# yifangao112/DinoUNet

Hardware: AMD Instinct MI355X
Metric: 2D slices/sec training, dinounet_l 512x512 bf16 (higher is better)
Workload: dtype bf16; 1 GPU; dinounet_l train step (fwd+loss+bwd+clip+SGD), 512x512x3 slices, batch 8/GPU, frozen ViT + adapter + FAPM + U-Net decoder, random-init weights; global_batch=8, parallelism=dp1

## Files before the change

### dinounet_amd/_lib.py

```python
import ctypes as C
import os
import re

HERE = os.path.dirname(os.path.abspath(__file__))
LIB_PATH = os.path.join(HERE, "libdinounet_hip.so")
HEADER = os.path.join(os.path.dirname(HERE), "include", "dinounet_hip.h")

DU_F32, DU_BF16 = 0, 1
PLAIN_ROW, PLAIN_COL, IM2COL_ROW, IM2COL_COL = 0, 1, 2, 3
ACT_NONE, ACT_GELU, ACT_RELU, ACT_LEAKY, ACT_SWIGLU = 0, 1, 2, 3, 4
STORE_PLAIN, STORE_PIXEL_SHUFFLE2, STORE_QKV_ROPE, STORE_SLABS, STORE_QKV_HEADS, STORE_MSDA_PREP = 0, 1, 2, 4, 5, 6
ERRORS = {-1: "DU_ERR_BAD_ARG", -2: "DU_ERR_UNSUPPORTED", -3: "DU_ERR_LAUNCH"}


class ConvGeom(C.Structure):
    _fields_ = [("p2", C.c_void_p), ("ld2", C.c_int64), ("C1", C.c_int32), ("Hi", C.c_int32), ("Wi", C.c_int32),
                ("C", C.c_int32), ("KH", C.c_int32), ("KW", C.c_int32), ("stride", C.c_int32), ("pad", C.c_int32),
                ("Ho", C.c_int32), ("Wo", C.c_int32), ("transposed", C.c_int32)]


class GemmArgs(C.Structure):
    _fields_ = [("dtype", C.c_int32), ("out_dtype", C.c_int32), ("a_mode", C.c_int32), ("b_mode", C.c_int32),
                ("M", C.c_int32), ("N", C.c_int32), ("K", C.c_int32),
                ("A", C.c_void_p), ("lda", C.c_int64), ("a_batch_stride", C.c_int64),
                ("B", C.c_void_p), ("ldb", C.c_int64), ("b_batch_stride", C.c_int64),
                ("C", C.c_void_p), ("ldc", C.c_int64), ("c_batch_stride", C.c_int64),
                ("batch", C.c_int32), ("split_k", C.c_int32), ("alpha", C.c_float),
                ("bias", C.c_void_p), ("act", C.c_int32), ("gamma", C.c_void_p),
                ("row_scale", C.c_void_p), ("rs_rows", C.c_int32),
                ("residual", C.c_void_p), ("ldr", C.c_int64),
                ("store_mode", C.c_int32), ("ps_H", C.c_int32), ("ps_W", C.c_int32), ("ps_C", C.c_int32),
                ("geom", ConvGeom), ("ws", C.c_void_p), ("ws_elems", C.c_int64),
                ("rope_sin", C.c_void_p), ("rope_cos", C.c_void_p), ("rope_prefix", C.c_int32), ("rope_qscale", C.c_float),
                ("a_colsum", C.c_void_p), ("b_colsum", C.c_void_p), ("C2", C.c_void_p), ("ks_ws", C.c_void_p), ("ks_ws_bytes", C.c_int64)]


class TnJob(C.Structure):
    _fields_ = [("A", C.c_void_p), ("lda", C.c_int64), ("B", C.c_void_p), ("ldb", C.c_int64), ("C", C.c_void_p), ("ldc", C.c_int64),
                ("a_colsum", C.c_void_p), ("alpha", C.c_void_p), ("M", C.c_int32), ("N", C.c_int32), ("K", C.c_int32),
                ("accumulate", C.c_int32), ("b_colsum", C.c_void_p),
                ("gather", C.c_int32), ("Hs", C.c_int32), ("Ws", C.c_int32), ("Cb", C.c_int32),
                ("taps", C.c_int32), ("inner", C.c_int32), ("inner_total", C.c_int32), ("c_off", C.c_int32)]


_CTYPE = {"int": C.c_int, "int64_t": C.c_int64, "float": C.c_float, "int32_t": C.c_int32, "double": C.c_double}


def header_prototypes(path=HEADER):
    src = open(path).read()
    src = re.sub(r"/\*.*?\*/", "", src, flags=re.S)
    protos = {}
    for m in re.finditer(r"\b(int64_t|int|const char\*)\s+(du_\w+)\s*\(([^;]*?)\)\s*;", src, flags=re.S):
        ret, name, args = m.group(1), m.group(2), m.group(3).strip()
        types = []
        if args and args != "void":
            for a in args.split(","):
                a = a.strip()
                if "*" in a:
                    types.append(C.c_void_p)
                else:
                    types.append(_CTYPE[a.split()[0] if not a.startswith("const") else a.split()[1]])
        protos[name] = (C.c_char_p if "char" in ret else (C.c_int64 if ret == "int64_t" else C.c_int), types)
    return protos


_lib = None


def lib():
    global _lib
    if _lib is None:
        if not os.path.exists(LIB_PATH):
            raise RuntimeError(
                f"{LIB_PATH} not found: the HIP extension is required (no CPU / eager fallback exists). "
                "Build it with `python -m dinounet_amd._build` or `__graft_entry__.build()`.")
        l = C.CDLL(LIB_PATH)
        for name, (ret, types) in header_prototypes().items():
            fn = getattr(l, name)
            fn.restype = ret
            fn.argtypes = types
        _lib = l
        for kv in os.environ.get("DINOUNET_LIB_OPTIONS", "").split(","):
            if "=" in kv:
                k, v = kv.split("=", 1)
                l.du_set_option(int(k), int(v))
    return _lib


def check(rc: int, what: str):
    if rc != 0:
        raise RuntimeError(f"dinounet_hip: {what} failed with {ERRORS.get(rc, rc)}")
```

### dinounet_amd/csrc/gemm.hip

```cpp
#include "common.h"
#include "gemm_params.h"
#include "gemm_plan.h"

namespace {

template <typename T, int MODE, int OUTER, int BK, int NT>
struct TileLoader {
  static constexpr int VEC = Elem<T>::VEC;
  static constexpr int LDS_LD = BK + VEC;
  static constexpr int TOTAL = OUTER * BK / VEC;
  static constexpr int NV = (TOTAL + NT - 1) / NT;
  static constexpr bool ROWMODE = (MODE == DU_PLAIN_ROW || MODE == DU_IM2COL_ROW);
  static constexpr int KV = BK / VEC;
  static constexpr int OV = OUTER / VEC;

  uint4 regs[NV];
  int pb[NV], py[NV], px[NV];

  __device__ __forceinline__ void init(const Operand& op, int tid, int o0, int outer_dim, int kbeg) {
    if constexpr (MODE == DU_IM2COL_ROW) {
#pragma unroll
      for (int i = 0; i < NV; i++) {
        int v = tid + i * NT;
        int o = o0 + v / KV;
// ... 320 lines not shown
      return;
    }
  }
  const int c = du_gemm_p8_choice(a);
  if (c) { multi_phase(a, c, 0); return; }
  if (du_gemm_glds_serves(a)) { p.family = 2; return; }
  if (du_gemm_modes_served(a.a_mode, a.b_mode)) p.family = 1; else p.rc = DU_ERR_UNSUPPORTED;
}

int64_t plan_ks_bytes(const du_gemm_args& a) {
  if (a.dtype != DU_BF16 || a.a_mode != DU_PLAIN_ROW || a.b_mode != DU_PLAIN_ROW) return 0;
  du_gemm_args head = a;
  head.ks_ws = nullptr; head.ks_ws_bytes = 0;
  int r = a.M % 256;
  if (r < 1 || r > 64 || !du_gemm_p8_tail_ok(a, r)) r = 0;
  head.M = a.M - r;
  const long pair = du_gemm_p8_ks_bytes(head);
  const int c = r > 0 ? du_gemm_p8_choice(head) : 0;
  const long tail = (c == 1 || c == 2) ? du_gemm_p8_tail_bytes(a) : 0;
  return pair > tail ? pair : tail;
}

int plan_check(const du_gemm_args& a, int family) {
  if (a.M <= 0 || a.N <= 0 || a.K <= 0) return DU_ERR_BAD_ARG;
  if (!a.A || !a.B || !a.C) return DU_ERR_BAD_ARG;
  const int vec = a.dtype == DU_BF16 ? 8 : 4;
  if (a.dtype != DU_BF16 && a.dtype != DU_F32) return DU_ERR_BAD_ARG;
  if (a.out_dtype != DU_BF16 && a.out_dtype != DU_F32) return DU_ERR_BAD_ARG;
  if (!aligned16(a.A) || !aligned16(a.B)) return DU_ERR_BAD_ARG;
  auto chk = [&](int mode, long ld, int outer, long bs) {
    if (ld % vec || bs % vec) return false;
    if (mode == DU_PLAIN_ROW) return a.K % vec == 0;
    if (mode == DU_PLAIN_COL) return outer % vec == 0;
    return true;
  };
  if (!chk(a.a_mode, a.lda, a.M, a.a_batch_stride) || !chk(a.b_mode, a.ldb, a.N, a.b_batch_stride)) return DU_ERR_BAD_ARG;
  const bool a_i2c = (a.a_mode == DU_IM2COL_ROW), b_i2c = (a.b_mode == DU_IM2COL_COL);
  if (a_i2c || b_i2c) {
    const du_conv_geom& g = a.geom;
    if (g.C % vec || g.KH <= 0 || g.KW <= 0 || g.stride <= 0) return DU_ERR_BAD_ARG;
    if (g.p2 && (g.C1 % vec || g.ld2 % vec || !aligned16(g.p2))) return DU_ERR_BAD_ARG;
    if (a_i2c && a.K != g.KH * g.KW * g.C) return DU_ERR_BAD_ARG;
    if (b_i2c && a.N != g.KH * g.KW * g.C) return DU_ERR_BAD_ARG;
  }
  const bool k_scale = a.row_scale && a.a_mode == DU_PLAIN_COL;
  if (k_scale && (family != 1 || a.rs_rows <= 0 || a.rs_rows % 64 || a.bias || a.act || a.gamma || a.residual || a.store_mode)) return DU_ERR_UNSUPPORTED;
  if (a.split_k > 1 && (a.out_dtype != DU_F32 || a.bias || a.act || a.gamma || (a.row_scale && !k_scale) || a.residual ||
                        (a.store_mode && a.store_mode != DU_STORE_SLABS))) return DU_ERR_BAD_ARG;
  if (a.store_mode == DU_STORE_SLABS && (a.split_k <= 1 || a.batch > 1 || family != 1)) return DU_ERR_UNSUPPORTED;
  if (a.store_mode == DU_STORE_PIXEL_SHUFFLE2 && (a.ps_C <= 0 || a.N != 4 * a.ps_C || a.ps_H <= 0 || a.ps_W <= 0 || a.M % (a.ps_H * a.ps_W))) return DU_ERR_BAD_ARG;
  const bool wgrad = a.a_mode == DU_PLAIN_COL && (family == 1 || family == 5);
  if (a.b_colsum && (!wgrad || a.b_mode != DU_IM2COL_COL || a.geom.C <= 0 || a.N % a.geom.C)) return DU_ERR_UNSUPPORTED;
  if (a.a_colsum && !wgrad) return DU_ERR_UNSUPPORTED;
  return DU_OK;
}

}

GemmPlan du_gemm_plan(const du_gemm_args& a) {
  static const bool generic_only = DU_GETENV("DU_GEMM_GENERIC") != nullptr;
  GemmPlan p{};
  plan_kernels(a, generic_only, p);
  if (!generic_only) {
    p.ws_elems = du_gemm_ragged_rows(a) > 0 ? du_gemm_skinny_ws_elems(a.N, a.K) : 0;
    p.ks_ws_bytes = plan_ks_bytes(a);
  }
  const int rc = plan_check(a, p.family);
  if (rc != DU_OK) p.rc = rc;
  return p;
}

extern "C" int du_gemm_route(const du_gemm_args* pa) { return pa ? du_gemm_plan(*pa).family : DU_ERR_BAD_ARG; }
extern "C" int64_t du_gemm_ws_elems(const du_gemm_args* pa) { return pa ? du_gemm_plan(*pa).ws_elems : 0; }
extern "C" int64_t du_gemm_ks_ws_bytes(const du_gemm_args* pa) { return pa ? du_gemm_plan(*pa).ks_ws_bytes : 0; }

extern "C" int du_gemm_plan_describe(const du_gemm_args* pa, int64_t* out, int n) {
  if (!pa || !out || n < 9) return DU_ERR_BAD_ARG;
  const GemmPlan p = du_gemm_plan(*pa);
  const int64_t v[9] = {p.rc, p.family, p.variant, p.gather, p.tail_rows, p.tail_form, p.tn_splits, p.ws_elems, p.ks_ws_bytes};
  for (int i = 0; i < 9; i++) out[i] = v[i];
  return 9;
}

extern "C" int du_gemm(const du_gemm_args* pa, void* stream) {
  if (!pa) return DU_ERR_BAD_ARG;
  const GemmPlan p = du_gemm_plan(*pa);
  if (p.rc != DU_OK) return p.rc;
  hipStream_t st = (hipStream_t)stream;
  du_gemm_args head = *pa, tail = *pa;
  if (p.tail_rows) split_rows(*pa, p.tail_rows, head, tail);
  int rc;
  if (p.variant) rc = du_gemm_nt_p8(head, st, p.variant, p.tail_form == DU_TAIL_RIDES ? p.tail_rows : 0);
  else switch (p.family) {
    case 0: rc = launch_generic(head, st); break;
    case 1: rc = du_gemm_bf16_tiles(head, st); break;
    case 2: rc = du_gemm_nt_glds(head, st); break;
    case 5: rc = du_gemm_tn_p8(head, st, p.tn_splits); break;
    default: rc = du_gemm_nt_rk(head, st); break;
  }
  if (rc != DU_OK) return rc;
  switch (p.tail_form) {
    case DU_TAIL_SKINNY_FUSED: case DU_TAIL_SKINNY_PAIR: return du_gemm_skinny(tail, st, p.tail_form);
    case DU_TAIL_TILE_ENGINE: tail.ws = nullptr; tail.ws_elems = 0; return du_gemm_bf16_tiles(tail, st);
  }
  return rc;
}
```

### dinounet_amd/csrc/gemm_p8.hip

```cpp
#include <algorithm>
#include <vector>
#include "common.h"
#include "gemm_params.h"
#include "gemm_plan.h"
#include "gemm_skinny_body.h"

namespace {

typedef __attribute__((address_space(3))) void lds_void;

constexpr int PBM = 256, PBN = 256, PBK = 64;
constexpr int HALF_B = 128 * PBK * 2;
constexpr int BUF_B = 4 * HALF_B;
constexpr int STG_LD = PBN + 4;

template <typename TC> struct Out4p;
template <> struct Out4p<float> {
  static __device__ __forceinline__ void load(const float* p, float* v) { float4 t = *(const float4*)p; v[0] = t.x; v[1] = t.y; v[2] = t.z; v[3] = t.w; }
  static __device__ __forceinline__ void store(float* p, const float* v) { *(float4*)p = make_float4(v[0], v[1], v[2], v[3]); }
};
template <> struct Out4p<bf16_t> {
  static __device__ __forceinline__ void load(const bf16_t* p, float* v) {
    bf16x4 t = __builtin_bit_cast(bf16x4, *(const uint2*)p);
#pragma unroll
// ... 1353 lines not shown
    stage_block_f32(acc[2 * h][0], stg, N_STG_LDF, wm * 64 + (lane & 31), wn * 64, lane);
    stage_block_f32(acc[2 * h][1], stg, N_STG_LDF, wm * 64 + (lane & 31), wn * 64 + 32, lane);
    stage_block_f32(acc[2 * h + 1][0], stg, N_STG_LDF, wm * 64 + 32 + (lane & 31), wn * 64, lane);
    stage_block_f32(acc[2 * h + 1][1], stg, N_STG_LDF, wm * 64 + 32 + (lane & 31), wn * 64 + 32, lane);
    __syncthreads();
    auto half = [&](auto w_c) {
      constexpr int w = decltype(w_c)::value;
      const int mrow0 = m0 + w * 128 + h * 64;
      const float* sp = stg + w * 64 * N_STG_LDF;
      if constexpr (sizeof(TC) == 4) {
        if (pre) {
          constexpr int CW = NBN / 4;
          float4 rr[8];
#pragma unroll
          for (int u = 0; u < 8; u++) {
            const int v = tid + u * 256;
            const int m = mrow0 + v / CW, n = n0 + (v % CW) * 4;
            rr[u] = (m < P.M && n < P.N) ? *(const float4*)((const float*)Rb + (long)m * P.ldr + n) : make_float4(0.f, 0.f, 0.f, 0.f);
          }
#pragma unroll
          for (int u = 0; u < 8; u++) {
            const int v = tid + u * 256;
            const int row = v / CW, cw = v % CW;
            const int m = mrow0 + row, n = n0 + cw * 4;
            if (m < P.M && n < P.N) {
              const float4 tt = *(const float4*)(sp + row * N_STG_LDF + cw * 4);
              float o[4] = {tt.x * P.alpha, tt.y * P.alpha, tt.z * P.alpha, tt.w * P.alpha};
              if (P.bias) {
                const float4 bb = *(const float4*)(P.bias + n);
                o[0] += bb.x; o[1] += bb.y; o[2] += bb.z; o[3] += bb.w;
              }
              if (P.act != DU_ACT_NONE) {
#pragma unroll
                for (int e = 0; e < 4; e++) o[e] = apply_act(o[e], P.act);
              }
              if (P.gamma) {
                const float4 gg = *(const float4*)(P.gamma + n);
                o[0] *= gg.x; o[1] *= gg.y; o[2] *= gg.z; o[3] *= gg.w;
              }
              if (P.row_scale) {
                const float rs = P.row_scale[m / P.rs_rows];
#pragma unroll
                for (int e = 0; e < 4; e++) o[e] *= rs;
              }
              *(float4*)((float*)Cb + (long)m * P.ldc + n) = make_float4(o[0] + rr[u].x, o[1] + rr[u].y, o[2] + rr[u].z, o[3] + rr[u].w);
            }
          }
          return;
        }
      }
      readout_f32_any<TC, NBN, 256>(P, sp, N_STG_LDF, 64, mrow0, n0, Cb, Rb, tid);
    };
    half(IC<0>{});
    half(IC<1>{});
  };
  pass(IC<0>{});
  pass(IC<1>{});
}

constexpr int PP_BIAS_OFF = P8N_LDS;
constexpr int PP_LDS = P8N_LDS + 3 * 128 * 4;
constexpr unsigned PP_OOR = 0x80000000u;

__device__ __forceinline__ void pp_swap_halves(unsigned& a, unsigned& b) {
  asm volatile("s_nop 1\n\tv_permlane32_swap_b32 %0, %1" : "+v"(a), "+v"(b));
}
__device__ __forceinline__ void pp_lds_read1(f32x4& a, unsigned addr) { asm volatile("ds_read_b128 %0, %1" : "=&v"(a) : "v"(addr)); }
__device__ __forceinline__ void pp_wait_lds(f32x4& a, f32x4& b) { asm volatile("s_waitcnt lgkmcnt(0)" : "+v"(a), "+v"(b) : : "memory"); }
__device__ __forceinline__ void pp_wait_lds1(f32x4& a) { asm volatile("s_waitcnt lgkmcnt(0)" : "+v"(a) : : "memory"); }

struct PpIdent {
  unsigned short v[128 * 128];
  constexpr PpIdent() : v() { for (int i = 0; i < 128; i++) v[i * 128 + i] = 0x3F80; }
};
__device__ const PpIdent g_pp_ident{};

constexpr int PP_ROPE_OFF = PP_BIAS_OFF + 2048;
constexpr int PP_ROPE_ROWS = 33;
constexpr int PP_LDS_ROPE = PP_ROPE_OFF + 2 * PP_ROPE_ROWS * 128;
__device__ __forceinline__ void pp_wait_lds4(f32x4& a, f32x4& b, f32x4& c, f32x4& d) {
  asm volatile("s_waitcnt lgkmcnt(0)" : "+v"(a), "+v"(b), "+v"(c), "+v"(d) : : "memory");
}

template <int ACT, bool NK4, int RES = 0, bool PS = false, int QKV = 0>
__global__ __launch_bounds__(512) void gemm_nt_pp_kernel(GemmParams P) {
  constexpr bool ROPE = QKV == 1, HEADS = QKV == 2;
  extern __shared__ __attribute__((aligned(16))) unsigned char smem[];
  if (P.tail_rows && (int)blockIdx.x >= P.main_wgs) { p8_tail<bf16_t>(P, smem); return; }
  static_assert(RES == 0 || ACT == DU_ACT_NONE, "the residual form has no activation");
  static_assert(QKV == 0 || (ACT == DU_ACT_NONE && !NK4 && RES == 0 && !PS), "the qkv stores: plain bias epilogue, K >= 384");
  constexpr bool FOUR = NK4 && RES == 0;
  const int tid = threadIdx.x, lane = tid & 63, hi = lane >> 5;
  const int wave = __builtin_amdgcn_readfirstlane(tid >> 6);
  const int wm = wave >> 1, wn = wave & 1;
  const int G = P.main_wgs;
  int lin;
  {
    const int bid = blockIdx.x, q = G >> 3, r = G & 7, xcd = bid & 7, idx = bid >> 3;
    lin = (xcd < r ? xcd * (q + 1) : r * (q + 1) + (xcd - r) * q) + idx;
  }
  const int ntiles = P.tiles_m * P.tiles_n;
  const int nk = P.K / PBK + (RES ? 2 : 0);
  auto coords = [&](int tile, int& m0, int& n0) {
    int tm, tn;
    if (P.group_m > 1) {
      const int band = P.group_m * P.tiles_n;
      const int g = tile / band, l = tile - g * band;
      const int first = g * P.group_m;
      const int gsz = min(P.tiles_m - first, P.group_m);
      tn = l / gsz; tm = first + (l - tn * gsz);
    } else {
      tm = tile / P.tiles_n; tn = tile - tm * P.tiles_n;
    }
    m0 = tm * PBM; n0 = tn * NBN;
  };

  const auto ra = __builtin_amdgcn_make_buffer_rsrc((void*)P.a.p, 0, (int)((((long)P.M - 1) * P.a.ld + P.K) * 2), 0x00020000);
  const auto rb = __builtin_amdgcn_make_buffer_rsrc((void*)P.b.p, 0, (int)((((long)P.N - 1) * P.b.ld + P.K) * 2), 0x00020000);
  const long out_rows = PS ? 4L * P.M : (long)P.M;
  const int out_cols = PS ? P.ps_C : P.N;
  const auto rc = __builtin_amdgcn_make_buffer_rsrc(P.C, 0, QKV ? (int)(3 * P.ldc * 2) : (int)(((out_rows - 1) * P.ldc + out_cols) * 2), 0x00020000);
  const int ps_lw = PS ? __builtin_ctz(P.ps_W) : 0, ps_lh = PS ? __builtin_ctz(P.ps_H) : 0;
  auto ps_pixel = [&](unsigned m) -> unsigned {
    const unsigned x = m & (unsigned)(P.ps_W - 1), y = (m >> ps_lw) & (unsigned)(P.ps_H - 1), b = m >> (ps_lw + ps_lh);
    return ((b * 2u * (unsigned)P.ps_H + 2u * y) * 2u * (unsigned)P.ps_W) + 2u * x;
  };
  const auto rbias = __builtin_amdgcn_make_buffer_rsrc(P.bias ? (void*)P.bias : P.C, 0, P.bias ? P.N * 4 : 0, 0x00020000);
  const int nrec_r = RES ? (int)(((out_rows - 1) * P.ldr + out_cols) * 2) : 0;
  const unsigned ldr2 = (unsigned)(P.ldr * 2);

  const int lc = (lane & 7) ^ (((wave & 1) << 2) | (lane >> 4));
  int srow[2];
  unsigned va0[2][2], vb0[2];
#pragma unroll
  for (int r = 0; r < 2; r++) {
    srow[r] = (r * 8 + wave) * 8 + (lane >> 3);
    va0[0][r] = (unsigned)srow[r] * (unsigned)(P.a.ld * 2) + lc * 16;
    va0[1][r] = (unsigned)(128 + srow[r]) * (unsigned)(P.a.ld * 2) + lc * 16;
    vb0[r] = (unsigned)srow[r] * (unsigned)(P.b.ld * 2) + lc * 16;
  }
  const unsigned lds_base = (unsigned)(unsigned long long)(__attribute__((address_space(3))) unsigned char*)smem;
  unsigned va_s[2][2], vb_s[2];
  unsigned sa_base = 0, sb_base = 0, sr_base = 0;
  unsigned sm0 = 0;
  unsigned sn0 = 0;
  auto set_stage_tile = [&](int tile, int slot) {
    if (tile < ntiles) {
      int m0, n0;
      coords(tile, m0, n0);
#pragma unroll
      for (int r = 0; r < 2; r++) {
        if constexpr (ROPE) {
          sm0 = (unsigned)m0; sn0 = (unsigned)n0;
        } else {
          va_s[0][r] = m0 + srow[r] < P.M ? va0[0][r] : PP_OOR;
          va_s[1][r] = m0 + 128 + srow[r] < P.M ? va0[1][r] : PP_OOR;
          vb_s[r] = n0 + srow[r] < P.N ? vb0[r] : PP_OOR;
        }
      }
      sa_base = (unsigned)m0 * (unsigned)(P.a.ld * 2);
      sb_base = (unsigned)n0 * (unsigned)(P.b.ld * 2);
      if constexpr (RES != 0 && !PS) sr_base = (unsigned)m0 * ldr2 + (unsigned)n0 * 2u;
      if constexpr (RES != 0 && PS) {
        const int q = n0 / P.ps_C, co0 = n0 - q * P.ps_C;
        sr_base = (unsigned)((q >> 1) * 2 * P.ps_W + (q & 1)) * ldr2 + (unsigned)co0 * 2u;
        sm0 = (unsigned)m0;
      }
      if (wave < 2) {
        const unsigned lds_dst = __builtin_amdgcn_readfirstlane(lds_base + PP_BIAS_OFF + slot * 512 + wave * 256);
        const unsigned voff = (unsigned)(n0 + wave * 64 + lane) * 4u;
        unsigned keep;
        asm volatile("s_mov_b32 %0, m0\n\ts_mov_b32 m0, %3\n\ts_nop 0\n\tbuffer_load_dword %1, %2, 0 offen lds\n\ts_mov_b32 m0, %0"
                     : "=&s"(keep) : "v"(voff), "s"(rbias), "s"(lds_dst) : "memory");
      }
    } else {
#pragma unroll
      for (int r = 0; r < 2; r++) { va_s[0][r] = PP_OOR; va_s[1][r] = PP_OOR; vb_s[r] = PP_OOR; }
      if constexpr (ROPE) { sm0 = 0x7fffffffu; sn0 = 0x7fffffffu; }
    }
  };
  const auto rr = __builtin_amdgcn_make_buffer_rsrc(RES ? (void*)P.residual : (void*)P.a.p, 0, nrec_r, 0x00020000);
  const auto ri = __builtin_amdgcn_make_buffer_rsrc((void*)g_pp_ident.v, 0, 32768, 0x00020000);
  auto stage = [&](auto which_c, int bo, unsigned kofs, auto ext_c) {
    constexpr int which = decltype(which_c)::value;
    constexpr bool EXT = RES != 0 && decltype(ext_c)::value != 0;
#pragma unroll
    for (int r = 0; r < 2; r++) {
      unsigned char* dst = smem + bo + which * HALF_B + (r * 8 + wave) * 1024;
      if constexpr (EXT) {
        unsigned sr = (unsigned)srow[r];
        asm volatile("" : "+v"(sr));
        if constexpr (which < 2) {
          const unsigned rowi = PS ? ps_pixel(sm0 + which * 128u + sr) : which * 128u + sr;
          const unsigned vext = va_s[which][r] == PP_OOR ? PP_OOR : rowi * ldr2 + (unsigned)lc * 16u;
          __builtin_amdgcn_raw_ptr_buffer_load_lds(rr, (lds_void*)dst, 16, vext, sr_base + kofs, 0, 0);
        } else {
          __builtin_amdgcn_raw_ptr_buffer_load_lds(ri, (lds_void*)dst, 16, sr * 256u + (unsigned)lc * 16u, kofs, 0, 0);
        }
      } else if constexpr (ROPE) {
        unsigned sr = (unsigned)srow[r];
        asm volatile("" : "+v"(sr));
        if constexpr (which < 2) {
          const unsigned row = which * 128u + sr;
          const unsigned vo = sm0 + row < (unsigned)P.M ? row * (unsigned)(P.a.ld * 2) + (unsigned)lc * 16u : PP_OOR;
          __builtin_amdgcn_raw_ptr_buffer_load_lds(ra, (lds_void*)dst, 16, vo, sa_base + kofs, 0, 0);
        } else {
          const unsigned vo = sn0 + sr < (unsigned)P.N ? sr * (unsigned)(P.b.ld * 2) + (unsigned)lc * 16u : PP_OOR;
          __builtin_amdgcn_raw_ptr_buffer_load_lds(rb, (lds_void*)dst, 16, vo, sb_base + kofs, 0, 0);
        }
      } else {
        if constexpr (which < 2) __builtin_amdgcn_raw_ptr_buffer_load_lds(ra, (lds_void*)dst, 16, va_s[which][r], sa_base + kofs, 0, 0);
        else __builtin_amdgcn_raw_ptr_buffer_load_lds(rb, (lds_void*)dst, 16, vb_s[r], sb_base + kofs, 0, 0);
      }
    }
  };
  int L[4];
  {
    const int x = hi ^ ((lane >> 1) & 7);
#pragma unroll
    for (int kk = 0; kk < 4; kk++) L[kk] = (lane & 31) * 128 + ((x ^ (2 * kk)) << 4);
  }
  const int aoff = wm * 32 * 128, boff = 2 * HALF_B + wn * 64 * 128;

  bf16x8 Af[2][4];
  bf16x8 Bf[2][2][4];
  f32x16 acc[2][2];
  f32x16 prev[2][2];
#pragma unroll
  for (int i = 0; i < 2; i++)
#pragma unroll
    for (int c = 0; c < 2; c++)
#pragma unroll
      for (int r = 0; r < 16; r++) prev[i][c][r] = 0.f;
  auto readA = [&](auto set_c, int bo) {
    constexpr int set = decltype(set_c)::value;
#pragma unroll
    for (int kk = 0; kk < 4; kk++) Af[set][kk] = *(const bf16x8*)(smem + bo + set * HALF_B + aoff + L[kk]);
  };
  auto readB = [&](auto set_c, int bo) {
    constexpr int set = decltype(set_c)::value;
#pragma unroll
    for (int c = 0; c < 2; c++)
#pragma unroll
      for (int kk = 0; kk < 4; kk++) Bf[set][c][kk] = *(const bf16x8*)(smem + bo + boff + c * 4096 + L[kk]);
  };
  auto mma = [&](auto i_c, auto bset_c, auto first_c) {
    constexpr int i = decltype(i_c)::value, bset = decltype(bset_c)::value;
    constexpr bool FIRST = decltype(first_c)::value;
#pragma unroll
    for (int kk = 0; kk < 4; kk++)
#pragma unroll
      for (int c = 0; c < 2; c++) {
        if constexpr (FIRST) {
          if (kk == 0) {
            const f32x16 z = {0.f, 0.f, 0.f, 0.f, 0.f, 0.f, 0.f, 0.f, 0.f, 0.f, 0.f, 0.f, 0.f, 0.f, 0.f, 0.f};
            acc[i][c] = __builtin_amdgcn_mfma_f32_32x32x16_bf16(Bf[bset][c][kk], Af[i][kk], z, 0, 0, 0);
            continue;
          }
        }
        acc[i][c] = __builtin_amdgcn_mfma_f32_32x32x16_bf16(Bf[bset][c][kk], Af[i][kk], acc[i][c], 0, 0, 0);
      }
  };
  auto pin = [&](auto nrd_c, auto ndma_c) {
    constexpr int nrd = decltype(nrd_c)::value, ndma = decltype(ndma_c)::value;
#pragma unroll
    for (int m = 0; m < 8; m++) {
      __builtin_amdgcn_sched_group_barrier(0x008, 1, 0);
      if (m < 4) __builtin_amdgcn_sched_group_barrier(0x100, nrd / 4, 0);
      else if (m - 4 < ndma) __builtin_amdgcn_sched_group_barrier(0x020, 1, 0);
    }
  };
  const int nlim = (P.dbg & 1) ? 0 : P.N;
  unsigned pbias = lds_base + PP_BIAS_OFF + (unsigned)((wn * 64 + 4 * hi) * 4);
  unsigned crow[2] = {PP_OOR, PP_OOR};
  int pcol = 0;
  float rs_cur = 1.0f, rs_prev = 1.0f;
  unsigned trow[2] = {0u, 0u};
  float qs_prev = 1.0f;
  const unsigned rope_tbl = lds_base + PP_ROPE_OFF + (unsigned)(4 * hi * 4);
  auto set_prev_tile = [&](int tile) {
    int m0, n0;
    coords(tile, m0, n0);
    pcol = n0 + wn * 64 + hi * 8;
    if constexpr (QKV != 0) {
      const int hd = P.ps_C * 64, which = n0 / hd, head = ((n0 - which * hd) >> 6) + wn;
      if constexpr (ROPE) qs_prev = which == 0 ? P.rope_qscale : 1.0f;
#pragma unroll
      for (int i = 0; i < 2; i++) {
        const int m = m0 + i * 128 + wm * 32 + (lane & 31);
        const int b = m / P.ps_H, t = m - b * P.ps_H;
        crow[i] = m < P.M ? (unsigned)(((long)which * P.ldc + (((long)b * P.ps_C + head) * P.ps_W + t) * 64 + hi * (ROPE ? 4 : 8)) * 2) : PP_OOR;
        if constexpr (ROPE) {
          const int tt = t - P.rope_prefix, ty = tt / P.b.Wi, tx = tt - ty * P.b.Wi;
          trow[i] = (which < 2 && tt >= 0 && m < P.M) ? (unsigned)ty | ((unsigned)tx << 8) : (32u | (32u << 8));
        }
      }
      return;
    }
#pragma unroll
    for (int i = 0; i < 2; i++) {
      const int m = m0 + i * 128 + wm * 32 + (lane & 31);
      if constexpr (PS) {
        const int q = n0 / P.ps_C, co0 = n0 - q * P.ps_C;
        const unsigned pix = ps_pixel((unsigned)m) + (unsigned)((q >> 1) * 2 * P.ps_W + (q & 1));
        crow[i] = m < P.M ? (unsigned)(((long)pix * P.ldc + co0 + wn * 64 + hi * 8) * 2) : PP_OOR;
      } else {
        crow[i] = m < P.M ? (unsigned)(((long)m * P.ldc + pcol) * 2) : PP_OOR;
      }
    }
  };
  f32x4 bqa = {0.f, 0.f, 0.f, 0.f}, bqb = {0.f, 0.f, 0.f, 0.f};
  unsigned keep0 = 0u, keep1 = 0u;
  f32x4 cq = {0.f, 0.f, 0.f, 0.f}, sq = {0.f, 0.f, 0.f, 0.f};
  auto fetch = [&](auto h_c, f32x4& bq, unsigned base) {
    constexpr int h = decltype(h_c)::value;
    if constexpr (h >= 0) {
      if constexpr (ROPE) {
        constexpr int ph = h >> 1, c = h & 1, i = ph >> 2, g = ph & 3, axis = g >> 1;
        pp_lds_read1(bq, base + (unsigned)((c * 32 + 8 * g) * 4));
        if constexpr (c == 0) {
          const unsigned pos = axis ? (trow[i] >> 8) : (trow[i] & 0xffu);
          const unsigned ta = rope_tbl + (unsigned)(axis * PP_ROPE_ROWS * 128 + ((8 * g) & 15) * 4) + pos * 128u;
          pp_lds_read1(cq, ta);
          pp_lds_read1(sq, ta + 64u);
        }
      } else {
        constexpr int u = h >> 1, c = (u >> 1) & 1, g = 2 * (u & 1) + (h & 1);
        pp_lds_read1(bq, base + (unsigned)((c * 32 + 8 * g) * 4));
      }
    }
  };
  auto rope_pair = [&](auto h_c) {
    constexpr int h = decltype(h_c)::value;
    if constexpr (h >= 0) {
      constexpr int ph = h >> 1, i = ph >> 2, g = ph & 3, h2 = g >> 1;
      const f32x16& a0 = prev[i][0];
      const f32x16& a1 = prev[i][1];
      unsigned pk[4];
#pragma unroll
      for (int e = 0; e < 4; e += 2) {
        const float ca = cq[e], sa = sq[e], cb = cq[e + 1], sb = sq[e + 1];
        const float x1a = a0[4 * g + e] + bqa[e], x1b = a0[4 * g + e + 1] + bqa[e + 1];
        const float x2a = a1[4 * g + e] + bqb[e], x2b = a1[4 * g + e + 1] + bqb[e + 1];
        const float o1a = (x1a * ca - x2a * sa) * qs_prev, o1b = (x1b * cb - x2b * sb) * qs_prev;
        const float o2a = (x2a * ca + x1a * sa) * qs_prev, o2b = (x2b * cb + x1b * sb) * qs_prev;
        const bf16x2 t1 = {(bf16_t)o1a, (bf16_t)o1b}, t2 = {(bf16_t)o2a, (bf16_t)o2b};
        pk[e >> 1] = __builtin_bit_cast(unsigned, t1);
        pk[2 + (e >> 1)] = __builtin_bit_cast(unsigned, t2);
      }
      (void)h2;
      typedef unsigned u32x2_t __attribute__((ext_vector_type(2)));
      const u32x2_t v0 = {pk[0], pk[1]}, v1 = {pk[2], pk[3]};
      const unsigned off = nlim ? crow[i] + (unsigned)(8 * g * 2) : PP_OOR;
      __builtin_amdgcn_raw_buffer_store_b64(v0, rc, off, 0, 0);
      __builtin_amdgcn_raw_buffer_store_b64(v1, rc, off == PP_OOR ? PP_OOR : off + 64u, 0, 0);
    }
  };
  auto half = [&](auto h_c, const f32x4& bq) {
    constexpr int h = decltype(h_c)::value;
    if constexpr (h >= 0) {
      constexpr int u = h >> 1, part = h & 1, i = u >> 2, c = (u >> 1) & 1, h2 = u & 1, g = 2 * h2 + part;
      const f32x16& a = prev[i][c];
      f32x2 o0, o1;
      if constexpr (RES == 2) {
        o0 = {__builtin_fmaf(bq[0], rs_prev, a[4 * g]), __builtin_fmaf(bq[1], rs_prev, a[4 * g + 1])};
        o1 = {__builtin_fmaf(bq[2], rs_prev, a[4 * g + 2]), __builtin_fmaf(bq[3], rs_prev, a[4 * g + 3])};
      } else {
        o0 = {a[4 * g] + bq[0], a[4 * g + 1] + bq[1]}; o1 = {a[4 * g + 2] + bq[2], a[4 * g + 3] + bq[3]};
      }
      if constexpr (ACT == DU_ACT_GELU) { o0 = gelu_pk(o0); o1 = gelu_pk(o1); }
      const bf16x2 t0 = {(bf16_t)o0.x, (bf16_t)o0.y}, t1 = {(bf16_t)o1.x, (bf16_t)o1.y};
      if constexpr (part == 0) {
        keep0 = __builtin_bit_cast(unsigned, t0); keep1 = __builtin_bit_cast(unsigned, t1);
      } else {
        unsigned k4 = __builtin_bit_cast(unsigned, t0), k5 = __builtin_bit_cast(unsigned, t1);
        pp_swap_halves(keep0, k4);
        pp_swap_halves(keep1, k5);
        const u32x4_t v = {keep0, keep1, k4, k5};
        const unsigned off = pcol + c * 32 + 16 * h2 < nlim ? crow[i] + (unsigned)((c * 32 + 16 * h2) * 2) : PP_OOR;
        __builtin_amdgcn_raw_buffer_store_b128(v, rc, off, 0, 0);
      }
    }
  };
  auto finish6 = [&]() {
    __builtin_amdgcn_sched_barrier(0);
    asm volatile("s_waitcnt vmcnt(6)" ::: "memory");
    if constexpr (ROPE) pp_wait_lds4(bqa, bqb, cq, sq); else pp_wait_lds(bqa, bqb);
    __builtin_amdgcn_s_barrier();
    __builtin_amdgcn_sched_barrier(0);
  };
// ... 68 lines not shown

  int bc = 0, bn = NBUF_B, bnn = 2 * NBUF_B;
  int slot = 0;
  auto rot2 = [&]() { const int o = bc; bc = bnn; bnn = bn; bn = o; };
  auto bias_at = [&](int sl) { return lds_base + PP_BIAS_OFF + (unsigned)(sl * 512 + (wn * 64 + 4 * hi) * 4); };
  for (;;) {
    const int next = tile + G;
    if constexpr (RES == 2) {
      int m0c, n0c;
      coords(tile, m0c, n0c);
      rs_cur = P.row_scale[__builtin_amdgcn_readfirstlane(m0c / P.rs_rows)];
    }
    if constexpr (FOUR) {
      const int nslot = slot == 2 ? 0 : slot + 1;
      dstep(IC<0>{}, IC<0>{}, bc, bn, bnn, 2u * 128u, 0u);
      dstep(IC<1>{}, IC<1>{}, bn, bnn, bc, 3u * 128u, 0u);
      rot2();
      set_stage_tile(next, nslot);
      dstep(IC<2>{}, IC<0>{}, bc, bn, bnn, 0u, 0u);
      dstep(IC<3>{}, IC<1>{}, bn, bnn, bc, 128u, bias_at(slot));
      rot2();
      pbias = bias_at(slot);
      set_prev_tile(tile);
      slot = nslot;
    } else {
      dstep(IC<0>{}, IC<0>{}, bc, bn, bnn, 2u * 128u, 0u);
      dstep(IC<1>{}, IC<1>{}, bn, bnn, bc, 3u * 128u, 0u);
      rot2();
      dstep(IC<2>{}, IC<0>{}, bc, bn, bnn, 4u * 128u, 0u);
      dstep(IC<3>{}, IC<1>{}, bn, bnn, bc, 5u * 128u, 0u);
      rot2();
      int t = 4;
      for (; t + (RES != 0 && !NK4 ? 4 : 2) < nk; t += 2) {
        kstep(IC<0>{}, F_{}, N_{}, N_{}, N_{}, N_{}, N_{}, N_{}, F_{}, F_{}, bc, bn, bnn, (unsigned)(t + 2) * 128u, 0u, 0u, IC<0>{}, IC<0>{});
        kstep(IC<1>{}, F_{}, N_{}, N_{}, N_{}, N_{}, N_{}, N_{}, F_{}, F_{}, bn, bnn, bc, (unsigned)(t + 3) * 128u, 0u, 0u, IC<0>{}, IC<0>{});
        rot2();
      }
      if constexpr (RES != 0 && !NK4) {
        kstep(IC<0>{}, F_{}, N_{}, N_{}, N_{}, N_{}, N_{}, N_{}, F_{}, F_{}, bc, bn, bnn, 0u, 0u, 0u, IC<0>{}, IC<1>{});
        kstep(IC<1>{}, F_{}, N_{}, N_{}, N_{}, N_{}, N_{}, N_{}, F_{}, F_{}, bn, bnn, bc, 128u, 0u, 0u, IC<1>{}, IC<1>{});
        rot2();
      }
      set_stage_tile(next, slot ^ 1);
      pbias = bias_at(slot);
      if constexpr (ROPE) set_prev_tile(tile);
      kstep(IC<0>{}, F_{}, N_{}, N_{}, N_{}, N_{}, N_{}, N_{}, F_{}, F_{}, bc, bn, bnn, 0u, 0u, 0u, IC<2>{}, IC<0>{});
      kstep(IC<1>{}, F_{}, N_{}, N_{}, N_{}, N_{}, IC<0>{}, IC<1>{}, F_{}, T_{}, bn, bnn, bc, 128u, 0u, pbias, IC<0>{}, IC<0>{});
      rot2();
      if constexpr (!ROPE) set_prev_tile(tile);
      rs_prev = rs_cur;
      slot ^= 1;
    }
    tile = next;
    if (tile >= ntiles) break;
  }
  prev[1][0] = acc[1][0]; prev[1][1] = acc[1][1];
  if (P.dbg & 2) return;
  auto last = [&](auto h_c) {
    constexpr int h = decltype(h_c)::value;
    pp_wait_lds(bqa, bqb);
    __builtin_amdgcn_sched_barrier(0);
    if constexpr (h & 1) half(h_c, bqb); else half(h_c, bqa);
    __builtin_amdgcn_sched_barrier(0);
    if constexpr (h & 1) { fetch(IC<(h + 1 < 16 ? h + 1 : -1)>{}, bqa, pbias); fetch(IC<(h + 2 < 16 ? h + 2 : -1)>{}, bqb, pbias); }
  };
  auto last_pair = [&](auto ph_c) {
    constexpr int ph = decltype(ph_c)::value;
    pp_wait_lds4(bqa, bqb, cq, sq);
    __builtin_amdgcn_sched_barrier(0);
    rope_pair(IC<2 * ph>{});
    __builtin_amdgcn_sched_barrier(0);
    fetch(IC<(ph + 1 < 8 ? 2 * ph + 2 : -1)>{}, bqa, pbias); fetch(IC<(ph + 1 < 8 ? 2 * ph + 3 : -1)>{}, bqb, pbias);
  };
  if constexpr (ROPE) {
    last_pair(IC<0>{}); last_pair(IC<1>{}); last_pair(IC<2>{}); last_pair(IC<3>{});
    last_pair(IC<4>{}); last_pair(IC<5>{}); last_pair(IC<6>{}); last_pair(IC<7>{});
  } else {
    last(IC<0>{}); last(IC<1>{}); last(IC<2>{}); last(IC<3>{}); last(IC<4>{}); last(IC<5>{}); last(IC<6>{}); last(IC<7>{});
    last(IC<8>{}); last(IC<9>{}); last(IC<10>{}); last(IC<11>{}); last(IC<12>{}); last(IC<13>{}); last(IC<14>{}); last(IC<15>{});
  }
  if (P.tail_rows && (int)gridDim.x == G) p8_tail_inline<bf16_t>(P, smem, lin, G);
}

int g_p8_mode = -1;
int g_p8_sched = 1;
int g_p8_corun = 1;
int g_p8_persist = 1;
int g_p8_tail_inline = 0;
int g_p8_res = 1;
int g_p8_pp_full = 0;
int g_p8_group = 4;
int g_p8_debug = 0;

constexpr long KS_STATE_BYTES = 131072;
int g_p8_tail_slices = 1;
static int tail_slices_for(const du_gemm_args& a, bool have_ws) {
  if (!g_p8_tail_slices || a.K < (g_p8_tail_slices >= 2 ? 1024 : 2048) || g_p8_tail_inline) return 1;
  const int units = (a.N + SK_BN - 1) / SK_BN;
  int s = a.K / 512;
  if (s > 8) s = 8;
  while (s > 1 && (a.K % (s * SK_CHUNK) || units * s > 256)) s--;
  if (s < 2 || units > 16384) return 1;
  if (have_ws && (!a.ks_ws || a.ks_ws_bytes < KS_STATE_BYTES + (long)units * s * 64 * SK_BN * 4)) return 1;
  return s;
}

template <typename TC, int SCHED, bool NARROW, bool GA = false>
int launch_p8(const du_gemm_args& a, hipStream_t st, int tail_rows = 0) {
  static_assert(!(NARROW && GA), "the gather form exists for the 256 x 256 kernel only");
  constexpr int LDS_BYTES = NARROW ? P8N_LDS : P8_LDS;
  constexpr int TBN = NARROW ? NBN : PBN;
  GemmParams P = make_params(a, GA ? DU_IM2COL_ROW : DU_PLAIN_ROW, DU_PLAIN_ROW, PBM, TBN, PBK);
  P.tiles_m = (a.M + PBM - 1) / PBM;
  P.group_m = g_p8_group;
  P.dbg = g_p8_debug;
  dim3 grid(P.tiles_m * P.tiles_n, a.batch < 1 ? 1 : a.batch);
  if (tail_rows > 0 && !GA) {
    P.tail_rows = tail_rows; P.main_wgs = P.tiles_m * P.tiles_n;
    if (!(g_p8_tail_inline && grid.y == 1 && (long)grid.x * g_p8_corun >= 256)) {
      P.tail_slices = tail_slices_for(a, true); P.ks_ws = a.ks_ws;
      grid.x += (a.N + SK_BN - 1) / SK_BN * P.tail_slices;
    }
  }
  void (*kfn)(GemmParams);
  if constexpr (NARROW) kfn = gemm_nt_p8n_kernel<TC, SCHED>; else kfn = gemm_nt_p8_kernel<TC, SCHED, false, GA>;
  static bool attr_set = false;
  if (!attr_set) {
    if (hipFuncSetAttribute((const void*)kfn, hipFuncAttributeMaxDynamicSharedMemorySize, LDS_BYTES) != hipSuccess) return DU_ERR_LAUNCH;
    attr_set = true;
  }
  hipLaunchKernelGGL(kfn, grid, dim3(512), LDS_BYTES, st, P);
  return du_check_launch();
}

int launch_pp(const du_gemm_args& a, hipStream_t st, int tail_rows = 0) {
  GemmParams P = make_params(a, DU_PLAIN_ROW, DU_PLAIN_ROW, PBM, NBN, PBK);
  P.tiles_m = (a.M + PBM - 1) / PBM;
  P.group_m = g_p8_group;
  P.dbg = g_p8_debug;
  const long ntiles = (long)P.tiles_m * P.tiles_n;
  const long cus = g_p8_pp_full ? 256 : 256 / g_p8_corun;
  P.main_wgs = (int)(ntiles < cus ? ntiles : cus);
  dim3 grid(P.main_wgs, 1);
  if (tail_rows > 0) {
    P.tail_rows = tail_rows;
    if (!g_p8_tail_inline) grid.x += (a.N + SK_BN - 1) / SK_BN;
  }
  const bool nk4 = a.K == 256;
  const int res = a.residual ? (a.row_scale ? 2 : 1) : 0;
  const bool ps = a.store_mode == DU_STORE_PIXEL_SHUFFLE2;
  const bool rope = a.store_mode == DU_STORE_QKV_ROPE;
  const bool heads = a.store_mode == DU_STORE_QKV_HEADS;
  if (rope) { P.b.Hi = a.geom.Hi; P.b.Wi = a.geom.Wi; }
  void (*kfn)(GemmParams);
  if (rope) kfn = gemm_nt_pp_kernel<DU_ACT_NONE, false, 0, false, 1>;
  else if (heads) kfn = gemm_nt_pp_kernel<DU_ACT_NONE, false, 0, false, 2>;
  else if (ps) kfn = gemm_nt_pp_kernel<DU_ACT_NONE, false, 1, true>;
  else if (res == 2) kfn = nk4 ? gemm_nt_pp_kernel<DU_ACT_NONE, true, 2> : gemm_nt_pp_kernel<DU_ACT_NONE, false, 2>;
  else if (res == 1) kfn = nk4 ? gemm_nt_pp_kernel<DU_ACT_NONE, true, 1> : gemm_nt_pp_kernel<DU_ACT_NONE, false, 1>;
  else if (nk4) kfn = a.act == DU_ACT_GELU ? gemm_nt_pp_kernel<DU_ACT_GELU, true> : gemm_nt_pp_kernel<DU_ACT_NONE, true>;
  else kfn = a.act == DU_ACT_GELU ? gemm_nt_pp_kernel<DU_ACT_GELU, false> : gemm_nt_pp_kernel<DU_ACT_NONE, false>;
  static bool attr_set[11] = {false, false, false, false, false, false, false, false, false, false, false};
  const int lds_bytes = rope ? PP_LDS_ROPE : PP_LDS;
  const int ai = heads ? 10 : rope ? 9 : ps ? 8 : (res ? 2 + 2 * res + (nk4 ? 1 : 0) : (a.act == DU_ACT_GELU ? 1 : 0) + (nk4 ? 2 : 0));
  if (!attr_set[ai]) {
    if (hipFuncSetAttribute((const void*)kfn, hipFuncAttributeMaxDynamicSharedMemorySize, lds_bytes) != hipSuccess) return DU_ERR_LAUNCH;
    attr_set[ai] = true;
  }
  hipLaunchKernelGGL(kfn, grid, dim3(512), lds_bytes, st, P);
  return du_check_launch();
}

template <typename TC>
int launch_p4(const du_gemm_args& a, hipStream_t st, int tail_rows = 0) {
  GemmParams P = make_params(a, DU_PLAIN_ROW, DU_PLAIN_ROW, PBM, NBN, 32);
  P.tiles_m = (a.M + PBM - 1) / PBM;
  P.group_m = g_p8_group;
  P.dbg = g_p8_debug;
  dim3 grid(P.tiles_m * P.tiles_n, a.batch < 1 ? 1 : a.batch);
  if (tail_rows > 0) {
    P.tail_rows = tail_rows; P.main_wgs = P.tiles_m * P.tiles_n;
    grid.x += (a.N + SK_BN - 1) / SK_BN;
  }
  void (*kfn)(GemmParams) = gemm_nt_p4_kernel<TC>;
  static bool attr_set = false;
  if (!attr_set) {
    if (hipFuncSetAttribute((const void*)kfn, hipFuncAttributeMaxDynamicSharedMemorySize, P4_LDS) != hipSuccess) return DU_ERR_LAUNCH;
    attr_set = true;
  }
  hipLaunchKernelGGL(kfn, grid, dim3(256), P4_LDS, st, P);
  return du_check_launch();
}

int g_p8_ks = 0;
inline long ks_ws_need(long tiles) { return KS_STATE_BYTES + tiles * 2 * PBM * PBN * 4; }

int launch_p8ks(const du_gemm_args& a, hipStream_t st, int tail_rows) {
  GemmParams P = make_params(a, DU_PLAIN_ROW, DU_PLAIN_ROW, PBM, PBN, PBK);
  P.tiles_m = (a.M + PBM - 1) / PBM;
  P.group_m = g_p8_group;
  P.dbg = g_p8_debug;
  P.ks_ws = a.ks_ws;
  P.main_wgs = 2 * P.tiles_m * P.tiles_n;
  dim3 grid(P.main_wgs, 1);
  if (tail_rows > 0) { P.tail_rows = tail_rows; grid.x += (a.N + SK_BN - 1) / SK_BN; }
  void (*kfn)(GemmParams) = g_p8_sched ? gemm_nt_p8ks_kernel<1> : gemm_nt_p8ks_kernel<0>;
  static bool attr_set[2] = {false, false};
  if (!attr_set[g_p8_sched ? 1 : 0]) {
    if (hipFuncSetAttribute((const void*)kfn, hipFuncAttributeMaxDynamicSharedMemorySize, P8_LDS) != hipSuccess) return DU_ERR_LAUNCH;
    attr_set[g_p8_sched ? 1 : 0] = true;
  }
  hipLaunchKernelGGL(kfn, grid, dim3(512), P8_LDS, st, P);
  return du_check_launch();
}

int g_p8_tn = 1;

template <int SCHED, bool GA>
int launch_p8_tn(const du_gemm_args& a, int splits, hipStream_t st) {
  GemmParams P = make_params(a, DU_PLAIN_COL, GA ? DU_IM2COL_COL : DU_PLAIN_COL, PBM, PBN, PBK);
  P.tiles_m = (a.M + PBM - 1) / PBM;
  P.split_k = splits;
  P.k_per_split = 0;
  P.dbg = g_p8_debug;
  dim3 grid(P.tiles_m * P.tiles_n * splits, 1);
  void (*kfn)(GemmParams) = GA ? gemm_nt_p8_kernel<float, SCHED, true, true> : gemm_nt_p8_kernel<float, SCHED, true, false>;
  static bool attr_set = false;
  if (!attr_set) {
    if (hipFuncSetAttribute((const void*)kfn, hipFuncAttributeMaxDynamicSharedMemorySize, P8_LDS) != hipSuccess) return DU_ERR_LAUNCH;
    attr_set = true;
  }
  hipLaunchKernelGGL(kfn, grid, dim3(512), P8_LDS, st, P);
  return du_check_launch();
}

}

extern int g_attn_w;
extern int g_attn_impl, g_attn_thresh_log2, g_attn_var;
extern int g_rk_mode;
extern int g_wgrad_rows;
extern int g_ln_rows2;
extern int g_dwconv_band;

extern "C" int du_set_option(int key, int value) {
  switch (key) {
    case 4: g_attn_w = value; return DU_OK;
    case 6: g_attn_impl = value; return DU_OK;
    case 7: g_attn_thresh_log2 = value; return DU_OK;
    case 8: g_attn_var = value; return DU_OK;
    case 0: g_p8_mode = value; return DU_OK;
    case 1: g_p8_sched = value; return DU_OK;
// ... 73 lines not shown
    if ((4L * a.M * a.ldc + a.N) * 2 >= 0x7fffffffL || (4L * a.M * a.ldr + a.N) * 2 >= 0x7fffffffL) return false;
  } else if (a.store_mode != DU_STORE_PLAIN) return false;
  if (a.gamma || a.alpha != 1.0f || (a.act != DU_ACT_NONE && a.act != DU_ACT_GELU)) return false;
  if ((a.K != 256 && a.K < 384) || a.N % 8 || a.ldc % 8 || (((uintptr_t)a.C) & 15)) return false;
  const long lim = 0x7fffffffL;
  if (a.residual) {
    if (a.act != DU_ACT_NONE || a.N % 128 || a.ldr % 8 || (((uintptr_t)a.residual) & 15)) return false;
    if (a.row_scale && (a.rs_rows < 256 || a.rs_rows % 256)) return false;
    if (((long)a.M * a.ldr + a.N) * 2 >= lim) return false;
  } else if (a.row_scale) return false;
  return ((long)a.M * a.lda + a.K) * 2 < lim && ((long)a.N * a.ldb + a.K) * 2 < lim && ((long)a.M * a.ldc + a.N) * 2 < lim;
}

static bool ks_shape_ok(const du_gemm_args& a) {
  if (!p8_legal(a) || a.out_dtype != DU_F32 || a.store_mode != DU_STORE_PLAIN || a.batch > 1 || a.act == DU_ACT_SWIGLU) return false;
  if (a.K % 256 || a.K < 1024 || g_p8_corun != 1) return false;
  const long tiles = (long)((a.M + 255) / 256) * ((a.N + 255) / 256);
  return tiles % 8 == 0 && tiles >= 64 && tiles <= 128;
}
static bool ks_legal(const du_gemm_args& a) {
  if (!ks_shape_ok(a) || !a.ks_ws || (((uintptr_t)a.ks_ws) & 15)) return false;
  return a.ks_ws_bytes >= ks_ws_need((long)((a.M + 255) / 256) * ((a.N + 255) / 256));
}

int du_gemm_p8_choice(const du_gemm_args& a) {
  if (g_p8_mode != 0 && g_p8_tn && p8_gather_legal(a))
    return (g_p8_mode > 0 || (long)((a.M + 255) / 256) * ((a.N + 255) / 256) >= 192) ? 1 : 0;
  if (g_p8_mode == 0 || !p8_legal(a)) return 0;
  if (a.store_mode == DU_STORE_MSDA_PREP) return 1;
  if (a.store_mode == DU_STORE_QKV_HEADS) return (g_p8_mode != 0 && pp_legal(a)) ? 4 : 0;
  if (a.store_mode == DU_STORE_QKV_ROPE) {
    const long t = (long)((a.M + 255) / 256) * ((a.N + 127) / 128);
    return (g_p8_persist && g_p8_mode != 2 && pp_legal(a) && (g_p8_persist > 1 || g_p8_mode == 4 || t >= 2 * (256 / g_p8_corun))) ? 4 : 2;
  }
  if (g_p8_ks && g_p8_mode < 0 && ks_legal(a)) return 5;
  if (g_p8_mode == 5) return ks_legal(a) ? 5 : 2;
  if (g_p8_mode == 3) return a.act == DU_ACT_SWIGLU ? 2 : 3;
  if (g_p8_mode == 4) return pp_legal(a) ? 4 : 2;
  if (g_p8_mode > 0) return g_p8_mode == 2 ? 2 : 1;
  const long batch = a.batch < 1 ? 1 : a.batch;
  const long tm = (a.M + 255) / 256;
  const long t256 = tm * ((a.N + 255) / 256) * batch, t128 = tm * ((a.N + 127) / 128) * batch;
  const long cus = 256 / g_p8_corun;
  if (t128 * g_p8_corun < 192) return 0;
  const double c256 = (double)((t256 + cus - 1) / cus) * 1.0, c128 = (double)((t128 + cus - 1) / cus) * (a.K >= 1024 ? 0.68 : 0.56);
  if (g_p8_persist && pp_legal(a)) {
    if (a.residual) {
      if (g_p8_res && (g_p8_persist > 1 || t128 >= 2 * cus)) return 4;
    } else {
    const double r = a.K <= 256 ? 0.40 : (a.K <= 512 ? 0.45 : (a.act == DU_ACT_GELU ? 0.49 : 0.53));
    const double cpp = (double)((t128 + cus - 1) / cus) * r;
    const double best = (t256 * g_p8_corun >= 128 && c256 <= c128) ? c256 : c128;
    if (g_p8_persist > 1 || (t128 >= 2 * cus && cpp < best)) return 4;
    }
  }
  if (t256 * g_p8_corun >= 128 && c256 <= c128) return 1;
  return 2;
}
bool du_gemm_p8_wants(const du_gemm_args& a) { return du_gemm_p8_choice(a) != 0; }
long du_gemm_p8_tail_bytes(const du_gemm_args& whole) {
  const int s = tail_slices_for(whole, false);
  return s > 1 ? KS_STATE_BYTES + (long)((whole.N + SK_BN - 1) / SK_BN) * s * 64 * SK_BN * 4 : 0;
}
long du_gemm_p8_ks_bytes(const du_gemm_args& a) {
  if (!(g_p8_ks && g_p8_mode < 0) && g_p8_mode != 5) return 0;
  return ks_shape_ok(a) ? ks_ws_need((long)((a.M + 255) / 256) * ((a.N + 255) / 256)) : 0;
}

int du_gemm_nt_p8(const du_gemm_args& a, hipStream_t st, int c, int tail_rows) {
  if (a.a_mode == DU_IM2COL_ROW) return g_p8_sched ? launch_p8<bf16_t, 1, false, true>(a, st) : launch_p8<bf16_t, 0, false, true>(a, st);
  const bool bf = a.out_dtype == DU_BF16;
  const int tr = tail_rows;
  if (c == 5) return launch_p8ks(a, st, tr);
  if (c == 4) return launch_pp(a, st, tr);
  if (c == 3) return bf ? launch_p4<bf16_t>(a, st, tr) : launch_p4<float>(a, st, tr);
  if (c == 1) {
    if (bf) return g_p8_sched ? launch_p8<bf16_t, 1, false>(a, st, tr) : launch_p8<bf16_t, 0, false>(a, st, tr);
    return g_p8_sched ? launch_p8<float, 1, false>(a, st, tr) : launch_p8<float, 0, false>(a, st, tr);
  }
  if (bf) return g_p8_sched ? launch_p8<bf16_t, 1, true>(a, st, tr) : launch_p8<bf16_t, 0, true>(a, st, tr);
  return g_p8_sched ? launch_p8<float, 1, true>(a, st, tr) : launch_p8<float, 0, true>(a, st, tr);
}

bool du_gemm_p8_tail_ok(const du_gemm_args& whole, int r) {
  static const bool off = DU_GETENV("DU_P8_NO_TAIL") != nullptr;
  static const int kmax = DU_GETENV("DU_SKINNY_FUSE_KMAX") ? atoi(DU_GETENV("DU_SKINNY_FUSE_KMAX")) : 4096;
  if (off || r < 1 || r > 64 || whole.K > kmax || whole.K % SK_CHUNK || whole.N % 4 || whole.batch > 1) return false;
  if ((whole.store_mode != DU_STORE_PLAIN && whole.store_mode != DU_STORE_QKV_HEADS) || whole.act == DU_ACT_SWIGLU ||
      whole.a_mode != DU_PLAIN_ROW || whole.b_mode != DU_PLAIN_ROW) return false;
  return 8 * 64 * (SK_BN + 1) * 4 <= P8_LDS;
}

int du_gemm_tn_p8_splits(const du_gemm_args& a) {
  if (!g_p8_tn || g_p8_mode == 0) return 0;
  if (a.dtype != DU_BF16 || a.out_dtype != DU_F32 || a.a_mode != DU_PLAIN_COL) return 0;
  if (a.b_mode != DU_PLAIN_COL && a.b_mode != DU_IM2COL_COL) return 0;
  if (a.split_k <= 1 || a.batch > 1 || a.store_mode != DU_STORE_PLAIN) return 0;
  if (a.bias || a.act || a.gamma || a.row_scale || a.residual) return 0;
  if (a.K % 128 || a.K < 512 || a.M <= 128 || a.N <= 128) return 0;
  if (a.lda % 8 || a.ldb % 8 || (((uintptr_t)a.A) & 15) || (((uintptr_t)a.B) & 15)) return 0;
  if (a.b_mode == DU_IM2COL_COL) {
    if (!convt_gather_geom(a, a.B, a.ldb, a.K) || a.N != 4 * a.geom.C || a.geom.C % 256) return 0;
    if (a.geom.Wo & (a.geom.Wo - 1)) return 0;
  }
  const long tiles = (long)((a.M + 255) / 256) * ((a.N + 255) / 256);
  const int npairs = a.K / 128;
  long s = tiles >= 256 ? 1 : 256 / tiles;
  if (s > npairs / 2) s = npairs / 2;
  if (s < 1) s = 1;
  if (g_p8_tn < 2 && npairs / s < 16) return 0;
  const long ldmax = a.b_mode == DU_PLAIN_COL && a.ldb > a.lda ? a.ldb : a.lda;
  if ((long)(npairs / s + 1) * 128 * ldmax * 2 > 0x7fffffffL) return 0;
  return (int)s;
}

static bool pow2(int x) { return x > 0 && (x & (x - 1)) == 0; }
static bool tn_group_legal(const du_tn_job& j) {
  if (!j.A || !j.B || !j.C || j.M <= 0 || j.N <= 0) return false;
  if (j.K % 128 || j.K < 512) return false;
  if (j.lda % 8 || j.ldb % 8 || j.lda < j.M) return false;
  if ((((uintptr_t)j.A) | ((uintptr_t)j.B)) & 15) return false;
  if (j.lda > 0x7fffffffL / 4 || j.ldb > 0x7fffffffL / 4 || j.ldc > 0x7fffffffL) return false;
  if (j.taps > 1 && (j.inner <= 0 || j.N != j.taps * j.inner)) return false;
  if (j.taps <= 1 && j.ldc < j.N) return false;
  if (((long)j.K + 128) * j.lda * 2 > 0x7fffffffL) return false;
  if (j.taps > 1 && (j.c_off < 0 || j.inner_total < j.c_off + j.inner)) return false;
  if (j.gather == 0) {
    if (j.ldb < j.N || j.b_colsum) return false;
    return ((long)j.K + 128) * j.ldb * 2 <= 0x7fffffffL;
  }
  if (j.gather != 2 && j.gather != 3) return false;
  if (j.Cb <= 0 || j.Cb % 8 || j.ldb < j.Cb || !pow2(j.Ws) || j.Hs <= 0 || j.K % (j.Hs * j.Ws)) return false;
  if (j.gather == 2) {
    if (j.N != 4 * j.Cb) return false;
    return (long)j.K * 4 * j.ldb * 2 <= 0x7fffff00L;
  }
  if (j.N != 9 * j.Cb || !pow2(j.Hs) || j.b_colsum) return false;
  if (j.Ws % 64) return false;
  return (long)j.K * j.ldb * 2 <= 0x7fffff00L;
}
extern "C" int du_gemm_tn_group_legal(const du_tn_job* job) { return (job && g_p8_mode != 0 && tn_group_legal(*job)) ? 1 : 0; }

template <int GG>
static int tn_group_launch(const du_tn_job* const* jobs, int njobs, hipStream_t st) {
  static const int target_units = DU_GETENV("DU_TN_GROUP_UNITS") ? atoi(DU_GETENV("DU_TN_GROUP_UNITS")) : 256;
  static const int min_pairs = DU_GETENV("DU_TN_GROUP_MINPAIRS") ? atoi(DU_GETENV("DU_TN_GROUP_MINPAIRS")) : 8;
  void (*kfn)(TnGroupArgs) = g_p8_sched ? gemm_tn_group_kernel<1, GG> : gemm_tn_group_kernel<0, GG>;
  static bool attr_set[2] = {false, false};
  if (!attr_set[g_p8_sched ? 1 : 0]) {
    if (hipFuncSetAttribute((const void*)kfn, hipFuncAttributeMaxDynamicSharedMemorySize, P8_LDS) != hipSuccess) return DU_ERR_LAUNCH;
    attr_set[g_p8_sched ? 1 : 0] = true;
  }
  static const int max_jobs = DU_GETENV("DU_TN_GROUP_MAXJOBS") ? std::max(1, std::min(TN_GROUP_MAX, atoi(DU_GETENV("DU_TN_GROUP_MAXJOBS")))) : TN_GROUP_MAX;
  int i0 = 0;
  while (i0 < njobs) {
    int tiles[TN_GROUP_MAX], pairs[TN_GROUP_MAX], splits[TN_GROUP_MAX];
    int n = 0, units = 0;
    while (i0 + n < njobs && n < max_jobs) {
      const du_tn_job& j = *jobs[i0 + n];
      const int t = ((j.M + PBM - 1) / PBM) * ((j.N + PBN - 1) / PBN);
      if (n > 0 && units + t > target_units) break;
      tiles[n] = t; pairs[n] = j.K / 128; splits[n] = 1;
      units += t; n++;
    }
    for (;;) {
      int best = -1; double len = 0.0;
// ... 50 lines not shown
```

### dinounet_amd/csrc/gemm_plan.h

```cpp
#pragma once
#include "common.h"

enum { DU_TAIL_NONE = 0, DU_TAIL_RIDES = 1, DU_TAIL_SKINNY_FUSED = 2, DU_TAIL_SKINNY_PAIR = 3, DU_TAIL_TILE_ENGINE = 4 };

struct GemmPlan {
  int rc;
  int family;
  int variant;
  int gather;
  int tail_rows;
  int tail_form;
  int tn_splits;
  int64_t ws_elems;
  int64_t ks_ws_bytes;
};

GemmPlan du_gemm_plan(const du_gemm_args& a);

bool du_gemm_modes_served(int a_mode, int b_mode);
int du_gemm_bf16_tiles(const du_gemm_args& a, hipStream_t st);
int du_gemm_ragged_rows(const du_gemm_args& a);
bool du_gemm_glds_serves(const du_gemm_args& a);
int du_gemm_nt_glds(const du_gemm_args& a, hipStream_t st);
bool du_gemm_rk_serves(const du_gemm_args& a);
int du_gemm_nt_rk(const du_gemm_args& a, hipStream_t st);
bool p8_legal(const du_gemm_args& a);
int du_gemm_p8_choice(const du_gemm_args& a);
bool du_gemm_p8_tail_ok(const du_gemm_args& whole, int r);
long du_gemm_p8_ks_bytes(const du_gemm_args& a);
long du_gemm_p8_tail_bytes(const du_gemm_args& whole);
int du_gemm_nt_p8(const du_gemm_args& a, hipStream_t st, int choice, int tail_rows);
int du_gemm_tn_p8_splits(const du_gemm_args& a);
int du_gemm_tn_p8(const du_gemm_args& a, hipStream_t st, int splits);
int du_gemm_skinny_form(const du_gemm_args& a);
int64_t du_gemm_skinny_ws_elems(int N, int K);
int du_gemm_skinny(const du_gemm_args& a, hipStream_t st, int form);
```

### dinounet_amd/csrc/norm.hip

```cpp
#include "common.h"
#include "ln_bwd_row.h"

int g_ln_rows2 = 1;

namespace {

template <typename TI, typename TO, int MAXV>
__global__ __launch_bounds__(256) void layernorm_fwd_kernel(const TI* __restrict__ x, long ldx, const float* __restrict__ w,
                                                            const float* __restrict__ b, TO* __restrict__ y, long ldy,
                                                            float* __restrict__ mean_out, float* __restrict__ rstd_out,
                                                            long rows, int D, float eps) {
  constexpr int VI = Elem<TI>::VEC;
  const int lane = threadIdx.x & 63;
  const long row = (long)blockIdx.x * 4 + (threadIdx.x >> 6);
  if (row >= rows) return;
  const int nvec = D / VI;
  float v[MAXV][VI];
  float s = 0.f;
#pragma unroll
  for (int i = 0; i < MAXV; i++) {
    int vi = lane + i * 64;
    if (vi < nvec) {
      Vec16<TI> t = as_vec<TI>(*(const uint4*)(x + row * ldx + (long)vi * VI));
#pragma unroll
      for (int j = 0; j < VI; j++) { v[i][j] = to_f32(t.v[j]); s += v[i][j]; }
    } else {
#pragma unroll
      for (int j = 0; j < VI; j++) v[i][j] = 0.f;
    }
  }
  const float mean = wave_sum(s) / (float)D;
  float s2 = 0.f;
#pragma unroll
  for (int i = 0; i < MAXV; i++) {
    int vi = lane + i * 64;
    if (vi < nvec) {
#pragma unroll
      for (int j = 0; j < VI; j++) { float d = v[i][j] - mean; s2 += d * d; }
    }
  }
  const float rstd = rsqrtf(wave_sum(s2) / (float)D + eps);
  if (lane == 0) {
    if (mean_out) mean_out[row] = mean;
    if (rstd_out) rstd_out[row] = rstd;
  }
#pragma unroll
  for (int i = 0; i < MAXV; i++) {
    int vi = lane + i * 64;
    if (vi < nvec) {
      const int c0 = vi * VI;
#pragma unroll
      for (int j = 0; j < VI; j++) y[row * ldy + c0 + j] = from_f32<TO>((v[i][j] - mean) * rstd * w[c0 + j] + b[c0 + j]);
    }
  }
}

template <typename TI, typename TO, int MAXV>
__global__ __launch_bounds__(256) void layernorm_fwd2_kernel(const TI* __restrict__ x, long ldx, const float* __restrict__ w,
                                                             const float* __restrict__ b, TO* __restrict__ y, long ldy,
                                                             float* __restrict__ mean_out, float* __restrict__ rstd_out,
                                                             long rows, int D, float eps) {
  constexpr int VI = Elem<TI>::VEC;
  const int lane = threadIdx.x & 63;
  const long row0 = ((long)blockIdx.x * 4 + (threadIdx.x >> 6)) * 2;
  if (row0 >= rows) return;
  const bool two = row0 + 1 < rows;
  const int nvec = D / VI;
  float v[2][MAXV][VI];
  float s[2] = {0.f, 0.f};
#pragma unroll
  for (int u = 0; u < 2; u++)
#pragma unroll
    for (int i = 0; i < MAXV; i++) {
      const int vi = lane + i * 64;
      if (vi < nvec && (u == 0 || two)) {
        Vec16<TI> t = as_vec<TI>(*(const uint4*)(x + (row0 + u) * ldx + (long)vi * VI));
#pragma unroll
        for (int j = 0; j < VI; j++) { v[u][i][j] = to_f32(t.v[j]); s[u] += v[u][i][j]; }
      } else {
#pragma unroll
        for (int j = 0; j < VI; j++) v[u][i][j] = 0.f;
      }
    }
  float mean[2], rstd[2];
#pragma unroll
  for (int u = 0; u < 2; u++) mean[u] = wave_sum(s[u]) / (float)D;
#pragma unroll
  for (int u = 0; u < 2; u++) {
    float s2 = 0.f;
#pragma unroll
    for (int i = 0; i < MAXV; i++) {
      const int vi = lane + i * 64;
      if (vi < nvec) {
#pragma unroll
        for (int j = 0; j < VI; j++) { const float d = v[u][i][j] - mean[u]; s2 += d * d; }
      }
    }
    rstd[u] = rsqrtf(wave_sum(s2) / (float)D + eps);
  }
  if (lane == 0) {
    if (mean_out) { mean_out[row0] = mean[0]; if (two) mean_out[row0 + 1] = mean[1]; }
    if (rstd_out) { rstd_out[row0] = rstd[0]; if (two) rstd_out[row0 + 1] = rstd[1]; }
  }
#pragma unroll
  for (int i = 0; i < MAXV; i++) {
    const int vi = lane + i * 64;
    if (vi < nvec) {
      const int c0 = vi * VI;
#pragma unroll
      for (int u = 0; u < 2; u++) {
        if (u == 1 && !two) break;
#pragma unroll
        for (int j = 0; j < VI; j++) y[(row0 + u) * ldy + c0 + j] = from_f32<TO>((v[u][i][j] - mean[u]) * rstd[u] * w[c0 + j] + b[c0 + j]);
      }
    }
  }
}

template <typename T, int MAXV>
__global__ __launch_bounds__(256) void layernorm_bwd_dx_kernel(const T* __restrict__ x, const T* __restrict__ dy,
                                                               const float* __restrict__ w, const float* __restrict__ mean,
                                                               const float* __restrict__ rstd, T* __restrict__ dx, long rows, int D,
                                                               const T* __restrict__ dres) {
  constexpr int VI = Elem<T>::VEC;
  const int lane = threadIdx.x & 63;
  const long row = (long)blockIdx.x * 4 + (threadIdx.x >> 6);
  if (row >= rows) return;
  const int nvec = D / VI;
  const float mu = mean[row], rs = rstd[row];
  float xh[MAXV][VI], g[MAXV][VI];
  float c1 = 0.f, c2 = 0.f;
#pragma unroll
  for (int i = 0; i < MAXV; i++) {
    int vi = lane + i * 64;
    if (vi < nvec) {
      Vec16<T> tx = as_vec<T>(*(const uint4*)(x + row * (long)D + (long)vi * VI));
      Vec16<T> tg = as_vec<T>(*(const uint4*)(dy + row * (long)D + (long)vi * VI));
#pragma unroll
// ... 3 lines not shown
        c1 += g[i][j];
        c2 += g[i][j] * xh[i][j];
      }
    }
  }
  c1 = wave_sum(c1) / (float)D;
  c2 = wave_sum(c2) / (float)D;
#pragma unroll
  for (int i = 0; i < MAXV; i++) {
    int vi = lane + i * 64;
    if (vi < nvec) {
      Vec16<T> o;
      if (dres) {
        Vec16<T> tr = as_vec<T>(*(const uint4*)(dres + row * (long)D + (long)vi * VI));
#pragma unroll
        for (int j = 0; j < VI; j++) o.v[j] = from_f32<T>(rs * (g[i][j] - c1 - xh[i][j] * c2) + to_f32(tr.v[j]));
      } else {
#pragma unroll
        for (int j = 0; j < VI; j++) o.v[j] = from_f32<T>(rs * (g[i][j] - c1 - xh[i][j] * c2));
      }
      *(uint4*)(dx + row * (long)D + (long)vi * VI) = as_u4(o);
    }
  }
}

template <typename T, int MAXV>
__global__ __launch_bounds__(256) void layernorm_bwd_fused_kernel(const T* __restrict__ x, const T* __restrict__ dy,
                                                                  const float* __restrict__ w, const float* __restrict__ mean,
                                                                  const float* __restrict__ rstd, T* __restrict__ dx, long rows, int D,
                                                                  const T* __restrict__ dres, int strip, float* __restrict__ part) {
  constexpr int VI = Elem<T>::VEC;
  extern __shared__ float ln_red[];
  const int lane = threadIdx.x & 63, wave = threadIdx.x >> 6;
  const int nvec = D / VI;
  float wv[MAXV][VI], sa[MAXV][VI], sb[MAXV][VI];
#pragma unroll
  for (int i = 0; i < MAXV; i++) {
    const int vi = lane + i * 64;
#pragma unroll
    for (int j = 0; j < VI; j++) { wv[i][j] = vi < nvec ? w[vi * VI + j] : 0.f; sa[i][j] = 0.f; sb[i][j] = 0.f; }
  }
  const long r0 = (long)blockIdx.x * strip;
  const long r1 = r0 + strip < rows ? r0 + strip : rows;
  for (long row0 = r0 + wave; row0 < r1; row0 += 8) {
    uint4 rx[2][MAXV], rg[2][MAXV];
    float mu[2], rs[2];
#pragma unroll
    for (int u = 0; u < 2; u++) {
      const long row = row0 + 4 * u;
      const bool live = row < r1;
      mu[u] = live ? mean[row] : 0.f; rs[u] = live ? rstd[row] : 0.f;
#pragma unroll
      for (int i = 0; i < MAXV; i++) {
        const int vi = lane + i * 64;
        rx[u][i] = make_uint4(0, 0, 0, 0); rg[u][i] = make_uint4(0, 0, 0, 0);
        if (live && vi < nvec) {
          rx[u][i] = *(const uint4*)(x + row * (long)D + (long)vi * VI);
          rg[u][i] = *(const uint4*)(dy + row * (long)D + (long)vi * VI);
        }
      }
    }
#pragma unroll
    for (int u = 0; u < 2; u++) {
      const long row = row0 + 4 * u;
      if (row >= r1) break;
      float xh[MAXV][VI], g[MAXV][VI];
      float c1 = 0.f, c2 = 0.f;
#pragma unroll
      for (int i = 0; i < MAXV; i++) {
        const int vi = lane + i * 64;
        if (vi < nvec) ln_bwd_row_terms<T>(rx[u][i], rg[u][i], mu[u], rs[u], wv[i], xh[i], g[i], c1, c2, sa[i], sb[i]);
      }
      c1 = wave_sum(c1) / (float)D;
      c2 = wave_sum(c2) / (float)D;
#pragma unroll
      for (int i = 0; i < MAXV; i++) {
        const int vi = lane + i * 64;
        if (vi < nvec) {
          uint4 o;
          if (dres) o = ln_bwd_row_dx<T, true>(xh[i], g[i], c1, c2, rs[u], *(const uint4*)(dres + row * (long)D + (long)vi * VI));
          else o = ln_bwd_row_dx<T, false>(xh[i], g[i], c1, c2, rs[u], make_uint4(0, 0, 0, 0));
          *(uint4*)(dx + row * (long)D + (long)vi * VI) = o;
        }
      }
    }
  }
  if (wave > 0) {
#pragma unroll
    for (int i = 0; i < MAXV; i++) {
      const int vi = lane + i * 64;
      if (vi < nvec) {
#pragma unroll
        for (int j = 0; j < VI; j += 2)
          *(float4*)(ln_red + ((long)(wave - 1) * D + vi * VI + j) * 2) = make_float4(sa[i][j], sb[i][j], sa[i][j + 1], sb[i][j + 1]);
      }
    }
  }
  __syncthreads();
  if (wave == 0) {
#pragma unroll
    for (int i = 0; i < MAXV; i++) {
      const int vi = lane + i * 64;
      if (vi < nvec) {
#pragma unroll
        for (int j = 0; j < VI; j += 2) {
          float4 t = make_float4(sa[i][j], sb[i][j], sa[i][j + 1], sb[i][j + 1]);
#pragma unroll
          for (int q = 0; q < 3; q++) {
            const float4 u = *(const float4*)(ln_red + ((long)q * D + vi * VI + j) * 2);
            t.x += u.x; t.y += u.y; t.z += u.z; t.w += u.w;
          }
          *(float4*)(part + ((long)blockIdx.x * D + vi * VI + j) * 2) = t;
        }
      }
    }
  }
}

static inline int pick_strip(int G, long P, int C, int vec) {
  const int cvb = (C / vec) < 256 ? (C / vec) : 256;
  const int np = 256 / (cvb > 0 ? cvb : 1);
  static const long tmax = DU_GETENV("DU_STRIP_TARGET") ? atol(DU_GETENV("DU_STRIP_TARGET")) : 512;
  long target = 65536L * 8 / C;
  if (target > tmax) target = tmax;
  if (target < 256) target = 256;
  long per_group = target / (G > 0 ? G : 1);
  if (per_group < 1) per_group = 1;
  long s = (P + per_group - 1) / per_group;
  const long smin = (long)np * 4;
  if (s < smin) s = smin;
  if (s > P) s = P;
  return (int)s;
}

template <typename T, int KIND>
struct StatOp;

template <int V, typename E>
__device__ __forceinline__ void lane_reduce(float* a, float* b, int cvb, int np, int tp, int tcv, float (*red)[256 * V], bool valid, E emit) {
  const bool pow2 = (cvb & (cvb - 1)) == 0;
  if (pow2 && cvb < 64) {
#pragma unroll
    for (int j = 0; j < V; j++) {
      for (int o = cvb; o < 64; o <<= 1) { a[j] += __shfl_xor(a[j], o, 64); b[j] += __shfl_xor(b[j], o, 64); }
    }
    const int wave = threadIdx.x >> 6, lane = threadIdx.x & 63;
    if (lane < cvb) {
#pragma unroll
      for (int j = 0; j < V; j++) { red[0][(wave * cvb + lane) * V + j] = a[j]; red[1][(wave * cvb + lane) * V + j] = b[j]; }
    }
    __syncthreads();
    if (threadIdx.x < cvb && valid) {
#pragma unroll
      for (int j = 0; j < V; j++) {
        float sa = 0.f, sb = 0.f;
#pragma unroll
        for (int q = 0; q < 4; q++) { sa += red[0][(q * cvb + threadIdx.x) * V + j]; sb += red[1][(q * cvb + threadIdx.x) * V + j]; }
        emit(j, sa, sb);
      }
    }
    __syncthreads();
    return;
  }
#pragma unroll
  for (int j = 0; j < V; j++) { red[0][threadIdx.x * V + j] = a[j]; red[1][threadIdx.x * V + j] = b[j]; }
  __syncthreads();
  if (tp == 0 && valid) {
#pragma unroll
    for (int j = 0; j < V; j++) {
      float sa = 0.f, sb = 0.f;
      for (int q = 0; q < np; q++) { sa += red[0][(q * cvb + tcv) * V + j]; sb += red[1][(q * cvb + tcv) * V + j]; }
      emit(j, sa, sb);
    }
  }
  __syncthreads();
}

template <typename T, typename F>
__device__ __forceinline__ void strip_reduce(int G, long P, int C, int STRIP, float* out , float* part, F f) {
  constexpr int V = Elem<T>::VEC;
  __shared__ float red[2][256 * V];
  const int cv_total = C / V;
  const long strips = (P + STRIP - 1) / STRIP;
  const int g = blockIdx.x / strips;
  const long p0 = (long)(blockIdx.x % strips) * STRIP;
  const long p1 = min(P, p0 + STRIP);
  const int cvb = min(cv_total, 256);
  const int tp = threadIdx.x / cvb;
  const int tcv = threadIdx.x % cvb;
  const int np = 256 / cvb;
  for (int cv0 = 0; cv0 < cv_total; cv0 += cvb) {
    const int cv = cv0 + tcv;
    float a[V], b[V];
#pragma unroll
    for (int j = 0; j < V; j++) { a[j] = 0.f; b[j] = 0.f; }
    if (cv < cv_total && tp < np) {
#pragma unroll 4
      for (long p = p0 + tp; p < p1; p += np) f((long)g * P + p, g, cv * V, a, b);
    }
    lane_reduce<V>(a, b, cvb, np, tp, tcv, red, cv < cv_total, [&](int j, float sa, float sb) {
      if (part) {
        part[((long)blockIdx.x * C + cv * V + j) * 2 + 0] = sa;
        part[((long)blockIdx.x * C + cv * V + j) * 2 + 1] = sb;
      } else {
        atomic_add_f32(out + ((long)g * C + cv * V + j) * 2 + 0, sa);
        atomic_add_f32(out + ((long)g * C + cv * V + j) * 2 + 1, sb);
      }
    });
  }
}

template <typename T>
__global__ __launch_bounds__(256) void layernorm_bwd_wb_kernel(const T* __restrict__ x, const T* __restrict__ dy,
                                                               const float* __restrict__ mean, const float* __restrict__ rstd,
                                                               float* __restrict__ out, long rows, int D, int strip, float* part) {
  constexpr int V = Elem<T>::VEC;
  strip_reduce<T>(1, rows, D, strip, out, part, [&](long row, int g, int c0, float* a, float* b) {
    Vec16<T> tx = as_vec<T>(*(const uint4*)(x + row * (long)D + c0));
    Vec16<T> tg = as_vec<T>(*(const uint4*)(dy + row * (long)D + c0));
    const float mu = mean[row], rs = rstd[row];
#pragma unroll
    for (int j = 0; j < V; j++) {
      float gy = to_f32(tg.v[j]);
      a[j] += gy * (to_f32(tx.v[j]) - mu) * rs;
      b[j] += gy;
    }
  });
}

template <typename T>
__global__ __launch_bounds__(256) void chan_stats_kernel(const T* __restrict__ x, long ldx, float* __restrict__ sums, int G,
                                                         long P, int C, int strip, float* part) {
  constexpr int V = Elem<T>::VEC;
  strip_reduce<T>(G, P, C, strip, sums, part, [&](long pix, int g, int c0, float* a, float* b) {
    Vec16<T> t = as_vec<T>(*(const uint4*)(x + pix * ldx + c0));
#pragma unroll
    for (int j = 0; j < V; j++) { float v = to_f32(t.v[j]); a[j] += v; b[j] += v * v; }
  });
}

template <typename T>
__global__ __launch_bounds__(256) void chan_dot_kernel(const T* __restrict__ a_, long lda, const T* __restrict__ b_, long ldb,
                                                       float* __restrict__ sums, int G, long P, int C, int strip, float* part) {
  constexpr int V = Elem<T>::VEC;
  strip_reduce<T>(G, P, C, strip, sums, part, [&](long pix, int g, int c0, float* a, float* b) {
    Vec16<T> ta = as_vec<T>(*(const uint4*)(a_ + pix * lda + c0));
    Vec16<T> tb = as_vec<T>(*(const uint4*)(b_ + pix * ldb + c0));
#pragma unroll
    for (int j = 0; j < V; j++) { float va = to_f32(ta.v[j]); a[j] += va * to_f32(tb.v[j]); b[j] += va; }
  });
}

template <typename T>
__global__ __launch_bounds__(256) void norm_act_fwd_kernel(const T* __restrict__ x, long ldx, T* __restrict__ y, long ldy,
                                                           const float* __restrict__ mean, const float* __restrict__ rstd,
                                                           const float* __restrict__ w, const float* __restrict__ b, long P,
                                                           int C, int act) {
  constexpr int V = Elem<T>::VEC;
  const int cvn = C / V, cvb = min(cvn, 256), np = 256 / cvb;
  const int tp = threadIdx.x / cvb, tcv = threadIdx.x % cvb;
  if (tp >= np) return;
  const int g = blockIdx.y;
  for (int cv = tcv; cv < cvn; cv += cvb) {
    const int c0 = cv * V;
    float sc[V], sh[V];
#pragma unroll
    for (int j = 0; j < V; j++) {
      sc[j] = rstd[(long)g * C + c0 + j] * w[c0 + j];
      sh[j] = b[c0 + j] - mean[(long)g * C + c0 + j] * sc[j];
    }
    const long step = (long)gridDim.x * np;
    long p = (long)blockIdx.x * np + tp;
    for (; p + 3 * step < P; p += 4 * step) {
      uint4 r[4];
#pragma unroll
      for (int u = 0; u < 4; u++) r[u] = *(const uint4*)(x + ((long)g * P + p + u * step) * ldx + c0);
#pragma unroll
      for (int u = 0; u < 4; u++) {
        Vec16<T> t = as_vec<T>(r[u]);
        Vec16<T> o;
#pragma unroll
        for (int j = 0; j < V; j++) o.v[j] = from_f32<T>(apply_act(to_f32(t.v[j]) * sc[j] + sh[j], act));
        *(uint4*)(y + ((long)g * P + p + u * step) * ldy + c0) = as_u4(o);
      }
    }
    for (; p < P; p += step) {
      const long pix = (long)g * P + p;
      Vec16<T> t = as_vec<T>(*(const uint4*)(x + pix * ldx + c0));
      Vec16<T> o;
#pragma unroll
      for (int j = 0; j < V; j++) o.v[j] = from_f32<T>(apply_act(to_f32(t.v[j]) * sc[j] + sh[j], act));
      *(uint4*)(y + pix * ldy + c0) = as_u4(o);
    }
  }
}

template <typename T, int U>
__global__ __launch_bounds__(256) void norm_act_bwd_stats_kernel(const T* __restrict__ x, long ldx, const T* __restrict__ dy,
                                                                 long lddy, const float* __restrict__ mean,
                                                                 const float* __restrict__ rstd, const float* __restrict__ w,
                                                                 const float* __restrict__ b, float* __restrict__ bsums, int G,
                                                                 long P, int C, int act, int STRIP, float* part) {
  constexpr int V = Elem<T>::VEC;
// ... 273 lines not shown
  float a = 0.f, b = 0.f;
  for (int g = 0; g < G; g++) { b += bs[((long)g * C + c) * 2]; a += bs[((long)g * C + c) * 2 + 1]; }
  dw[c] = a; db[c] = b;
}

int grid_for(long total) { long g = (total + 255) / 256; return (int)(g > 8192 ? 8192 : (g < 1 ? 1 : g)); }

template <typename TI, typename TO>
int ln_fwd_dispatch(const void* x, long ldx, const float* w, const float* b, void* y, long ldy, float* m, float* r, long rows,
                    int D, float eps, hipStream_t st) {
  const int nvec = D / Elem<TI>::VEC;
  const int maxv = (nvec + 63) / 64;
  dim3 grid((unsigned)((rows + 3) / 4)), block(256);
  static int wave_slots = 0;
  if (!wave_slots) {
    int dev = 0; hipDeviceProp_t prop;
    wave_slots = (hipGetDevice(&dev) == hipSuccess && hipGetDeviceProperties(&prop, dev) == hipSuccess) ? 32 * prop.multiProcessorCount : 8192;
  }
  if (g_ln_rows2 && maxv <= 4 && (g_ln_rows2 > 1 || (rows > wave_slots && rows <= 2L * wave_slots))) {
    dim3 grid2((unsigned)((rows + 7) / 8));
#define LN2_LAUNCH(MV) hipLaunchKernelGGL((layernorm_fwd2_kernel<TI, TO, MV>), grid2, block, 0, st, (const TI*)x, ldx, w, b, (TO*)y, ldy, m, r, rows, D, eps)
    if (maxv <= 1) LN2_LAUNCH(1); else if (maxv <= 2) LN2_LAUNCH(2); else LN2_LAUNCH(4);
#undef LN2_LAUNCH
    return du_check_launch();
  }
#define LN_LAUNCH(MV) hipLaunchKernelGGL((layernorm_fwd_kernel<TI, TO, MV>), grid, block, 0, st, (const TI*)x, ldx, w, b, (TO*)y, ldy, m, r, rows, D, eps)
  if (maxv <= 1) LN_LAUNCH(1); else if (maxv <= 2) LN_LAUNCH(2); else if (maxv <= 4) LN_LAUNCH(4);
  else if (maxv <= 8) LN_LAUNCH(8); else if (maxv <= 16) LN_LAUNCH(16); else return DU_ERR_UNSUPPORTED;
#undef LN_LAUNCH
  return du_check_launch();
}

template <typename T>
int ln_bwd_dispatch(const void* x, const void* dy, const float* w, const float* mean, const float* rstd, void* dx, float* dwdb,
                    long rows, int D, float* ws, long ws_elems, const void* dres, hipStream_t st) {
  const int nvec = D / Elem<T>::VEC;
  const int maxv = (nvec + 63) / 64;
  dim3 grid((unsigned)((rows + 3) / 4)), block(256);
  {
    static const bool off = DU_GETENV("DU_LN_BWD_FUSED") && atoi(DU_GETENV("DU_LN_BWD_FUSED")) == 0;
    const int STRIP = pick_strip(1, rows, D, Elem<T>::VEC);
    const long strips = (rows + STRIP - 1) / STRIP;
    const size_t lds = (size_t)3 * D * 2 * sizeof(float);
    if (!off && maxv <= 4 && ws && ws_elems >= strips * D * 2 && lds <= 64 * 1024) {
      return strip_launch(dwdb, ws, ws_elems, 1, strips, D, st, [&](float* part) {
#define LNF_LAUNCH(MV) hipLaunchKernelGGL((layernorm_bwd_fused_kernel<T, MV>), dim3((unsigned)strips), block, lds, st, (const T*)x, (const T*)dy, w, mean, rstd, (T*)dx, rows, D, (const T*)dres, STRIP, part)
        if (maxv <= 1) LNF_LAUNCH(1); else if (maxv <= 2) LNF_LAUNCH(2); else LNF_LAUNCH(4);
#undef LNF_LAUNCH
      }, 2);
    }
  }
#define LNB_LAUNCH(MV) hipLaunchKernelGGL((layernorm_bwd_dx_kernel<T, MV>), grid, block, 0, st, (const T*)x, (const T*)dy, w, mean, rstd, (T*)dx, rows, D, (const T*)dres)
  if (maxv <= 1) LNB_LAUNCH(1); else if (maxv <= 2) LNB_LAUNCH(2); else if (maxv <= 4) LNB_LAUNCH(4);
  else if (maxv <= 8) LNB_LAUNCH(8); else if (maxv <= 16) LNB_LAUNCH(16); else return DU_ERR_UNSUPPORTED;
#undef LNB_LAUNCH
  const int STRIP = pick_strip(1, rows, D, Elem<T>::VEC);
  long strips = (rows + STRIP - 1) / STRIP;
  return strip_launch(dwdb, ws, ws_elems, 1, strips, D, st, [&](float* part) {
    hipLaunchKernelGGL(layernorm_bwd_wb_kernel<T>, dim3((unsigned)strips), block, 0, st, (const T*)x, (const T*)dy, mean, rstd, dwdb, rows, D, STRIP, part);
  }, (ws && ws_elems >= (long)strips * D * 2) ? 2 : 0);
}

}

int du_norm_finalize_planar(const float* part, float* out, int strips, int C, hipStream_t st) {
  if ((long)C * 2 >= 4096) hipLaunchKernelGGL(finalize_kernel<32>, dim3((unsigned)((C * 2 + 31) / 32)), dim3(256), 0, st, part, out, 1, strips, C * 2, 2);
  else hipLaunchKernelGGL(finalize_kernel<4>, dim3((unsigned)((C * 2 + 3) / 4)), dim3(256), 0, st, part, out, 1, strips, C * 2, 2);
  return du_check_launch();
}

extern "C" int du_layernorm_fwd(int in_dtype, int out_dtype, const void* x, int64_t ldx, const float* w, const float* b, void* y,
                                int64_t ldy, float* mean_out, float* rstd_out, int64_t rows, int D, float eps, void* stream) {
  hipStream_t st = (hipStream_t)stream;
  if (rows <= 0 || D <= 0 || !x || !y || !w || !b) return DU_ERR_BAD_ARG;
  const int vi = in_dtype == DU_BF16 ? 8 : 4;
  if (D % vi || ldx % vi) return DU_ERR_BAD_ARG;
  if (in_dtype == DU_F32 && out_dtype == DU_F32) return ln_fwd_dispatch<float, float>(x, ldx, w, b, y, ldy, mean_out, rstd_out, rows, D, eps, st);
  if (in_dtype == DU_F32 && out_dtype == DU_BF16) return ln_fwd_dispatch<float, bf16_t>(x, ldx, w, b, y, ldy, mean_out, rstd_out, rows, D, eps, st);
  if (in_dtype == DU_BF16 && out_dtype == DU_BF16) return ln_fwd_dispatch<bf16_t, bf16_t>(x, ldx, w, b, y, ldy, mean_out, rstd_out, rows, D, eps, st);
  if (in_dtype == DU_BF16 && out_dtype == DU_F32) return ln_fwd_dispatch<bf16_t, float>(x, ldx, w, b, y, ldy, mean_out, rstd_out, rows, D, eps, st);
  return DU_ERR_BAD_ARG;
}

extern "C" int du_strip_finalize(const float* part, float* out, int G, int strips, int C, void* stream) {
  hipStream_t st = (hipStream_t)stream;
  if (!part || !out || G <= 0 || strips <= 0 || C <= 0) return DU_ERR_BAD_ARG;
  if ((long)G * C * 2 >= 4096) {
    const int chunks = (C * 2 + 31) / 32;
    hipLaunchKernelGGL(finalize_kernel<32>, dim3((unsigned)(G * chunks)), dim3(256), 0, st, part, out, G, strips, C * 2, 0);
  } else {
    const int chunks = (C * 2 + 3) / 4;
    hipLaunchKernelGGL(finalize_kernel<4>, dim3((unsigned)(G * chunks)), dim3(256), 0, st, part, out, G, strips, C * 2, 0);
  }
  return du_check_launch();
}

extern "C" int64_t du_reduce_ws_elems(int dtype, int G, int64_t P, int C) {
  const int v = dtype == DU_BF16 ? 8 : 4;
  if (G <= 0 || P <= 0 || C <= 0 || C % v) return 0;
  const int STRIP = pick_strip(G, P, C, v);
  return (int64_t)G * ((P + STRIP - 1) / STRIP) * C * 2;
}

extern "C" int du_layernorm_bwd(int dtype, const void* x, const void* dy, const float* w, const float* mean, const float* rstd,
                                void* dx, float* dwdb, int64_t rows, int D, float* ws, int64_t ws_elems, const void* dres, void* stream) {
  hipStream_t st = (hipStream_t)stream;
  if (rows <= 0 || D <= 0 || !x || !dy || !dx || !dwdb) return DU_ERR_BAD_ARG;
  const int vi = dtype == DU_BF16 ? 8 : 4;
  if (D % vi) return DU_ERR_BAD_ARG;
  if (dtype == DU_F32) return ln_bwd_dispatch<float>(x, dy, w, mean, rstd, dx, dwdb, rows, D, ws, ws_elems, dres, st);
  if (dtype == DU_BF16) return ln_bwd_dispatch<bf16_t>(x, dy, w, mean, rstd, dx, dwdb, rows, D, ws, ws_elems, dres, st);
  return DU_ERR_BAD_ARG;
}

extern "C" int du_chan_stats(int dtype, const void* x, int64_t ldx, float* sums, int G, int64_t P, int C, float* ws, int64_t ws_elems,
                             void* stream) {
  hipStream_t st = (hipStream_t)stream;
  const int v = dtype == DU_BF16 ? 8 : 4;
  if (G <= 0 || P <= 0 || C <= 0 || C % v || ldx % v || !x || !sums) return DU_ERR_BAD_ARG;
  const int STRIP = pick_strip(G, P, C, v);
  long strips = (P + STRIP - 1) / STRIP;
  dim3 grid((unsigned)(G * strips)), block(256);
  if (dtype != DU_BF16 && dtype != DU_F32) return DU_ERR_BAD_ARG;
  return strip_launch(sums, ws, ws_elems, G, strips, C, st, [&](float* part) {
    if (dtype == DU_BF16) hipLaunchKernelGGL(chan_stats_kernel<bf16_t>, grid, block, 0, st, (const bf16_t*)x, ldx, sums, G, P, C, STRIP, part);
    else hipLaunchKernelGGL(chan_stats_kernel<float>, grid, block, 0, st, (const float*)x, ldx, sums, G, P, C, STRIP, part);
  });
}

extern "C" int du_colsum(int dtype, const void* x, int64_t ldx, float* out, int64_t rows, int C, float* ws, int64_t ws_elems, void* stream) {
  hipStream_t st = (hipStream_t)stream;
  const int v = dtype == DU_BF16 ? 8 : 4;
  if (rows <= 0 || C <= 0 || C % v || ldx % v || !x || !out || !ws) return DU_ERR_BAD_ARG;
  if (dtype != DU_BF16 && dtype != DU_F32) return DU_ERR_BAD_ARG;
  const int STRIP = pick_strip(1, rows, C, v);
  long strips = (rows + STRIP - 1) / STRIP;
  dim3 grid((unsigned)strips), block(256);
  return strip_launch(out, ws, ws_elems, 1, strips, C, st, [&](float* part) {
    if (dtype == DU_BF16) hipLaunchKernelGGL(chan_stats_kernel<bf16_t>, grid, block, 0, st, (const bf16_t*)x, ldx, out, 1, (long)rows, C, STRIP, part);
    else hipLaunchKernelGGL(chan_stats_kernel<float>, grid, block, 0, st, (const float*)x, ldx, out, 1, (long)rows, C, STRIP, part);
  }, 1);
}

extern "C" int du_chan_dot(int dtype, const void* a, int64_t lda, const void* b, int64_t ldb, float* sums, int G, int64_t P, int C,
                           float* ws, int64_t ws_elems, void* stream) {
  hipStream_t st = (hipStream_t)stream;
  const int v = dtype == DU_BF16 ? 8 : 4;
  if (G <= 0 || P <= 0 || C <= 0 || C % v || lda % v || ldb % v || !a || !b || !sums) return DU_ERR_BAD_ARG;
  const int STRIP = pick_strip(G, P, C, v);
  long strips = (P + STRIP - 1) / STRIP;
  dim3 grid((unsigned)(G * strips)), block(256);
  if (dtype != DU_BF16 && dtype != DU_F32) return DU_ERR_BAD_ARG;
  return strip_launch(sums, ws, ws_elems, G, strips, C, st, [&](float* part) {
    if (dtype == DU_BF16) hipLaunchKernelGGL(chan_dot_kernel<bf16_t>, grid, block, 0, st, (const bf16_t*)a, lda, (const bf16_t*)b, ldb, sums, G, P, C, STRIP, part);
    else hipLaunchKernelGGL(chan_dot_kernel<float>, grid, block, 0, st, (const float*)a, lda, (const float*)b, ldb, sums, G, P, C, STRIP, part);
  });
}

extern "C" int du_norm_stats_finalize(const float* sums, float count, float eps, float* mean, float* rstd, int G, int C, float* run_mean,
                                      float* run_var, float momentum, void* stream) {
  hipStream_t st = (hipStream_t)stream;
  if (!sums || !mean || !rstd || G <= 0 || C <= 0 || count <= 0.f || (run_mean && G != 1) || (!run_mean != !run_var)) return DU_ERR_BAD_ARG;
  const long n = (long)G * C;
  const float unbias = count > 1.f ? count / (count - 1.f) : 1.f;
  hipLaunchKernelGGL(norm_stats_finalize_kernel, dim3((unsigned)((n + 255) / 256)), dim3(256), 0, st, sums, 1.f / count, eps, mean, rstd, n,
                     run_mean, run_var, momentum, unbias);
// ... 117 lines not shown
```

### dinounet_amd/dinov3/adapter.py

```python
import math
from functools import partial

import torch
from torch import nn

from .. import ops
from .._lib import ACT_GELU, ACT_NONE, ACT_RELU


def _act_dtype(module):
    return getattr(module, "_act_dtype", torch.bfloat16)


class MSDeformAttn(nn.Module):

    def __init__(self, d_model=256, n_levels=4, n_heads=8, n_points=4, ratio=1.0):
        super().__init__()
        if d_model % n_heads != 0:
            raise ValueError("d_model must be divisible by n_heads, but got {} and {}".format(d_model, n_heads))
        self.im2col_step = 64
        self.d_model, self.n_levels, self.n_heads, self.n_points, self.ratio = d_model, n_levels, n_heads, n_points, ratio
        self.sampling_offsets = nn.Linear(d_model, n_heads * n_levels * n_points * 2)
        self.attention_weights = nn.Linear(d_model, n_heads * n_levels * n_points)
        self.value_proj = nn.Linear(d_model, int(d_model * ratio))
        self.output_proj = nn.Linear(int(d_model * ratio), d_model)
        self._reset_parameters()

    def _reset_parameters(self):
        nn.init.constant_(self.sampling_offsets.weight.data, 0.0)
        thetas = torch.arange(self.n_heads, dtype=torch.float32) * (2.0 * math.pi / self.n_heads)
        grid_init = torch.stack([thetas.cos(), thetas.sin()], -1)
        grid_init = (grid_init / grid_init.abs().max(-1, keepdim=True)[0]).view(self.n_heads, 1, 1, 2).repeat(
            1, self.n_levels, self.n_points, 1)
        for i in range(self.n_points):
            grid_init[:, :, i, :] *= i + 1
        with torch.no_grad():
            self.sampling_offsets.bias = nn.Parameter(grid_init.view(-1))
        nn.init.constant_(self.attention_weights.weight.data, 0.0)
        nn.init.constant_(self.attention_weights.bias.data, 0.0)
        nn.init.xavier_uniform_(self.value_proj.weight.data)
        nn.init.constant_(self.value_proj.bias.data, 0.0)
        nn.init.xavier_uniform_(self.output_proj.weight.data)
        nn.init.constant_(self.output_proj.bias.data, 0.0)

    def forward(self, query, reference_points, input_flatten, input_spatial_shapes, input_level_start_index,
                input_padding_mask=None, residual=None, query_norm=None):
        assert input_padding_mask is None and self.n_levels == 1 and len(input_spatial_shapes) == 1
        N, Lq, _ = query.shape
        _, S, _ = input_flatten.shape
        Hs, Ws = input_spatial_shapes[0]
        assert Hs * Ws == S
        M, P = self.n_heads, self.n_points
        value = ops.linear(input_flatten, self.value_proj.weight, self.value_proj.bias)
        value = value.view(N, S, M, value.shape[-1] // M)
        if query_norm is not None:
            loc, attn, residual = ops.layer_norm_offsets_prep(query, query_norm.weight, query_norm.bias, query_norm.eps,
                                                              self.sampling_offsets.weight, self.attention_weights.weight,
                                                              self.sampling_offsets.bias, self.attention_weights.bias, reference_points,
                                                              Lq, M, P, Hs, Ws)
        else:
            loc, attn = ops.offsets_prep(query, self.sampling_offsets.weight, self.attention_weights.weight, self.sampling_offsets.bias,
                                         self.attention_weights.bias, reference_points, Lq, M, P, Hs, Ws)
        shapes, lsi = _level_tensors(Hs, Ws, query.device)
        out = ops.msda(value, shapes, lsi, loc.view(N, Lq, M, 1, P, 2), attn.view(N, Lq, M, 1, P))
        return ops.linear(out, self.output_proj.weight, self.output_proj.bias, residual=residual)


_LEVEL_CACHE = {}


def _level_tensors(Hs, Ws, device):
    key = (Hs, Ws, str(device))
    if key not in _LEVEL_CACHE:
        _LEVEL_CACHE[key] = (torch.tensor([[Hs, Ws]], dtype=torch.long, device=device),
                             torch.zeros(1, dtype=torch.long, device=device))
    return _LEVEL_CACHE[key]


class DWConv(nn.Module):
    def __init__(self, dim=768):
        super().__init__()
        self.dwconv = nn.Conv2d(dim, dim, 3, 1, 1, bias=True, groups=dim)


class ConvFFN(nn.Module):

    def __init__(self, in_features, hidden_features=None, out_features=None, drop=0.0):
        super().__init__()
        out_features = out_features or in_features
        hidden_features = hidden_features or in_features
        self.fc1 = nn.Linear(in_features, hidden_features)
        self.dwconv = DWConv(hidden_features)
        self.act = nn.GELU()
        self.fc2 = nn.Linear(hidden_features, out_features)
        self.drop = nn.Dropout(drop)

    def forward(self, x, H, W, residual=None, row_scale=None, norm=None):
        if norm is not None:
            h, residual = ops.layer_norm_linear(x, norm.weight, norm.bias, norm.eps, self.fc1.weight, self.fc1.bias)
        else:
            h = ops.linear(x, self.fc1.weight, self.fc1.bias)
        h = ops.dwconv_tokens(h, self.dwconv.dwconv.weight, self.dwconv.dwconv.bias, H, W, ACT_GELU)
        return ops.linear(h, self.fc2.weight, self.fc2.bias, residual=residual, row_scale=row_scale, rs_rows=x.shape[1])


class DropPath(nn.Module):
    def __init__(self, drop_prob=0.0):
        super().__init__()
        self.drop_prob = drop_prob
        self.pinned_mask = None
        self.predrawn = None

    def mask(self, B, device):
        if self.drop_prob == 0.0 or not self.training:
            return None
        if self.pinned_mask is not None:
            return self.pinned_mask.to(device=device, dtype=torch.float32)
        if self.predrawn is not None and self.predrawn.shape[0] == B:
            m, self.predrawn = self.predrawn, None
            return m
        keep = 1 - self.drop_prob
        m = torch.empty(B, device=device, dtype=torch.float32).bernoulli_(keep)
        if keep > 0.0:
            m.div_(keep)
        return m


class Extractor(nn.Module):

    def __init__(self, dim, num_heads=6, n_points=4, n_levels=1, deform_ratio=1.0, with_cffn=True, cffn_ratio=0.25, drop=0.0,
                 drop_path=0.0, norm_layer=partial(nn.LayerNorm, eps=1e-6), with_cp=False):
        super().__init__()
        self.query_norm = norm_layer(dim)
        self.feat_norm = norm_layer(dim)
        self.attn = MSDeformAttn(d_model=dim, n_levels=n_levels, n_heads=num_heads, n_points=n_points, ratio=deform_ratio)
        self.with_cffn = with_cffn
        self.with_cp = with_cp
        if with_cffn:
            self.ffn = ConvFFN(in_features=dim, hidden_features=int(dim * cffn_ratio), drop=drop)
            self.ffn_norm = norm_layer(dim)
            self.drop_path = DropPath(drop_path) if drop_path > 0.0 else nn.Identity()

    def forward(self, query, reference_points, feat, spatial_shapes, level_start_index, H, W):
        fn = ops.layer_norm(feat, self.feat_norm.weight, self.feat_norm.bias, self.feat_norm.eps)
        query = self.attn(query, reference_points, fn, spatial_shapes, level_start_index, None, query_norm=self.query_norm)
        if self.with_cffn:
            mask = self.drop_path.mask(query.shape[0], query.device) if isinstance(self.drop_path, DropPath) else None
            query = self.ffn(query, H, W, row_scale=mask, norm=self.ffn_norm)
        return query


class InteractionBlockWithCls(nn.Module):

    def __init__(self, dim, num_heads=6, n_points=4, norm_layer=partial(nn.LayerNorm, eps=1e-6), drop=0.0, drop_path=0.0,
                 with_cffn=True, cffn_ratio=0.25, init_values=0.0, deform_ratio=1.0, extra_extractor=False, with_cp=False):
        super().__init__()
        mk = lambda: Extractor(dim=dim, n_levels=1, num_heads=num_heads, n_points=n_points, norm_layer=norm_layer,
                               deform_ratio=deform_ratio, with_cffn=with_cffn, cffn_ratio=cffn_ratio, drop=drop,
                               drop_path=drop_path, with_cp=with_cp)
        self.extractor = mk()
        self.extra_extractors = nn.Sequential(*[mk() for _ in range(2)]) if extra_extractor else None

    def forward(self, x, c, ref, shapes, H_c, W_c):
        c = self.extractor(c, ref, x, shapes, None, H_c, W_c)
        if self.extra_extractors is not None:
            for ex in self.extra_extractors:
                c = ex(c, ref, x, shapes, None, H_c, W_c)
        return c


class SpatialPriorModule(nn.Module):

    def __init__(self, inplanes=64, embed_dim=384, with_cp=False):
        super().__init__()
        bn = nn.SyncBatchNorm
        self.stem = nn.Sequential(
            nn.Conv2d(3, inplanes, kernel_size=3, stride=2, padding=1, bias=False), bn(inplanes), nn.ReLU(inplace=True),
            nn.Conv2d(inplanes, inplanes, kernel_size=3, stride=1, padding=1, bias=False), bn(inplanes), nn.ReLU(inplace=True),
            nn.Conv2d(inplanes, inplanes, kernel_size=3, stride=1, padding=1, bias=False), bn(inplanes), nn.ReLU(inplace=True),
            nn.MaxPool2d(kernel_size=3, stride=2, padding=1))
        self.conv2 = nn.Sequential(nn.Conv2d(inplanes, 2 * inplanes, 3, 2, 1, bias=False), bn(2 * inplanes), nn.ReLU(inplace=True))
        self.conv3 = nn.Sequential(nn.Conv2d(2 * inplanes, 4 * inplanes, 3, 2, 1, bias=False), bn(4 * inplanes), nn.ReLU(inplace=True))
        self.conv4 = nn.Sequential(nn.Conv2d(4 * inplanes, 4 * inplanes, 3, 2, 1, bias=False), bn(4 * inplanes), nn.ReLU(inplace=True))
        self.fc1 = nn.Conv2d(inplanes, embed_dim, kernel_size=1)
        self.fc2 = nn.Conv2d(2 * inplanes, embed_dim, kernel_size=1)
        self.fc3 = nn.Conv2d(4 * inplanes, embed_dim, kernel_size=1)
        self.fc4 = nn.Conv2d(4 * inplanes, embed_dim, kernel_size=1)

    def _cbr(self, x, conv, bn, stride, group):
        w = conv.weight
        if w.shape[1] % 8:
            w = torch.nn.functional.pad(w, (0, 0, 0, 0, 0, 8 - w.shape[1] % 8))
        y, st = ops.conv2d_stats(x, w, None, stride=stride, pad=1)
        return bn_act(y, bn, ACT_RELU, self.training, group, st)

    def forward(self, x8, level_embed, group=None):
        c = self._cbr(x8, self.stem[0], self.stem[1], 2, group)
        c = self._cbr(c, self.stem[3], self.stem[4], 1, group)
        c = self._cbr(c, self.stem[6], self.stem[7], 1, group)
        c1 = ops.maxpool3x3s2(c)
        c2 = self._cbr(c1, self.conv2[0], self.conv2[1], 2, group)
        c3 = self._cbr(c2, self.conv3[0], self.conv3[1], 2, group)
        c4 = self._cbr(c3, self.conv4[0], self.conv4[1], 2, group)
        c1 = ops.conv1x1(c1, self.fc1.weight, self.fc1.bias)
        c2 = ops.conv1x1(c2, self.fc2.weight, self.fc2.bias + level_embed[0])
        c3 = ops.conv1x1(c3, self.fc3.weight, self.fc3.bias + level_embed[1])
        c4 = ops.conv1x1(c4, self.fc4.weight, self.fc4.bias + level_embed[2])
        tok = lambda t: t.view(t.shape[0], -1, t.shape[-1])
        return c1, tok(c2), tok(c3), tok(c4)


_TICK_STACK = []


def _tick(bn):
    if _TICK_STACK:
        _TICK_STACK[-1].append(bn.num_batches_tracked)
    else:
        bn.num_batches_tracked += 1


class _collect_ticks:

    def __enter__(self):
        _TICK_STACK.append([])
        return self

    def __exit__(self, *exc):
        ticks = _TICK_STACK.pop()
        if ticks:
            torch._foreach_add_(ticks, 1)
        return False


def bn_act(x, bn, act, training, group, stats_part=None):
    if training and bn.track_running_stats and bn.num_batches_tracked is not None:
        _tick(bn)
    return ops.norm_act(x, bn.weight, bn.bias, "bn", act, bn.eps, training, bn.running_mean, bn.running_var,
                        bn.momentum if bn.momentum is not None else 0.1, group, stats_part=stats_part if training else None)


def get_reference_points(spatial_shapes, device):
    refs = []
    for (H_, W_) in spatial_shapes:
        ry, rx = torch.meshgrid(torch.linspace(0.5, H_ - 0.5, H_, dtype=torch.float32),
                                torch.linspace(0.5, W_ - 0.5, W_, dtype=torch.float32), indexing="ij")
        refs.append(torch.stack((rx.reshape(-1) / W_, ry.reshape(-1) / H_), -1))
    return torch.cat(refs, 0).to(device).contiguous()


class DINOv3_Adapter(nn.Module):

    def __init__(self, backbone, interaction_indexes=[9, 19, 29, 39], pretrain_size=512, conv_inplane=64, n_points=4,
                 deform_num_heads=16, drop_path_rate=0.3, init_values=0.0, with_cffn=True, cffn_ratio=0.25, deform_ratio=0.5,
                 add_vit_feature=True, use_extra_extractor=True, with_cp=True):
        super().__init__()
        self.backbone = backbone
        self.backbone.requires_grad_(False)
        self.pretrain_size = (pretrain_size, pretrain_size)
        self.interaction_indexes = interaction_indexes
        self.add_vit_feature = add_vit_feature
        embed_dim = self.backbone.embed_dim
        self.patch_size = self.backbone.patch_size
        self.level_embed = nn.Parameter(torch.zeros(3, embed_dim))
        self.spm = SpatialPriorModule(inplanes=conv_inplane, embed_dim=embed_dim, with_cp=False)
        self.interactions = nn.Sequential(*[
            InteractionBlockWithCls(dim=embed_dim, num_heads=deform_num_heads, n_points=n_points, init_values=init_values,
                                    drop_path=drop_path_rate, norm_layer=partial(nn.LayerNorm, eps=1e-6), with_cffn=with_cffn,
                                    cffn_ratio=cffn_ratio, deform_ratio=deform_ratio,
                                    extra_extractor=((i == len(interaction_indexes) - 1) and use_extra_extractor), with_cp=with_cp)
            for i in range(len(interaction_indexes))])
        self.up = nn.ConvTranspose2d(embed_dim, embed_dim, 2, 2)
        self.norm1 = nn.SyncBatchNorm(embed_dim)
        self.norm2 = nn.SyncBatchNorm(embed_dim)
        self.norm3 = nn.SyncBatchNorm(embed_dim)
        self.norm4 = nn.SyncBatchNorm(embed_dim)
        self.up.apply(self._init_weights)
        self.spm.apply(self._init_weights)
        self.interactions.apply(self._init_weights)
        self.apply(self._init_deform_weights)
        torch.nn.init.normal_(self.level_embed)
        self._ref_cache = {}

    def _init_weights(self, m):
        if isinstance(m, nn.Linear):
            torch.nn.init.trunc_normal_(m.weight, std=0.02)
            if m.bias is not None:
                nn.init.constant_(m.bias, 0)
        elif isinstance(m, (nn.LayerNorm, nn.BatchNorm2d)):
            nn.init.constant_(m.bias, 0)
            nn.init.constant_(m.weight, 1.0)
        elif isinstance(m, (nn.Conv2d, nn.ConvTranspose2d)):
            fan_out = m.kernel_size[0] * m.kernel_size[1] * m.out_channels
            fan_out //= m.groups
            m.weight.data.normal_(0, math.sqrt(2.0 / fan_out))
            if m.bias is not None:
                m.bias.data.zero_()

    def _init_deform_weights(self, m):
        if isinstance(m, MSDeformAttn):
            m._reset_parameters()

    def forward(self, x, layers=None):
        with _collect_ticks():
            return self._forward(x, layers)

    def backbone_layers(self, x):
        return self.backbone.get_intermediate_layers(x, n=self.interaction_indexes, return_class_token=True, dtype=_act_dtype(self))

    def _forward(self, x, layers=None):
        dt = _act_dtype(self)
        B, _, H, W = x.shape
        D = self.backbone.embed_dim
        H_c, W_c = H // 16, W // 16
        H_t, W_t = H // self.patch_size, W // self.patch_size
        group = torch.distributed.group.WORLD if (torch.distributed.is_available() and torch.distributed.is_initialized()) else None
        key = (H, W, str(x.device))
        if key not in self._ref_cache:
            self._ref_cache = {key: get_reference_points([(H // 8, W // 8), (H // 16, W // 16), (H // 32, W // 32)], x.device)}
        ref = self._ref_cache[key]
        shapes = [(H_t, W_t)]

        if self.training:
            dps = [m for m in self.modules() if isinstance(m, DropPath) and m.drop_prob > 0.0 and m.pinned_mask is None]
            keeps = {1 - m.drop_prob for m in dps}
            if len(dps) > 1 and len(keeps) == 1:
                keep = keeps.pop()
                tbl = torch.empty((len(dps), x.shape[0]), device=x.device, dtype=torch.float32).bernoulli_(keep)
                if keep > 0.0:
                    tbl.div_(keep)
                for i, m in enumerate(dps):
                    m.predrawn = tbl[i]
        chained = layers is None and getattr(self.backbone, "chains", 1) > 1
        if chained:
            vit = self.backbone.begin_intermediate_layers(x, n=self.interaction_indexes, return_class_token=True, dtype=dt)
            if not getattr(self.backbone, "overlap_prior", True):
                vit_out = vit()
                vit = lambda: vit_out
        x8 = ops.nchw_to_nhwc(x, dt, 8)
        c1, c2, c3, c4 = self.spm(x8, self.level_embed, group)
        n2, n3 = c2.shape[1], c3.shape[1]
        c = torch.cat([c2, c3, c4], dim=1)

        if chained:
            layers = vit()
        elif layers is None:
            layers = self.backbone.get_intermediate_layers(x, n=self.interaction_indexes, return_class_token=True, dtype=dt)

        for i, layer in enumerate(self.interactions):
            xi, _cls = layers[i]
            c = layer(xi, c, ref, shapes, H_c, W_c)

        c2, c3, c4 = c.split([n2, n3, c.shape[1] - n2 - n3], dim=1)
        c2 = c2.contiguous().view(B, H_c * 2, W_c * 2, D)
        c3 = c3.contiguous().view(B, H_c, W_c, D)
        c4 = c4.contiguous().view(B, H_c // 2, W_c // 2, D)
        c1 = ops.conv_transpose2x2(c2, self.up.weight, self.up.bias, residual=c1)
        cs = [c1, c2, c3, c4]
        if self.add_vit_feature:
            cs = [ops.bilinear_add(layers[j][0].view(B, H_t, W_t, D), cs[j]) for j in range(4)]
        norms = [self.norm1, self.norm2, self.norm3, self.norm4]
        if (self.training and group is not None and ops.sync_active(group)
                and all(bn.track_running_stats for bn in norms)):
            for bn in norms:
                if bn.num_batches_tracked is not None:
                    _tick(bn)
            fs = ops.sync_bn_multi(cs, norms, ACT_NONE, group)
        else:
            fs = [bn_act(cs[j], norms[j], ACT_NONE, self.training, group) for j in range(4)]
        return {"1": fs[0], "2": fs[1], "3": fs[2], "4": fs[3]}
```

### dinounet_amd/ops.py

```python
import ctypes as C
import math
import os
import weakref

import torch

from . import _lib
from ._lib import (ACT_GELU, ACT_LEAKY, ACT_NONE, ACT_RELU, ACT_SWIGLU, DU_BF16, DU_F32, IM2COL_COL, IM2COL_ROW, PLAIN_COL,
                   PLAIN_ROW, STORE_MSDA_PREP, STORE_PIXEL_SHUFFLE2, STORE_QKV_HEADS, STORE_QKV_ROPE, STORE_SLABS, ConvGeom, GemmArgs)

__all__ = ["mm", "linear", "conv2d", "conv_transpose2x2", "norm_act", "layer_norm", "msda", "dwconv3x3",
           "maxpool3x3s2", "bilinear_add", "bilinear_resize", "squeeze_excite", "dice_ce_loss", "dice_ce_masked_loss", "dice_bce_loss",
           "labels_to_regions", "val_dice_ce", "val_dice_bce", "ds_seg_loss", "downsample_seg"]


def _code(dt):
    if dt == torch.bfloat16:
        return DU_BF16
    if dt == torch.float32:
        return DU_F32
    raise RuntimeError(f"dinounet_amd: unsupported dtype {dt} (bf16 / fp32 only)")


def _req(*ts):
# ... 1500 lines not shown
            wsb, nws = _reduce_ws(x.dtype, 1, B * H * W, Cc, dev)
            bsj = C.c_void_p(flat.data_ptr() + 4 * offs[j])
            _lib.check(L.du_norm_act_bwd_stats(_code(x.dtype), _p(x), ld, _p(dy), Cc, _p(mean), _p(rstd), _p(wf), _p(bf), bsj, 1, B * H * W,
                                               Cc, act, _p(wsb), nws, _st()), "du_norm_act_bwd_stats")
            dw = torch.empty(Cc, dtype=torch.float32, device=dev)
            db = torch.empty(Cc, dtype=torch.float32, device=dev)
            _lib.check(L.du_norm_param_grads(bsj, _p(dw), _p(db), 1, Cc, _st()), "du_norm_param_grads")
            dws.append(dw); dbs.append(db)
        _small_all_reduce(flat, group, "syncbn_bwd")
        dxs = []
        for j in range(n):
            x, mean, rstd, wf, bf = sv[5 * j:5 * j + 5]
            B, H, W, Cc, ld = geo[j]
            dx = torch.empty((B, H, W, Cc), dtype=x.dtype, device=dev)
            _lib.check(L.du_norm_act_bwd_dx(_code(x.dtype), _p(x), ld, _p(dyc[j]), Cc, _p(dx), Cc, _p(mean), _p(rstd), _p(wf), _p(bf),
                                            C.c_void_p(flat.data_ptr() + 4 * offs[j]), 1, B * H * W, Cc, act, float(B * H * W * world), 1, _st()),
                       "du_norm_act_bwd_dx")
            dxs.append(dx)
        return (None, None, None, *dxs, *dws, *dbs, None)


def sync_bn_multi(xs, bns, act, group):
    n = len(xs)
    mods = [(bn.eps, bn.running_mean, bn.running_var, bn.momentum if bn.momentum is not None else 0.1) for bn in bns]
    return list(_SyncBNMulti.apply(group, act, n, *xs, *[bn.weight for bn in bns], *[bn.bias for bn in bns], mods))


def layernorm_raw(x2d, w, b, eps, out_dtype, want_stats=False, out=None):
    rows, D, ld = _rows2d(x2d)
    if out is None:
        y = torch.empty((rows, D), dtype=out_dtype, device=x2d.device)
    else:
        y = out
        assert y.shape == (rows, D) and y.dtype == out_dtype and y.is_contiguous()
    mean = rstd = None
    if want_stats:
        mean = torch.empty(rows, dtype=torch.float32, device=x2d.device)
        rstd = torch.empty(rows, dtype=torch.float32, device=x2d.device)
    _lib.check(_lib.lib().du_layernorm_fwd(_code(x2d.dtype), _code(out_dtype), _p(x2d), ld, _p(w), _p(b), _p(y), D, _p(mean),
                                           _p(rstd), rows, D, eps, _st()), "du_layernorm_fwd")
    return y, mean, rstd


class _LayerNorm(torch.autograd.Function):

    @staticmethod
    def forward(ctx, x, w, b, eps, with_res):
        xc = x.contiguous()
        wf, bf = _f32(w), _f32(b)
        y, mean, rstd = layernorm_raw(xc.view(-1, xc.shape[-1]), wf, bf, eps, xc.dtype, True)
        ctx.save_for_backward(xc, wf, mean, rstd)
        ctx.with_res = with_res
        ctx.set_materialize_grads(False)
        if with_res:
            return y.view(x.shape), xc.view(x.shape).view_as(xc)
        return y.view(x.shape)

    @staticmethod
    def backward(ctx, dy, dres=None):
        xc, wf, mean, rstd = ctx.saved_tensors
        D = xc.shape[-1]
        if dy is None:
            return dres, None, None, None, None
        dyc = dy.contiguous()
        dx = torch.empty_like(xc)
        dwdb = torch.empty((2, D), dtype=torch.float32, device=xc.device)
        ws, n = _reduce_ws(xc.dtype, 1, xc.numel() // D, D, xc.device)
        dr = None
        if dres is not None:
            dr = dres.contiguous()
            if dr.dtype != xc.dtype:
                dr = cast(dr, xc.dtype)
        _lib.check(_lib.lib().du_layernorm_bwd(_code(xc.dtype), _p(xc), _p(dyc), _p(wf), _p(mean), _p(rstd), _p(dx), _p(dwdb),
                                               xc.numel() // D, D, _p(ws), n, _p(dr), _st()), "du_layernorm_bwd")
        return dx, dwdb[0], dwdb[1], None, None


def layer_norm(x, w, b, eps):
    return _LayerNorm.apply(x, w, b, eps, False)


def layer_norm_res(x, w, b, eps):
    return _LayerNorm.apply(x, w, b, eps, True)


def msda_forward_raw(value, shapes, lsi, loc, attn):
    _req(value, shapes, lsi, loc, attn)
    N, S, M, D = value.shape
    _, Lq, _, L, P, _ = loc.shape
    out = torch.empty((N, Lq, M * D), dtype=value.dtype, device=value.device)
    e0 = PROFILE.start() if PROFILE is not None else None
    _lib.check(_lib.lib().du_msda_forward(_code(value.dtype), _p(value), _p(shapes), _p(lsi), _p(loc), _p(attn), _p(out), N, S, M, D,
                                          L, Lq, P, _st()), "du_msda_forward")
    if PROFILE is not None:
        PROFILE.stop("msda_fwd<gather>", e0, 8.0 * N * Lq * M * L * P * D,
                     float(value.numel() * value.element_size() + loc.numel() * 4 + attn.numel() * 4 + out.numel() * out.element_size()))
    return out


def msda_backward_raw(value, shapes, lsi, loc, attn, grad_out, gv_like_value=False):
    _req(value, shapes, lsi, loc, attn, grad_out)
    N, S, M, D = value.shape
    _, Lq, _, L, P, _ = loc.shape
    gl = torch.empty(loc.shape, dtype=torch.float32, device=value.device)
    ga = torch.empty(attn.shape, dtype=torch.float32, device=value.device)
    n = int(_lib.lib().du_msda_bwd_ws_elems(N, S, M, D, L, Lq, P))
    ws = torch.empty(max(n, 1), dtype=torch.float32, device=value.device)
    e0 = PROFILE.start() if PROFILE is not None else None

    def _prof(gv):
        if PROFILE is not None:
            PROFILE.stop("msda_bwd<gather>", e0, 24.0 * N * Lq * M * L * P * D,
                         float(value.numel() * value.element_size() + loc.numel() * 8 + attn.numel() * 8
                               + grad_out.numel() * grad_out.element_size() + gv.numel() * gv.element_size()))
    if gv_like_value and value.dtype == torch.bfloat16:
        gvb = torch.empty((N, S, M, D), dtype=torch.bfloat16, device=value.device)
        rc = _lib.lib().du_msda_backward_bf16gv(_p(value), _p(shapes), _p(lsi), _p(loc), _p(attn), _p(grad_out), _p(gvb), _p(gl), _p(ga),
                                                N, S, M, D, L, Lq, P, _p(ws), n, _st())
        if rc == 0:
            _prof(gvb)
            return gvb, gl, ga
        if rc != -2:
            _lib.check(rc, "du_msda_backward_bf16gv")
    gv = torch.empty((N, S, M, D), dtype=torch.float32, device=value.device)
    _lib.check(_lib.lib().du_msda_backward(_code(value.dtype), _p(value), _p(shapes), _p(lsi), _p(loc), _p(attn), _p(grad_out), _p(gv),
                                           _p(gl), _p(ga), N, S, M, D, L, Lq, P, _p(ws), n, _st()), "du_msda_backward")
    _prof(gv)
    return gv, gl, ga


class _MSDA(torch.autograd.Function):

    @staticmethod
    def forward(ctx, value, shapes, lsi, loc, attn):
        value, loc, attn = value.contiguous(), loc.contiguous(), attn.contiguous()
        out = msda_forward_raw(value, shapes, lsi, loc, attn)
        ctx.save_for_backward(value, shapes, lsi, loc, attn)
        return out

    @staticmethod
    def backward(ctx, go):
        value, shapes, lsi, loc, attn = ctx.saved_tensors
        gv, gl, ga = msda_backward_raw(value, shapes, lsi, loc, attn, go.contiguous(), gv_like_value=True)
        return (gv if gv.dtype == value.dtype else gv.to(value.dtype)), None, None, gl, ga


def msda(value, shapes, lsi, loc, attn):
    return _MSDA.apply(value, shapes, lsi, loc, attn)


class _MSDAPrep(torch.autograd.Function):

    @staticmethod
    def forward(ctx, raw, ref, Lq, M, P, Hs, Ws):
        rows, ncol, ld = _rows2d(raw)
        assert ncol == M * P * 3
        loc = torch.empty((rows, M, P, 2), dtype=torch.float32, device=raw.device)
        attn = torch.empty((rows, M, P), dtype=torch.float32, device=raw.device)
        _lib.check(_lib.lib().du_msda_prep(_code(raw.dtype), _p(raw), ld, _p(ref), _p(loc), _p(attn), rows, Lq, M, P, Hs, Ws, _st()),
                   "du_msda_prep")
        ctx.save_for_backward(attn)
        ctx.conf = (M, P, Hs, Ws, raw.dtype, ncol)
        return loc, attn

    @staticmethod
    def backward(ctx, gloc, gattn):
# ... 907 lines not shown
```

### include/dinounet_hip.h

```cpp
#ifndef DINOUNET_HIP_H
#define DINOUNET_HIP_H

#include <stdint.h>

#ifdef __cplusplus
extern "C" {
#endif

#define DU_OK 0
#define DU_ERR_BAD_ARG (-1)
#define DU_ERR_UNSUPPORTED (-2)
#define DU_ERR_LAUNCH (-3)

#define DU_F32 0
#define DU_BF16 1

#define DU_PLAIN_ROW 0
#define DU_PLAIN_COL 1
#define DU_IM2COL_ROW 2
#define DU_IM2COL_COL 3

#define DU_ACT_NONE 0
#define DU_ACT_GELU 1
#define DU_ACT_RELU 2
#define DU_ACT_LEAKY 3
#define DU_ACT_SWIGLU 4

#define DU_STORE_PLAIN 0
#define DU_STORE_SLABS 4
#define DU_STORE_QKV_HEADS 5
#define DU_STORE_MSDA_PREP 6
#define DU_STORE_TAPS 3
#define DU_STORE_QKV_ROPE 2
#define DU_STORE_PIXEL_SHUFFLE2 1

typedef struct {
  const void* p2;
  int64_t ld2;
  int32_t C1;
  int32_t Hi, Wi;
  int32_t C;
  int32_t KH, KW, stride, pad;
  int32_t Ho, Wo;
  int32_t transposed;
} du_conv_geom;

typedef struct {
  int32_t dtype;
  int32_t out_dtype;
  int32_t a_mode, b_mode;
  int32_t M, N, K;
  const void* A; int64_t lda; int64_t a_batch_stride;
  const void* B; int64_t ldb; int64_t b_batch_stride;
  void* C; int64_t ldc; int64_t c_batch_stride;
  int32_t batch;
  int32_t split_k;
  float alpha;
  const float* bias;
  int32_t act;
  const float* gamma;
  const float* row_scale; int32_t rs_rows;
  const void* residual; int64_t ldr;
  int32_t store_mode;
  int32_t ps_H, ps_W, ps_C;
  du_conv_geom geom;
  float* ws; int64_t ws_elems;
  const float* rope_sin; const float* rope_cos; int32_t rope_prefix; float rope_qscale;
  float* a_colsum;
  float* b_colsum;
  float* C2;
  void* ks_ws;
  int64_t ks_ws_bytes;
} du_gemm_args;

int du_gemm(const du_gemm_args* args, void* stream);
int64_t du_gemm_ws_elems(const du_gemm_args* args);
int64_t du_gemm_ks_ws_bytes(const du_gemm_args* args);
int du_gemm_route(const du_gemm_args* args);
int du_gemm_plan_describe(const du_gemm_args* args, int64_t* out, int n);

typedef struct du_tn_job {
  const void* A; int64_t lda;
  const void* B; int64_t ldb;
  float* C; int64_t ldc;
  float* a_colsum;
  const float* alpha;
  int32_t M, N, K;
  int32_t accumulate;
  float* b_colsum;
  int32_t gather, Hs, Ws, Cb, taps, inner, inner_total, c_off;
} du_tn_job;
int du_gemm_tn_group_legal(const du_tn_job* job);
int du_gemm_tn_group(const du_tn_job* jobs, int njobs, void* stream);

int du_conv3x3_halo(const void* x, int64_t ldx, const void* x2, int64_t ldx2, int C1, int Cin, int Cout, int B, int H, int W,
                    const void* w, const float* bias, void* y, int64_t ldy, float* stats_part, void* stream);
int du_conv3x3_plan_describe(const void* x, int64_t ldx, const void* x2, int64_t ldx2, int C1, int Cin, int Cout, int B, int H, int W,
                             const void* w, const void* y, int64_t ldy, int want_stats, int64_t* out, int n);
int du_conv3x3_halo_parts(int C1, int Cin, int Cout, int B, int H, int W);
int du_conv3x3_strip(const void* x, int64_t ldx, const void* x2, int64_t ldx2, int C1, int Cin, int Cout, int B, int H, int W,
                     const void* w, const float* bias, void* y, int64_t ldy, float* stats_part, void* stream);
int du_conv3x3_wgrad_halo(const void* x, int64_t ldx, const void* x2, int64_t ldx2, int C1, int Cin, int Cout, int B, int H, int W,
                          const void* dy, int64_t lddy, float* part, float* dw, int with_db, void* stream);
int du_conv3x3_wgrad_plan_describe(const void* x, int64_t ldx, const void* x2, int64_t ldx2, int C1, int Cin, int Cout, int B, int H, int W,
                                   const void* dy, int64_t lddy, int64_t* out, int n);
int du_conv3x3_wgrad_halo_blocks(int C1, int Cin, int Cout, int B, int H, int W);
int du_strip_finalize(const float* part, float* out, int G, int strips, int C, void* stream);

int du_qkv_rope_split(int dtype, const void* qkv, void* q, void* k, void* v, const float* sin_t, const float* cos_t,
                      int B, int N, int Npad, int H, int Dh, int prefix, float qscale, void* stream);
int du_qkv_rope_split_rows(int dtype, const void* qkv_rows, void* q, void* k, void* v, const float* sin_t, const float* cos_t, int B, int N,
                           int Npad, int H, int Dh, int prefix, float qscale, int64_t m_begin, int m_count, void* stream);
int du_qkv_rope_inplace(int dtype, void* q, void* k, const float* sin_t, const float* cos_t, int B, int N, int Npad, int H, int Dh,
                        int prefix, float qscale, int64_t m_limit, void* stream);
int du_attention_fwd(const void* q, const void* k, const void* v, void* out, int B, int H, int N, int Npad, int Dh,
                     void* stream);
int du_softmax_rows_f32(float* x, int64_t rows, int cols, int64_t ld, void* stream);

int du_layernorm_fwd(int in_dtype, int out_dtype, const void* x, int64_t ldx, const float* w, const float* b, void* y,
                     int64_t ldy, float* mean_out, float* rstd_out, int64_t rows, int D, float eps, void* stream);
int64_t du_reduce_ws_elems(int dtype, int G, int64_t pix_per_group, int C);
int du_layernorm_bwd(int dtype, const void* x, const void* dy, const float* w, const float* mean, const float* rstd,
                     void* dx, float* dwdb, int64_t rows, int D, float* ws, int64_t ws_elems, const void* dres, void* stream);
int du_layernorm_bwd_prod_plan(int dtype, const void* x, const void* G, int64_t ldg, const void* Wt, int64_t ldw, int K, const void* dx,
                               const void* dres, int64_t rows, int D, int64_t* out, int n);
int du_layernorm_bwd_prod(int dtype, const void* x, const void* G, int64_t ldg, const void* Wt, int64_t ldw, int K, const float* w,
                          const float* mean, const float* rstd, void* dx, float* dwdb, int64_t rows, int D, float* ws, int64_t ws_elems,
                          const void* dres, void* stream);

int du_chan_stats(int dtype, const void* x, int64_t ldx, float* sums, int G, int64_t pix_per_group, int C, float* ws,
                  int64_t ws_elems, void* stream);
int du_colsum(int dtype, const void* x, int64_t ldx, float* out, int64_t rows, int C, float* ws, int64_t ws_elems, void* stream);
int du_chan_dot(int dtype, const void* a, int64_t lda, const void* b, int64_t ldb, float* sums, int G, int64_t pix_per_group, int C,
                float* ws, int64_t ws_elems, void* stream);
int du_norm_stats_finalize(const float* sums, float count, float eps, float* mean, float* rstd, int G, int C, float* run_mean,
                           float* run_var, float momentum, void* stream);
int du_norm_param_grads(const float* bsums, float* dw, float* db, int G, int C, void* stream);
int du_chan_stats_norm(int dtype, const void* x, int64_t ldx, float* sums, int G, int64_t pix_per_group, int C, float* ws, int64_t ws_elems,
                       float count, float eps, float* mean, float* rstd, float* run_mean, float* run_var, float momentum, void* stream);
int du_strip_finalize_norm(const float* part, float* sums, int G, int strips, int C, float count, float eps, float* mean, float* rstd,
                           float* run_mean, float* run_var, float momentum, void* stream);
int du_norm_act_bwd_stats_grads(int dtype, const void* x, int64_t ldx, const void* dy, int64_t lddy, const float* mean, const float* rstd,
                                const float* w, const float* b, float* bsums, float* dw, float* db, int G, int64_t pix_per_group, int C,
                                int act, float* ws, int64_t ws_elems, void* stream);
int du_norm_act_fwd(int dtype, const void* x, int64_t ldx, void* y, int64_t ldy, const float* mean, const float* rstd,
                    const float* w, const float* b, int G, int64_t pix_per_group, int C, int act, void* stream);
int du_norm_act_bwd_stats(int dtype, const void* x, int64_t ldx, const void* dy, int64_t lddy, const float* mean,
                          const float* rstd, const float* w, const float* b, float* bsums, int G, int64_t pix_per_group,
                          int C, int act, float* ws, int64_t ws_elems, void* stream);
int du_norm_act_bwd_dx(int dtype, const void* x, int64_t ldx, const void* dy, int64_t lddy, void* dx, int64_t lddx,
                       const float* mean, const float* rstd, const float* w, const float* b, const float* bsums, int G,
                       int64_t pix_per_group, int C, int act, float count, int use_batch_stats, void* stream);

int du_msda_forward(int dtype, const void* value, const int64_t* spatial_shapes, const int64_t* level_start_index,
                    const float* sampling_loc, const float* attn_weight, void* out, int N, int S, int M, int D, int L,
                    int Lq, int P, void* stream);
int64_t du_msda_bwd_ws_elems(int N, int S, int M, int D, int L, int Lq, int P);
int du_msda_backward(int dtype, const void* value, const int64_t* spatial_shapes, const int64_t* level_start_index,
                     const float* sampling_loc, const float* attn_weight, const void* grad_out, float* grad_value,
                     float* grad_sampling_loc, float* grad_attn_weight, int N, int S, int M, int D, int L, int Lq, int P,
                     float* ws, int64_t ws_elems, void* stream);

int du_msda_forward_f64(const double* value, const int64_t* spatial_shapes, const int64_t* level_start_index, const double* sampling_loc,
                        const double* attn_weight, double* out, int N, int S, int M, int D, int L, int Lq, int P, void* stream);
int du_msda_backward_f64(const double* value, const int64_t* spatial_shapes, const int64_t* level_start_index, const double* sampling_loc,
                         const double* attn_weight, const double* grad_out, double* grad_value, double* grad_sampling_loc,
                         double* grad_attn_weight, int N, int S, int M, int D, int L, int Lq, int P, void* stream);

int du_msda_backward_bf16gv(const void* value, const int64_t* spatial_shapes, const int64_t* level_start_index, const float* sampling_loc,
                            const float* attn_weight, const void* grad_out, void* grad_value_bf16, float* grad_sampling_loc,
                            float* grad_attn_weight, int N, int S, int M, int D, int L, int Lq, int P, float* ws, int64_t ws_elems,
                            void* stream);

int du_msda_prep(int dtype, const void* raw, int64_t ldr, const float* ref, float* loc, float* attn, int64_t rows, int Lq,
                 int M, int P, int Hs, int Ws, void* stream);
int du_msda_prep_bwd(int dtype, const float* attn, const float* gloc, const float* gattn, void* graw, int64_t ldr,
                     int64_t rows, int M, int P, int Hs, int Ws, void* stream);

int du_dwconv3x3_fwd(int dtype, const void* x, const float* w, const float* bias, void* y, void* z, int64_t ld, int64_t bs, int B, int H,
                     int W, int C, int pyramid, int act, void* stream);
int64_t du_dwconv3x3_bwd_ws_elems(int dtype, int64_t ld, int64_t bs, int B, int H, int W, int C, int pyramid, int act);
int du_dwconv3x3_bwd(int dtype, const void* z, const void* dy, const void* x, const float* w, void* dx, float* dw, float* db, void* dz,
                     int64_t ld, int64_t bs, int B, int H, int W, int C, int pyramid, int act, float* ws, int64_t ws_elems, void* stream);
int du_dwconv3x3_plan_describe(int dtype, int64_t ld, int64_t bs, int B, int H, int W, int C, int pyramid, int act, int64_t* out, int n);
int du_maxpool3x3s2_fwd(int dtype, const void* x, void* y, uint8_t* idx, int B, int H, int W, int C, void* stream);
int du_maxpool3x3s2_bwd(int dtype, const uint8_t* idx, const void* dy, void* dx, int B, int H, int W, int C, void* stream);
int du_bilinear_add_fwd(int src_dtype, int dtype, const void* src, int64_t lds_, const void* base, int64_t ldb, void* out,
                        int64_t ldo, int B, int Hs, int Ws, int Ho, int Wo, int C, void* stream);
int du_bilinear_resize_bwd(int dtype, const void* dy, int64_t lddy, void* dx, int64_t lddx, int B, int Hs, int Ws, int Ho, int Wo,
                           int C, void* stream);
int du_act_bwd(int dtype, const void* z, const void* dy, void* dz, int64_t n, int act, void* stream);

int du_se_gate_fwd(const float* sums, float inv_count, const float* W1, const float* b1, const float* W2, const float* b2,
                   float* hidden, float* gate, int B, int C, int R, void* stream);
int du_se_scale_fwd(int dtype, const void* x, int64_t ldx, const float* gate, const void* shortcut, int64_t ldsc, void* y, int64_t ldy,
                    int B, int64_t P, int C, void* stream);
int du_se_gate_bwd(const float* dsum, const float* sums, float inv_count, const float* gate, const float* hidden, const float* W1,
                   const float* W2, float* dpool, float* dW1, float* db1, float* dW2, float* db2, int B, int C, int R, void* stream);
int du_se_scale_bwd(int dtype, const void* dy, int64_t lddy, const float* gate, const float* dpool, void* dx, int64_t lddx, int B,
                    int64_t P, int C, void* stream);

int64_t du_dice_ce_ws_elems(int B, int K, int64_t HW);
int du_dice_ce_sums(const float* logits, const int64_t* target, float* sums, int B, int K, int64_t HW, float* ws, int64_t ws_elems,
                    void* stream);
int du_dice_ce_finish(const float* sums, float* loss, float* coef, int K, int64_t npix, float smooth, float grad_mult, void* stream);
int du_dice_ce_bwd(const float* logits, const int64_t* target, const float* coef, const float* grad_out, float* dlogits, int B, int K,
// ... 166 lines not shown
```

Before: 320.9 slices/s.

## Batch per-level feature LayerNorm+linear into grouped multi-job GEMM and LN kernels

Adds a grouped GEMM path that walks tiles of up to eight same-shape jobs in one persistent kernel launch, plus grouped LayerNorm forward and parameter-gradient kernels driven by job tables. A new autograd function runs the adapter's per-tap LayerNorm+linear value projections, and their backward, through these grouped launches instead of one launch per tap. The aim is to cut launch overhead and the tail underutilisation of several small GEMMs. In exchange, per-tile job lookup adds buffer-descriptor rebuilds inside the hot loop, and eligibility is limited to plain-epilogue, equal-shape cases.

```diff
diff --git a/dinounet_amd/_lib.py b/dinounet_amd/_lib.py
--- a/dinounet_amd/_lib.py
+++ b/dinounet_amd/_lib.py
@@ -41,6 +41,19 @@
                 ("accumulate", C.c_int32), ("b_colsum", C.c_void_p),
                 ("gather", C.c_int32), ("Hs", C.c_int32), ("Ws", C.c_int32), ("Cb", C.c_int32),
                 ("taps", C.c_int32), ("inner", C.c_int32), ("inner_total", C.c_int32), ("c_off", C.c_int32)]
+
+
+GEMM_JOBS_MAX = LN_JOBS_MAX = 8
+
+
+class GemmJob(C.Structure):
+    _fields_ = [("A", C.c_void_p), ("lda", C.c_int64), ("B", C.c_void_p), ("ldb", C.c_int64), ("C", C.c_void_p), ("ldc", C.c_int64),
+                ("bias", C.c_void_p), ("M", C.c_int32), ("N", C.c_int32), ("K", C.c_int32), ("reserved", C.c_int32)]
+
+
+class LnJob(C.Structure):
+    _fields_ = [("x", C.c_void_p), ("ldx", C.c_int64), ("w", C.c_void_p), ("b", C.c_void_p), ("y", C.c_void_p), ("ldy", C.c_int64),
+                ("mean", C.c_void_p), ("rstd", C.c_void_p), ("rows", C.c_int64), ("dy", C.c_void_p)]
 
 
 _CTYPE = {"int": C.c_int, "int64_t": C.c_int64, "float": C.c_float, "int32_t": C.c_int32, "double": C.c_double}
diff --git a/dinounet_amd/csrc/gemm.hip b/dinounet_amd/csrc/gemm.hip
--- a/dinounet_amd/csrc/gemm.hip
+++ b/dinounet_amd/csrc/gemm.hip
@@ -426,6 +426,61 @@
   return 9;
 }
 
+du_gemm_args du_gemm_job_args(const du_gemm_args& shape, const du_gemm_job& job) {
+  du_gemm_args a = shape;
+  a.A = job.A; a.lda = job.lda; a.B = job.B; a.ldb = job.ldb; a.C = job.C; a.ldc = job.ldc; a.bias = job.bias;
+  a.M = job.M; a.N = job.N; a.K = job.K;
+  return a;
+}
+
+GemmJobsPlan du_gemm_jobs_plan(const du_gemm_args& shape, const du_gemm_job* jobs, int njobs) {
+  GemmJobsPlan p{};
+  if (!jobs || njobs < 1) { p.rc = DU_ERR_BAD_ARG; return p; }
+  for (int j = 0; j < njobs; j++) {
+    const GemmPlan one = du_gemm_plan(du_gemm_job_args(shape, jobs[j]));
+    if (j == 0) { p.family = one.family; p.variant = one.variant; }
+    if (one.rc != DU_OK) { p.rc = one.rc; return p; }
+  }
+  static const bool generic_only = DU_GETENV("DU_GEMM_GENERIC") != nullptr;
+  if (generic_only || njobs > DU_GEMM_JOBS_MAX || shape.batch > 1 || shape.gamma || shape.ws || shape.ks_ws) return p;
+  for (int j = 0; j < njobs; j++) {
+    if (jobs[j].M != jobs[0].M || jobs[j].N != jobs[0].N || jobs[j].K != jobs[0].K) return p;
+    if (!du_gemm_pp_jobs_legal(du_gemm_job_args(shape, jobs[j]))) return p;
+  }
+  du_gemm_args all = du_gemm_job_args(shape, jobs[0]);
+  if ((long)all.M * njobs > 0x7fffffffL) return p;
+  all.M *= njobs;
+  if (du_gemm_p8_choice(all) != 4) return p;
+  p.grouped = 1; p.family = 6; p.variant = 4;
+  p.tiles = (long)njobs * (jobs[0].M / 256) * ((jobs[0].N + 127) / 128);
+  return p;
+}
+
+extern "C" int du_gemm_jobs_plan_describe(const du_gemm_args* shape, const du_gemm_job* jobs, int njobs, int64_t* out, int n) {
+  if (!shape || !out || n < 6) return DU_ERR_BAD_ARG;
+  const GemmJobsPlan p = du_gemm_jobs_plan(*shape, jobs, njobs);
+  const int64_t v[6] = {p.rc, p.grouped, p.family, p.variant, p.tiles, njobs};
+  for (int i = 0; i < 6; i++) out[i] = v[i];
+  return 6;
+}
+
+extern "C" int du_gemm_jobs(const du_gemm_args* shape, const du_gemm_job* jobs, int njobs, void* stream) {
+  if (!shape) return DU_ERR_BAD_ARG;
+  const GemmJobsPlan p = du_gemm_jobs_plan(*shape, jobs, njobs);
+  if (p.rc != DU_OK) return p.rc;
+  if (p.grouped) {
+    du_gemm_args each[DU_GEMM_JOBS_MAX];
+    for (int j = 0; j < njobs; j++) each[j] = du_gemm_job_args(*shape, jobs[j]);
+    return du_gemm_nt_pp_jobs(each, njobs, (hipStream_t)stream);
+  }
+  for (int j = 0; j < njobs; j++) {
+    const du_gemm_args a = du_gemm_job_args(*shape, jobs[j]);
+    const int rc = du_gemm(&a, stream);
+    if (rc != DU_OK) return rc;
+  }
+  return DU_OK;
+}
+
 extern "C" int du_gemm(const du_gemm_args* pa, void* stream) {
   if (!pa) return DU_ERR_BAD_ARG;
   const GemmPlan p = du_gemm_plan(*pa);
diff --git a/dinounet_amd/csrc/gemm_p8.hip b/dinounet_amd/csrc/gemm_p8.hip
--- a/dinounet_amd/csrc/gemm_p8.hip
+++ b/dinounet_amd/csrc/gemm_p8.hip
@@ -1459,13 +1459,17 @@
   asm volatile("s_waitcnt lgkmcnt(0)" : "+v"(a), "+v"(b), "+v"(c), "+v"(d) : : "memory");
 }
 
-template <int ACT, bool NK4, int RES = 0, bool PS = false, int QKV = 0>
-__global__ __launch_bounds__(512) void gemm_nt_pp_kernel(GemmParams P) {
+struct PpJob { const void* A; const void* W; const float* bias; void* C; int lda, ldb, ldc, pad_; };
+struct PpJobTable { int njobs, pad_; PpJob job[DU_GEMM_JOBS_MAX]; };
+
+template <int ACT, bool NK4, int RES, bool PS, int QKV, bool JOBS>
+__device__ __forceinline__ void pp_tile_walk(const GemmParams& P, const PpJobTable* T) {
   constexpr bool ROPE = QKV == 1, HEADS = QKV == 2;
   extern __shared__ __attribute__((aligned(16))) unsigned char smem[];
   if (P.tail_rows && (int)blockIdx.x >= P.main_wgs) { p8_tail<bf16_t>(P, smem); return; }
   static_assert(RES == 0 || ACT == DU_ACT_NONE, "the residual form has no activation");
   static_assert(QKV == 0 || (ACT == DU_ACT_NONE && !NK4 && RES == 0 && !PS), "the qkv stores: plain bias epilogue, K >= 384");
+  static_assert(!JOBS || (ACT == DU_ACT_NONE && !NK4 && RES == 0 && !PS && QKV == 0), "the job table: plain bias epilogue, K >= 384");
   constexpr bool FOUR = NK4 && RES == 0;
   const int tid = threadIdx.x, lane = tid & 63, hi = lane >> 5;
   const int wave = __builtin_amdgcn_readfirstlane(tid >> 6);
@@ -1476,8 +1480,14 @@
     const int bid = blockIdx.x, q = G >> 3, r = G & 7, xcd = bid & 7, idx = bid >> 3;
     lin = (xcd < r ? xcd * (q + 1) : r * (q + 1) + (xcd - r) * q) + idx;
   }
-  const int ntiles = P.tiles_m * P.tiles_n;
+  const int tpj = P.tiles_m * P.tiles_n;
+  const int ntiles = JOBS ? tpj * T->njobs : tpj;
   const int nk = P.K / PBK + (RES ? 2 : 0);
+  auto job_of = [&](int& tile) -> int {
+    const int j = __builtin_amdgcn_readfirstlane(tile / tpj);
+    tile -= j * tpj;
+    return j;
+  };
   auto coords = [&](int tile, int& m0, int& n0) {
     int tm, tn;
     if (P.group_m > 1) {
@@ -1492,17 +1502,19 @@
     m0 = tm * PBM; n0 = tn * NBN;
   };
 
-  const auto ra = __builtin_amdgcn_make_buffer_rsrc((void*)P.a.p, 0, (int)((((long)P.M - 1) * P.a.ld + P.K) * 2), 0x00020000);
-  const auto rb = __builtin_amdgcn_make_buffer_rsrc((void*)P.b.p, 0, (int)((((long)P.N - 1) * P.b.ld + P.K) * 2), 0x00020000);
+  auto ra = __builtin_amdgcn_make_buffer_rsrc((void*)P.a.p, 0, (int)((((long)P.M - 1) * P.a.ld + P.K) * 2), 0x00020000);
+  auto rb = __builtin_amdgcn_make_buffer_rsrc((void*)P.b.p, 0, (int)((((long)P.N - 1) * P.b.ld + P.K) * 2), 0x00020000);
   const long out_rows = PS ? 4L * P.M : (long)P.M;
   const int out_cols = PS ? P.ps_C : P.N;
-  const auto rc = __builtin_amdgcn_make_buffer_rsrc(P.C, 0, QKV ? (int)(3 * P.ldc * 2) : (int)(((out_rows - 1) * P.ldc + out_cols) * 2), 0x00020000);
+  auto rc = __builtin_amdgcn_make_buffer_rsrc(P.C, 0, QKV ? (int)(3 * P.ldc * 2) : (int)(((out_rows - 1) * P.ldc + out_cols) * 2), 0x00020000);
   const int ps_lw = PS ? __builtin_ctz(P.ps_W) : 0, ps_lh = PS ? __builtin_ctz(P.ps_H) : 0;
   auto ps_pixel = [&](unsigned m) -> unsigned {
     const unsigned x = m & (unsigned)(P.ps_W - 1), y = (m >> ps_lw) & (unsigned)(P.ps_H - 1), b = m >> (ps_lw + ps_lh);
     return ((b * 2u * (unsigned)P.ps_H + 2u * y) * 2u * (unsigned)P.ps_W) + 2u * x;
   };
-  const auto rbias = __builtin_amdgcn_make_buffer_rsrc(P.bias ? (void*)P.bias : P.C, 0, P.bias ? P.N * 4 : 0, 0x00020000);
+  auto rbias = __builtin_amdgcn_make_buffer_rsrc(P.bias ? (void*)P.bias : P.C, 0, P.bias ? P.N * 4 : 0, 0x00020000);
+  unsigned lda2 = (unsigned)(P.a.ld * 2), ldb2 = (unsigned)(P.b.ld * 2);
+  long ldc_prev = P.ldc;
   const int nrec_r = RES ? (int)(((out_rows - 1) * P.ldr + out_cols) * 2) : 0;
   const unsigned ldr2 = (unsigned)(P.ldr * 2);
 
@@ -1524,19 +1536,30 @@
   auto set_stage_tile = [&](int tile, int slot) {
     if (tile < ntiles) {
       int m0, n0;
+      if constexpr (JOBS) {
+        const PpJob& jb = T->job[job_of(tile)];
+        lda2 = (unsigned)jb.lda * 2u; ldb2 = (unsigned)jb.ldb * 2u;
+        ra = __builtin_amdgcn_make_buffer_rsrc((void*)jb.A, 0, (int)((((long)P.M - 1) * jb.lda + P.K) * 2), 0x00020000);
+        rb = __builtin_amdgcn_make_buffer_rsrc((void*)jb.W, 0, (int)((((long)P.N - 1) * jb.ldb + P.K) * 2), 0x00020000);
+        rbias = __builtin_amdgcn_make_buffer_rsrc(jb.bias ? (void*)jb.bias : jb.C, 0, jb.bias ? P.N * 4 : 0, 0x00020000);
+      }
       coords(tile, m0, n0);
 #pragma unroll
       for (int r = 0; r < 2; r++) {
         if constexpr (ROPE) {
           sm0 = (unsigned)m0; sn0 = (unsigned)n0;
+        } else if constexpr (JOBS) {
+          va_s[0][r] = m0 + srow[r] < P.M ? (unsigned)srow[r] * lda2 + lc * 16 : PP_OOR;
+          va_s[1][r] = m0 + 128 + srow[r] < P.M ? (unsigned)(128 + srow[r]) * lda2 + lc * 16 : PP_OOR;
+          vb_s[r] = n0 + srow[r] < P.N ? (unsigned)srow[r] * ldb2 + lc * 16 : PP_OOR;
         } else {
           va_s[0][r] = m0 + srow[r] < P.M ? va0[0][r] : PP_OOR;
           va_s[1][r] = m0 + 128 + srow[r] < P.M ? va0[1][r] : PP_OOR;
           vb_s[r] = n0 + srow[r] < P.N ? vb0[r] : PP_OOR;
         }
       }
-      sa_base = (unsigned)m0 * (unsigned)(P.a.ld * 2);
-      sb_base = (unsigned)n0 * (unsigned)(P.b.ld * 2);
+      sa_base = (unsigned)m0 * (JOBS ? lda2 : (unsigned)(P.a.ld * 2));
+      sb_base = (unsigned)n0 * (JOBS ? ldb2 : (unsigned)(P.b.ld * 2));
       if constexpr (RES != 0 && !PS) sr_base = (unsigned)m0 * ldr2 + (unsigned)n0 * 2u;
       if constexpr (RES != 0 && PS) {
         const int q = n0 / P.ps_C, co0 = n0 - q * P.ps_C;
@@ -1657,6 +1680,11 @@
   const unsigned rope_tbl = lds_base + PP_ROPE_OFF + (unsigned)(4 * hi * 4);
   auto set_prev_tile = [&](int tile) {
     int m0, n0;
+    if constexpr (JOBS) {
+      const PpJob& jb = T->job[job_of(tile)];
+      ldc_prev = jb.ldc;
+      rc = __builtin_amdgcn_make_buffer_rsrc(jb.C, 0, (int)((((long)P.M - 1) * jb.ldc + P.N) * 2), 0x00020000);
+    }
     coords(tile, m0, n0);
     pcol = n0 + wn * 64 + hi * 8;
     if constexpr (QKV != 0) {
@@ -1682,7 +1710,7 @@
         const unsigned pix = ps_pixel((unsigned)m) + (unsigned)((q >> 1) * 2 * P.ps_W + (q & 1));
         crow[i] = m < P.M ? (unsigned)(((long)pix * P.ldc + co0 + wn * 64 + hi * 8) * 2) : PP_OOR;
       } else {
-        crow[i] = m < P.M ? (unsigned)(((long)m * P.ldc + pcol) * 2) : PP_OOR;
+        crow[i] = m < P.M ? (unsigned)(((long)m * (JOBS ? ldc_prev : P.ldc) + pcol) * 2) : PP_OOR;
       }
     }
   };
@@ -1917,6 +1945,14 @@
   if (P.tail_rows && (int)gridDim.x == G) p8_tail_inline<bf16_t>(P, smem, lin, G);
 }
 
+template <int ACT, bool NK4, int RES = 0, bool PS = false, int QKV = 0>
+__global__ __launch_bounds__(512) void gemm_nt_pp_kernel(GemmParams P) {
+  pp_tile_walk<ACT, NK4, RES, PS, QKV, false>(P, nullptr);
+}
+__global__ __launch_bounds__(512) void gemm_nt_pp_jobs_kernel(GemmParams P, PpJobTable T) {
+  pp_tile_walk<DU_ACT_NONE, false, 0, false, 0, true>(P, &T);
+}
+
 int g_p8_mode = -1;
 int g_p8_sched = 1;
 int g_p8_corun = 1;
@@ -2003,6 +2039,31 @@
     attr_set[ai] = true;
   }
   hipLaunchKernelGGL(kfn, grid, dim3(512), lds_bytes, st, P);
+  return du_check_launch();
+}
+
+int launch_pp_jobs(const du_gemm_args* jobs, int n, hipStream_t st) {
+  if (n < 1 || n > DU_GEMM_JOBS_MAX) return DU_ERR_BAD_ARG;
+  const du_gemm_args& a = jobs[0];
+  GemmParams P = make_params(a, DU_PLAIN_ROW, DU_PLAIN_ROW, PBM, NBN, PBK);
+  P.tiles_m = (a.M + PBM - 1) / PBM;
+  P.group_m = g_p8_group;
+  P.dbg = g_p8_debug;
+  PpJobTable T{};
+  T.njobs = n;
+  for (int j = 0; j < n; j++) {
+    T.job[j].A = jobs[j].A; T.job[j].W = jobs[j].B; T.job[j].bias = jobs[j].bias; T.job[j].C = jobs[j].C;
+    T.job[j].lda = (int)jobs[j].lda; T.job[j].ldb = (int)jobs[j].ldb; T.job[j].ldc = (int)jobs[j].ldc;
+  }
+  const long ntiles = (long)n * P.tiles_m * P.tiles_n;
+  const long cus = g_p8_pp_full ? 256 : 256 / g_p8_corun;
+  P.main_wgs = (int)(ntiles < cus ? ntiles : cus);
+  static bool attr_set = false;
+  if (!attr_set) {
+    if (hipFuncSetAttribute((const void*)gemm_nt_pp_jobs_kernel, hipFuncAttributeMaxDynamicSharedMemorySize, PP_LDS) != hipSuccess) return DU_ERR_LAUNCH;
+    attr_set = true;
+  }
+  hipLaunchKernelGGL(gemm_nt_pp_jobs_kernel, dim3(P.main_wgs, 1), dim3(512), PP_LDS, st, P, T);
   return du_check_launch();
 }
 
@@ -2242,6 +2303,13 @@
   return g_p8_sched ? launch_p8<float, 1, true>(a, st, tr) : launch_p8<float, 0, true>(a, st, tr);
 }
 
+bool du_gemm_pp_jobs_legal(const du_gemm_args& a) {
+  if (!pp_legal(a) || a.store_mode != DU_STORE_PLAIN || a.act != DU_ACT_NONE || a.residual || a.row_scale) return false;
+  if (a.K < 384 || a.M % PBM) return false;
+  return a.lda <= 0x7fffffffL && a.ldb <= 0x7fffffffL && a.ldc <= 0x7fffffffL;
+}
+int du_gemm_nt_pp_jobs(const du_gemm_args* jobs, int n, hipStream_t st) { return launch_pp_jobs(jobs, n, st); }
+
 bool du_gemm_p8_tail_ok(const du_gemm_args& whole, int r) {
   static const bool off = DU_GETENV("DU_P8_NO_TAIL") != nullptr;
   static const int kmax = DU_GETENV("DU_SKINNY_FUSE_KMAX") ? atoi(DU_GETENV("DU_SKINNY_FUSE_KMAX")) : 4096;
diff --git a/dinounet_amd/csrc/gemm_plan.h b/dinounet_amd/csrc/gemm_plan.h
--- a/dinounet_amd/csrc/gemm_plan.h
+++ b/dinounet_amd/csrc/gemm_plan.h
@@ -17,6 +17,15 @@
 
 GemmPlan du_gemm_plan(const du_gemm_args& a);
 
+struct GemmJobsPlan {
+  int rc;
+  int grouped;
+  int family, variant;
+  long tiles;
+};
+GemmJobsPlan du_gemm_jobs_plan(const du_gemm_args& shape, const du_gemm_job* jobs, int njobs);
+du_gemm_args du_gemm_job_args(const du_gemm_args& shape, const du_gemm_job& job);
+
 bool du_gemm_modes_served(int a_mode, int b_mode);
 int du_gemm_bf16_tiles(const du_gemm_args& a, hipStream_t st);
 int du_gemm_ragged_rows(const du_gemm_args& a);
@@ -30,6 +39,8 @@
 long du_gemm_p8_ks_bytes(const du_gemm_args& a);
 long du_gemm_p8_tail_bytes(const du_gemm_args& whole);
 int du_gemm_nt_p8(const du_gemm_args& a, hipStream_t st, int choice, int tail_rows);
+bool du_gemm_pp_jobs_legal(const du_gemm_args& one);
+int du_gemm_nt_pp_jobs(const du_gemm_args* jobs, int n, hipStream_t st);
 int du_gemm_tn_p8_splits(const du_gemm_args& a);
 int du_gemm_tn_p8(const du_gemm_args& a, hipStream_t st, int splits);
 int du_gemm_skinny_form(const du_gemm_args& a);
diff --git a/dinounet_amd/csrc/norm.hip b/dinounet_amd/csrc/norm.hip
--- a/dinounet_amd/csrc/norm.hip
+++ b/dinounet_amd/csrc/norm.hip
@@ -54,6 +54,71 @@
     }
   }
 }
+
+struct LnJobTable {
+  int njobs, pad_;
+  int wg_end[DU_LN_JOBS_MAX];
+  du_ln_job job[DU_LN_JOBS_MAX];
+};
+template <typename TI, typename TO, int MAXV>
+__global__ __launch_bounds__(256) void layernorm_fwd_jobs_kernel(LnJobTable T, int D, float eps) {
+  int jn = 0, first = 0;
+  while (jn + 1 < T.njobs && (int)blockIdx.x >= T.wg_end[jn]) { first = T.wg_end[jn]; jn++; }
+  const du_ln_job& jb = T.job[jn];
+  const TI* __restrict__ x = (const TI*)jb.x;
+  const long ldx = jb.ldx;
+  const float* __restrict__ w = jb.w;
+  const float* __restrict__ b = jb.b;
+  TO* __restrict__ y = (TO*)jb.y;
+  const long ldy = jb.ldy;
+  float* __restrict__ mean_out = jb.mean;
+  float* __restrict__ rstd_out = jb.rstd;
+  const long rows = jb.rows;
+  constexpr int VI = Elem<TI>::VEC;
+  const int lane = threadIdx.x & 63;
+  const long row = (long)((int)blockIdx.x - first) * 4 + (threadIdx.x >> 6);
+  if (row >= rows) return;
+  const int nvec = D / VI;
+  float v[MAXV][VI];
+  float s = 0.f;
+#pragma unroll
+  for (int i = 0; i < MAXV; i++) {
+    int vi = lane + i * 64;
+    if (vi < nvec) {
+      Vec16<TI> t = as_vec<TI>(*(const uint4*)(x + row * ldx + (long)vi * VI));
+#pragma unroll
+      for (int j = 0; j < VI; j++) { v[i][j] = to_f32(t.v[j]); s += v[i][j]; }
+    } else {
+#pragma unroll
+      for (int j = 0; j < VI; j++) v[i][j] = 0.f;
+    }
+  }
+  const float mean = wave_sum(s) / (float)D;
+  float s2 = 0.f;
+#pragma unroll
+  for (int i = 0; i < MAXV; i++) {
+    int vi = lane + i * 64;
+    if (vi < nvec) {
+#pragma unroll
+      for (int j = 0; j < VI; j++) { float d = v[i][j] - mean; s2 += d * d; }
+    }
+  }
+  const float rstd = rsqrtf(wave_sum(s2) / (float)D + eps);
+  if (lane == 0) {
+    if (mean_out) mean_out[row] = mean;
+    if (rstd_out) rstd_out[row] = rstd;
+  }
+#pragma unroll
+  for (int i = 0; i < MAXV; i++) {
+    int vi = lane + i * 64;
+    if (vi < nvec) {
+      const int c0 = vi * VI;
+#pragma unroll
+      for (int j = 0; j < VI; j++) y[row * ldy + c0 + j] = from_f32<TO>((v[i][j] - mean) * rstd * w[c0 + j] + b[c0 + j]);
+    }
+  }
+}
+
 
 template <typename TI, typename TO, int MAXV>
 __global__ __launch_bounds__(256) void layernorm_fwd2_kernel(const TI* __restrict__ x, long ldx, const float* __restrict__ w,
@@ -223,6 +288,92 @@
           else o = ln_bwd_row_dx<T, false>(xh[i], g[i], c1, c2, rs[u], make_uint4(0, 0, 0, 0));
           *(uint4*)(dx + row * (long)D + (long)vi * VI) = o;
         }
+      }
+    }
+  }
+  if (wave > 0) {
+#pragma unroll
+    for (int i = 0; i < MAXV; i++) {
+      const int vi = lane + i * 64;
+      if (vi < nvec) {
+#pragma unroll
+        for (int j = 0; j < VI; j += 2)
+          *(float4*)(ln_red + ((long)(wave - 1) * D + vi * VI + j) * 2) = make_float4(sa[i][j], sb[i][j], sa[i][j + 1], sb[i][j + 1]);
+      }
+    }
+  }
+  __syncthreads();
+  if (wave == 0) {
+#pragma unroll
+    for (int i = 0; i < MAXV; i++) {
+      const int vi = lane + i * 64;
+      if (vi < nvec) {
+#pragma unroll
+        for (int j = 0; j < VI; j += 2) {
+          float4 t = make_float4(sa[i][j], sb[i][j], sa[i][j + 1], sb[i][j + 1]);
+#pragma unroll
+          for (int q = 0; q < 3; q++) {
+            const float4 u = *(const float4*)(ln_red + ((long)q * D + vi * VI + j) * 2);
+            t.x += u.x; t.y += u.y; t.z += u.z; t.w += u.w;
+          }
+          *(float4*)(part + ((long)blockIdx.x * D + vi * VI + j) * 2) = t;
+        }
+      }
+    }
+  }
+}
+
+template <typename T, int MAXV>
+__global__ __launch_bounds__(256) void layernorm_bwd_params_jobs_kernel(LnJobTable J, long rows, int D, int strip, int strips,
+                                                                        float* __restrict__ part) {
+  constexpr int VI = Elem<T>::VEC;
+  extern __shared__ float ln_red[];
+  const int lane = threadIdx.x & 63, wave = threadIdx.x >> 6;
+  const int nvec = D / VI;
+  const int job = blockIdx.x / strips, sidx = blockIdx.x - job * strips;
+  const du_ln_job& jb = J.job[job];
+  const T* __restrict__ x = (const T*)jb.x;
+  const T* __restrict__ dy = (const T*)jb.dy;
+  const float* __restrict__ mean = jb.mean;
+  const float* __restrict__ rstd = jb.rstd;
+  const long ldx = jb.ldx;
+  float wv[VI], sa[MAXV][VI], sb[MAXV][VI];
+#pragma unroll
+  for (int j = 0; j < VI; j++) wv[j] = 0.f;
+#pragma unroll
+  for (int i = 0; i < MAXV; i++)
+#pragma unroll
+    for (int j = 0; j < VI; j++) { sa[i][j] = 0.f; sb[i][j] = 0.f; }
+  const long r0 = (long)sidx * strip;
+  const long r1 = r0 + strip < rows ? r0 + strip : rows;
+  for (long row0 = r0 + wave; row0 < r1; row0 += 8) {
+    uint4 rx[2][MAXV], rg[2][MAXV];
+    float mu[2], rs[2];
+#pragma unroll
+    for (int u = 0; u < 2; u++) {
+      const long row = row0 + 4 * u;
+      const bool live = row < r1;
+      mu[u] = live ? mean[row] : 0.f; rs[u] = live ? rstd[row] : 0.f;
+#pragma unroll
+      for (int i = 0; i < MAXV; i++) {
+        const int vi = lane + i * 64;
+        rx[u][i] = make_uint4(0, 0, 0, 0); rg[u][i] = make_uint4(0, 0, 0, 0);
+        if (live && vi < nvec) {
+          rx[u][i] = *(const uint4*)(x + row * ldx + (long)vi * VI);
+          rg[u][i] = *(const uint4*)(dy + row * (long)D + (long)vi * VI);
+        }
+      }
+    }
+#pragma unroll
+    for (int u = 0; u < 2; u++) {
+      const long row = row0 + 4 * u;
+      if (row >= r1) break;
+      float xh[VI], g[VI];
+      float c1 = 0.f, c2 = 0.f;
+#pragma unroll
+      for (int i = 0; i < MAXV; i++) {
+        const int vi = lane + i * 64;
+        if (vi < nvec) ln_bwd_row_terms<T>(rx[u][i], rg[u][i], mu[u], rs[u], wv, xh, g, c1, c2, sa[i], sb[i]);
       }
     }
   }
@@ -360,6 +511,24 @@
     Vec16<T> tx = as_vec<T>(*(const uint4*)(x + row * (long)D + c0));
     Vec16<T> tg = as_vec<T>(*(const uint4*)(dy + row * (long)D + c0));
     const float mu = mean[row], rs = rstd[row];
+#pragma unroll
+    for (int j = 0; j < V; j++) {
+      float gy = to_f32(tg.v[j]);
+      a[j] += gy * (to_f32(tx.v[j]) - mu) * rs;
+      b[j] += gy;
+    }
+  });
+}
+
+template <typename T>
+__global__ __launch_bounds__(256) void layernorm_bwd_wb_jobs_kernel(LnJobTable J, long rows, int D, int strip, float* part) {
+  constexpr int V = Elem<T>::VEC;
+  strip_reduce<T>(J.njobs, rows, D, strip, nullptr, part, [&](long rowg, int g, int c0, float* a, float* b) {
+    const du_ln_job& jb = J.job[g];
+    const long row = rowg - (long)g * rows;
+    Vec16<T> tx = as_vec<T>(*(const uint4*)((const T*)jb.x + row * jb.ldx + c0));
+    Vec16<T> tg = as_vec<T>(*(const uint4*)((const T*)jb.dy + row * (long)D + c0));
+    const float mu = jb.mean[row], rs = jb.rstd[row];
 #pragma unroll
     for (int j = 0; j < V; j++) {
       float gy = to_f32(tg.v[j]);
@@ -799,6 +968,80 @@
   return DU_ERR_BAD_ARG;
 }
 
+template <typename TI, typename TO>
+int ln_fwd_jobs_dispatch(const LnJobTable& T, int nwg, int D, float eps, hipStream_t st) {
+  const int maxv = (D / Elem<TI>::VEC + 63) / 64;
+  dim3 grid((unsigned)nwg), block(256);
+#define LNJ_LAUNCH(MV) hipLaunchKernelGGL((layernorm_fwd_jobs_kernel<TI, TO, MV>), grid, block, 0, st, T, D, eps)
+  if (maxv <= 1) LNJ_LAUNCH(1); else if (maxv <= 2) LNJ_LAUNCH(2); else if (maxv <= 4) LNJ_LAUNCH(4);
+  else if (maxv <= 8) LNJ_LAUNCH(8); else if (maxv <= 16) LNJ_LAUNCH(16); else return DU_ERR_UNSUPPORTED;
+#undef LNJ_LAUNCH
+  return du_check_launch();
+}
+
+extern "C" int du_layernorm_fwd_jobs(int in_dtype, int out_dtype, const du_ln_job* jobs, int njobs, int D, float eps, void* stream) {
+  hipStream_t st = (hipStream_t)stream;
+  if (!jobs || njobs < 1 || njobs > DU_LN_JOBS_MAX || D <= 0) return DU_ERR_BAD_ARG;
+  const int vi = in_dtype == DU_BF16 ? 8 : 4;
+  if (D % vi) return DU_ERR_BAD_ARG;
+  LnJobTable T{};
+  T.njobs = njobs;
+  long wgs = 0;
+  for (int j = 0; j < njobs; j++) {
+    const du_ln_job& b = jobs[j];
+    if (b.rows <= 0 || !b.x || !b.y || !b.w || !b.b || b.ldx % vi || b.ldx < D || b.ldy < D) return DU_ERR_BAD_ARG;
+    wgs += (b.rows + 3) / 4;
+    if (wgs > 0x7fffffffL) return DU_ERR_BAD_ARG;
+    T.wg_end[j] = (int)wgs;
+    T.job[j] = b;
+  }
+  if (in_dtype == DU_F32 && out_dtype == DU_F32) return ln_fwd_jobs_dispatch<float, float>(T, (int)wgs, D, eps, st);
+  if (in_dtype == DU_F32 && out_dtype == DU_BF16) return ln_fwd_jobs_dispatch<float, bf16_t>(T, (int)wgs, D, eps, st);
+  if (in_dtype == DU_BF16 && out_dtype == DU_BF16) return ln_fwd_jobs_dispatch<bf16_t, bf16_t>(T, (int)wgs, D, eps, st);
+  if (in_dtype == DU_BF16 && out_dtype == DU_F32) return ln_fwd_jobs_dispatch<bf16_t, float>(T, (int)wgs, D, eps, st);
+  return DU_ERR_BAD_ARG;
+}
+
+extern "C" int du_layernorm_bwd_params_jobs(int dtype, const du_ln_job* jobs, int njobs, int D, float* dwdb, float* ws, int64_t ws_elems,
+                                            void* stream) {
+  hipStream_t st = (hipStream_t)stream;
+  if (!jobs || njobs < 1 || njobs > DU_LN_JOBS_MAX || D <= 0 || !dwdb || !ws) return DU_ERR_BAD_ARG;
+  if (dtype != DU_BF16 && dtype != DU_F32) return DU_ERR_BAD_ARG;
+  const int vi = dtype == DU_BF16 ? 8 : 4;
+  if (D % vi) return DU_ERR_BAD_ARG;
+  LnJobTable T{};
+  T.njobs = njobs;
+  const long rows = jobs[0].rows;
+  for (int j = 0; j < njobs; j++) {
+    const du_ln_job& b = jobs[j];
+    if (b.rows <= 0 || !b.x || !b.dy || !b.mean || !b.rstd || b.ldx % vi || b.ldx < D) return DU_ERR_BAD_ARG;
+    if (b.rows != rows) return DU_ERR_UNSUPPORTED;
+    T.job[j] = b;
+  }
+  const int STRIP = pick_strip(1, rows, D, vi);
+  const long strips = (rows + STRIP - 1) / STRIP;
+  if (ws_elems < (long)njobs * strips * D * 2 || (long)njobs * strips > 0x7fffffffL) return DU_ERR_BAD_ARG;
+  dim3 grid((unsigned)(njobs * strips)), block(256);
+  const int maxv = (D / vi + 63) / 64;
+  const size_t lds = (size_t)3 * D * 2 * sizeof(float);
+  const bool fused = maxv <= 4 && lds <= 64 * 1024;
+  float* part = ws;
+#define LNP_LAUNCH(TT, MV) hipLaunchKernelGGL((layernorm_bwd_params_jobs_kernel<TT, MV>), grid, block, lds, st, T, rows, D, STRIP, (int)strips, part)
+  if (fused && dtype == DU_BF16) { if (maxv <= 1) LNP_LAUNCH(bf16_t, 1); else if (maxv <= 2) LNP_LAUNCH(bf16_t, 2); else LNP_LAUNCH(bf16_t, 4); }
+  else if (fused) { if (maxv <= 1) LNP_LAUNCH(float, 1); else if (maxv <= 2) LNP_LAUNCH(float, 2); else LNP_LAUNCH(float, 4); }
+#undef LNP_LAUNCH
+  else if (dtype == DU_BF16) hipLaunchKernelGGL(layernorm_bwd_wb_jobs_kernel<bf16_t>, grid, block, 0, st, T, rows, D, STRIP, part);
+  else hipLaunchKernelGGL(layernorm_bwd_wb_jobs_kernel<float>, grid, block, 0, st, T, rows, D, STRIP, part);
+  if ((long)D * 2 >= 4096) {
+    const int chunks = (D * 2 + 31) / 32;
+    hipLaunchKernelGGL(finalize_kernel<32>, dim3((unsigned)(njobs * chunks)), dim3(256), 0, st, (const float*)part, dwdb, njobs, (int)strips, D * 2, 2);
+  } else {
+    const int chunks = (D * 2 + 3) / 4;
+    hipLaunchKernelGGL(finalize_kernel<4>, dim3((unsigned)(njobs * chunks)), dim3(256), 0, st, (const float*)part, dwdb, njobs, (int)strips, D * 2, 2);
+  }
+  return du_check_launch();
+}
+
 extern "C" int du_strip_finalize(const float* part, float* out, int G, int strips, int C, void* stream) {
   hipStream_t st = (hipStream_t)stream;
   if (!part || !out || G <= 0 || strips <= 0 || C <= 0) return DU_ERR_BAD_ARG;
diff --git a/dinounet_amd/dinov3/adapter.py b/dinounet_amd/dinov3/adapter.py
--- a/dinounet_amd/dinov3/adapter.py
+++ b/dinounet_amd/dinov3/adapter.py
@@ -44,14 +44,15 @@
         nn.init.constant_(self.output_proj.bias.data, 0.0)
 
     def forward(self, query, reference_points, input_flatten, input_spatial_shapes, input_level_start_index,
-                input_padding_mask=None, residual=None, query_norm=None):
+                input_padding_mask=None, residual=None, query_norm=None, value=None):
         assert input_padding_mask is None and self.n_levels == 1 and len(input_spatial_shapes) == 1
         N, Lq, _ = query.shape
-        _, S, _ = input_flatten.shape
+        _, S, _ = input_flatten.shape if value is None else value.shape
         Hs, Ws = input_spatial_shapes[0]
         assert Hs * Ws == S
         M, P = self.n_heads, self.n_points
-        value = ops.linear(input_flatten, self.value_proj.weight, self.value_proj.bias)
+        if value is None:
+            value = ops.linear(input_flatten, self.value_proj.weight, self.value_proj.bias)
         value = value.view(N, S, M, value.shape[-1] // M)
         if query_norm is not None:
             loc, attn, residual = ops.layer_norm_offsets_prep(query, query_norm.weight, query_norm.bias, query_norm.eps,
@@ -141,9 +142,10 @@
             self.ffn_norm = norm_layer(dim)
             self.drop_path = DropPath(drop_path) if drop_path > 0.0 else nn.Identity()
 
-    def forward(self, query, reference_points, feat, spatial_shapes, level_start_index, H, W):
-        fn = ops.layer_norm(feat, self.feat_norm.weight, self.feat_norm.bias, self.feat_norm.eps)
-        query = self.attn(query, reference_points, fn, spatial_shapes, level_start_index, None, query_norm=self.query_norm)
+    def forward(self, query, reference_points, feat, spatial_shapes, level_start_index, H, W, value=None):
+        fn = ops.layer_norm(feat, self.feat_norm.weight, self.feat_norm.bias, self.feat_norm.eps) if value is None else None
+        query = self.attn(query, reference_points, fn, spatial_shapes, level_start_index, None, query_norm=self.query_norm,
+                          value=value)
         if self.with_cffn:
             mask = self.drop_path.mask(query.shape[0], query.device) if isinstance(self.drop_path, DropPath) else None
             query = self.ffn(query, H, W, row_scale=mask, norm=self.ffn_norm)
@@ -161,11 +163,12 @@
         self.extractor = mk()
         self.extra_extractors = nn.Sequential(*[mk() for _ in range(2)]) if extra_extractor else None
 
-    def forward(self, x, c, ref, shapes, H_c, W_c):
-        c = self.extractor(c, ref, x, shapes, None, H_c, W_c)
-        if self.extra_extractors is not None:
-            for ex in self.extra_extractors:
-                c = ex(c, ref, x, shapes, None, H_c, W_c)
+    def extractors(self):
+        return [self.extractor] + (list(self.extra_extractors) if self.extra_extractors is not None else [])
+
+    def forward(self, x, c, ref, shapes, H_c, W_c, values=None):
+        for j, ex in enumerate(self.extractors()):
+            c = ex(c, ref, x, shapes, None, H_c, W_c, value=None if values is None else values[j])
         return c
 
 
@@ -308,6 +311,18 @@
     def backbone_layers(self, x):
         return self.backbone.get_intermediate_layers(x, n=self.interaction_indexes, return_class_token=True, dtype=_act_dtype(self))
 
+    def _feature_values(self, layers):
+        exs = [(i, ex) for i, blk in enumerate(self.interactions) for ex in blk.extractors()]
+        eps = {ex.feat_norm.eps for _, ex in exs}
+        if not exs or len(exs) > ops.FEAT_JOBS_MAX or len(eps) != 1 or len({layers[i][0].shape for i, _ in exs}) != 1:
+            return None
+        params = [(ex.feat_norm.weight, ex.feat_norm.bias, ex.attn.value_proj.weight, ex.attn.value_proj.bias) for _, ex in exs]
+        vals = ops.feature_values([layers[i][0] for i in range(len(self.interactions))], [i for i, _ in exs], params, eps.pop())
+        out = [[] for _ in self.interactions]
+        for (i, _), v in zip(exs, vals):
+            out[i].append(v)
+        return out
+
     def _forward(self, x, layers=None):
         dt = _act_dtype(self)
         B, _, H, W = x.shape
@@ -347,9 +362,10 @@
         elif layers is None:
             layers = self.backbone.get_intermediate_layers(x, n=self.interaction_indexes, return_class_token=True, dtype=dt)
 
+        values = self._feature_values(layers) if ops.FEAT_HOIST else None
         for i, layer in enumerate(self.interactions):
             xi, _cls = layers[i]
-            c = layer(xi, c, ref, shapes, H_c, W_c)
+            c = layer(xi, c, ref, shapes, H_c, W_c, values=None if values is None else values[i])
 
         c2, c3, c4 = c.split([n2, n3, c.shape[1] - n2 - n3], dim=1)
         c2 = c2.contiguous().view(B, H_c * 2, W_c * 2, D)
diff --git a/dinounet_amd/ops.py b/dinounet_amd/ops.py
--- a/dinounet_amd/ops.py
+++ b/dinounet_amd/ops.py
@@ -1606,6 +1606,193 @@
 
 def layer_norm_res(x, w, b, eps):
     return _LayerNorm.apply(x, w, b, eps, True)
+
+
+FEAT_HOIST = _ab_env("DINOUNET_FEAT_HOIST", "1") == "1"
+FEAT_JOBS_MAX = min(_lib.GEMM_JOBS_MAX, _lib.LN_JOBS_MAX)
+
+
+def _gemm_jobs_args(xs, ws, biases, outs):
+    x0, w0, o0 = xs[0], ws[0], outs[0]
+    a = GemmArgs()
+    a.dtype, a.out_dtype, a.a_mode, a.b_mode = _code(x0.dtype), _code(o0.dtype), PLAIN_ROW, PLAIN_ROW
+    a.batch, a.split_k, a.alpha, a.act = 1, 1, 1.0, ACT_NONE
+    jobs = (_lib.GemmJob * len(xs))()
+    for j, (x, w, o) in enumerate(zip(xs, ws, outs)):
+        _req(x, w, o)
+        M, K, lda = _rows2d(x)
+        N, K2, ldb = _rows2d(w)
+        assert K == K2 and x.dtype == w.dtype == x0.dtype and o.dtype == o0.dtype and o.shape == (M, N), (x.shape, w.shape, o.shape)
+        jb = jobs[j]
+        jb.A, jb.lda, jb.B, jb.ldb, jb.C, jb.ldc = x.data_ptr(), lda, w.data_ptr(), ldb, o.data_ptr(), o.stride(0)
+        jb.bias = _dp(biases[j]) if biases is not None else None
+        jb.M, jb.N, jb.K = M, N, K
+    return a, jobs
+
+
+def mm_jobs_plan(xs, ws, biases, outs):
+    a, jobs = _gemm_jobs_args(xs, ws, biases, outs)
+    d = (C.c_int64 * 6)()
+    assert _lib.lib().du_gemm_jobs_plan_describe(C.byref(a), jobs, len(xs), d, 6) == 6
+    return list(d)
+
+
+def mm_jobs(xs, ws, biases=None, outs=None):
+    if outs is None:
+        outs = [torch.empty((x.shape[0], w.shape[0]), dtype=x.dtype, device=x.device) for x, w in zip(xs, ws)]
+    a, jobs = _gemm_jobs_args(xs, ws, biases, outs)
+    if PROFILE is not None:
+        e0 = PROFILE.start()
+        grouped = mm_jobs_plan(xs, ws, biases, outs)[1]
+    _lib.check(_lib.lib().du_gemm_jobs(C.byref(a), jobs, len(xs), _st()), "du_gemm_jobs")
+    if PROFILE is not None:
+        M, K = xs[0].shape
+        N = ws[0].shape[0]
+        n = len(xs)
+        tag = f"{'gemm_nt_pp_jobs_kernel' if grouped else 'du_gemm_jobs(loop)'}<{'bf16' if xs[0].dtype == torch.bfloat16 else 'f32'},linear>"
+        if PROFILE.detail:
+            tag += f" M{M} N{N} K{K} jobs{n}"
+        es = xs[0].element_size()
+        PROFILE.stop(tag, e0, 2.0 * M * N * K * n, float(n) * es * (M * K + N * K + M * N))
+    return outs
+
+
+def _ln_jobs(xs, ws=None, bs=None, ys=None, means=None, rstds=None, dys=None):
+    jobs = (_lib.LnJob * len(xs))()
+    for j, x in enumerate(xs):
+        rows, D, ld = _rows2d(x)
+        jb = jobs[j]
+        jb.x, jb.ldx, jb.rows = x.data_ptr(), ld, rows
+        if ws is not None:
+            jb.w, jb.b, jb.y, jb.ldy = ws[j].data_ptr(), bs[j].data_ptr(), ys[j].data_ptr(), ys[j].stride(0)
+        jb.mean, jb.rstd = _dp(means[j]) if means is not None else None, _dp(rstds[j]) if rstds is not None else None
+        if dys is not None:
+            assert dys[j].is_contiguous() and dys[j].shape == x.shape and dys[j].dtype == x.dtype
+            jb.dy = dys[j].data_ptr()
+    return jobs
+
+
+def layernorm_jobs_raw(xs, ws, bs, eps, out_dtype, want_stats=False):
+    _req(*xs)
+    D = xs[0].shape[1]
+    assert 1 <= len(xs) <= _lib.LN_JOBS_MAX and all(x.shape[1] == D and x.dtype == xs[0].dtype for x in xs)
+    ys = [torch.empty((x.shape[0], D), dtype=out_dtype, device=x.device) for x in xs]
+    means = rstds = None
+    if want_stats:
+        means = [torch.empty(x.shape[0], dtype=torch.float32, device=x.device) for x in xs]
+        rstds = [torch.empty(x.shape[0], dtype=torch.float32, device=x.device) for x in xs]
+    jobs = _ln_jobs(xs, ws, bs, ys, means, rstds)
+    _lib.check(_lib.lib().du_layernorm_fwd_jobs(_code(xs[0].dtype), _code(out_dtype), jobs, len(xs), D, eps, _st()), "du_layernorm_fwd_jobs")
+    return ys, means, rstds
+
+
+def layernorm_bwd_params_jobs_raw(xs, dys, means, rstds):
+    _req(*xs)
+    rows, D = xs[0].shape
+    assert 1 <= len(xs) <= _lib.LN_JOBS_MAX and all(x.shape == (rows, D) and x.dtype == xs[0].dtype for x in xs)
+    dwdb = torch.empty((len(xs), 2, D), dtype=torch.float32, device=xs[0].device)
+    n = len(xs) * int(_lib.lib().du_reduce_ws_elems(_code(xs[0].dtype), 1, rows, D))
+    ws = torch.empty(max(n, 1), dtype=torch.float32, device=xs[0].device)
+    jobs = _ln_jobs(xs, means=means, rstds=rstds, dys=dys)
+    _lib.check(_lib.lib().du_layernorm_bwd_params_jobs(_code(xs[0].dtype), jobs, len(xs), D, _p(dwdb), _p(ws), n, _st()),
+               "du_layernorm_bwd_params_jobs")
+    return dwdb
+
+
+class _FeatValues(torch.autograd.Function):
+
+    @staticmethod
+    def forward(ctx, eps, idx, *args):
+        nt = max(idx) + 1
+        taps, par = args[:nt], args[nt:]
+        J = len(idx)
+        assert len(par) == 4 * J
+        xcs = [t.contiguous() for t in taps]
+        dt = xcs[0].dtype
+        x2 = [xcs[i].view(-1, xcs[i].shape[-1]) for i in idx]
+        lnw = [_f32(par[4 * j]) for j in range(J)]
+        lnb = [_f32(par[4 * j + 1]) for j in range(J)]
+        fns, means, rstds = layernorm_jobs_raw(x2, lnw, lnb, eps, dt, True)
+        wqs, wTs, biases, wrefs = [], [], [], []
+        for j in range(J):
+            w, bias = par[4 * j + 2], par[4 * j + 3]
+            wq = w
+            if w.dtype != dt:
+                wq = PACK.get(w, PK_CAST, dt)
+                if wq is None:
+                    wq = w.to(dt)
+                elif wq.dim() != 2:
+                    wq = wq.view(w.shape[0], -1)
+            wqs.append(wq)
+            wTs.append(PACK.get(w, PK_TRANSPOSE, dt) if (_DGRAD_NT and w.dtype != dt and w.shape[0] % 64 == 0) else None)
+            biases.append(_f32(bias))
+            wrefs.append(WGRAD.note_use(*([w] if bias is None else [w, bias])))
+        vals = mm_jobs(fns, wqs, biases)
+        ctx.save_for_backward(*xcs, *fns, *means, *rstds, *wqs, *[t for t in wTs if t is not None], *lnw)
+        ctx.idx, ctx.nt, ctx.wrefs = idx, nt, wrefs
+        ctx.has_wT = [t is not None for t in wTs]
+        ctx.has_bias = [par[4 * j + 3] is not None for j in range(J)]
+        return tuple(v.view(*taps[i].shape[:-1], v.shape[-1]) for v, i in zip(vals, idx))
+
+    @staticmethod
+    def backward(ctx, *dvals):
+        idx, nt = ctx.idx, ctx.nt
+        J = len(idx)
+        sv = list(ctx.saved_tensors)
+        take = lambda n: [sv.pop(0) for _ in range(n)]
+        xcs, fns, means, rstds, wqs = take(nt), take(J), take(J), take(J), take(J)
+        wTs = [sv.pop(0) if h else None for h in ctx.has_wT]
+        lnw = take(J)
+        dt = xcs[0].dtype
+        D = xcs[0].shape[-1]
+        x2 = [xcs[i].view(-1, D) for i in idx]
+        dys = []
+        for j, dv in enumerate(dvals):
+            d2 = dv.reshape(-1, dv.shape[-1])
+            d2 = d2 if d2.is_contiguous() else d2.contiguous()
+            dys.append(d2 if d2.dtype == dt else cast(d2, dt))
+        if all(t is not None for t in wTs):
+            dfn = mm_jobs(dys, wTs)
+        else:
+            dfn = [mm(dys[j], wTs[j]) if wTs[j] is not None else mm_dgrad(dys[j], wqs[j]) for j in range(J)]
+        need_dx = [ctx.needs_input_grad[2 + i] for i in range(nt)]
+        dtaps = [None] * nt
+        if not any(need_dx) and len({x.shape for x in x2}) == 1:
+            dwdb = layernorm_bwd_params_jobs_raw(x2, dfn, means, rstds)
+        else:
+            dwdb = torch.empty((J, 2, D), dtype=torch.float32, device=xcs[0].device)
+            for j in range(J):
+                rows = x2[j].shape[0]
+                dx = torch.empty_like(x2[j])
+                ws, n = _reduce_ws(dt, 1, rows, D, dx.device)
+                _lib.check(_lib.lib().du_layernorm_bwd(_code(dt), _p(x2[j]), _p(dfn[j]), _p(lnw[j]), _p(means[j]), _p(rstds[j]), _p(dx), _p(dwdb[j]),
+                                                       rows, D, _p(ws), n, None, _st()), "du_layernorm_bwd")
+                if need_dx[idx[j]]:
+                    dx = dx.view(xcs[idx[j]].shape)
+                    dtaps[idx[j]] = dx if dtaps[idx[j]] is None else dtaps[idx[j]] + dx
+        grads = []
+        for j in range(J):
+            need_w, need_b = ctx.needs_input_grad[2 + nt + 4 * j + 2], ctx.has_bias[j] and ctx.needs_input_grad[2 + nt + 4 * j + 3]
+            dw = db = None
+            if need_w:
+                grp = WGRAD.begin(ctx.wrefs[j])
+                if need_b:
+                    dw, db = mm_wgrad(dys[j], fns[j], with_colsum=True, defer=grp)
+                else:
+                    dw = mm_wgrad(dys[j], fns[j], defer=grp)
+                if grp is not None and not grp["ret"]:
+                    dw = db = None
+            elif need_b:
+                db = colsum(dys[j])
+            grads += [dwdb[j, 0], dwdb[j, 1], dw, db]
+        return (None, None, *dtaps, *grads)
+
+
+def feature_values(taps, idx, params, eps):
+    if not taps[0].is_cuda:
+        return [linear(layer_norm(taps[i], lw, lb, eps), w, b) for i, (lw, lb, w, b) in zip(idx, params)]
+    flat = [p for ps in params for p in ps]
+    return list(_FeatValues.apply(eps, tuple(idx), *taps, *flat))
 
 
 def msda_forward_raw(value, shapes, lsi, loc, attn):
diff --git a/include/dinounet_hip.h b/include/dinounet_hip.h
--- a/include/dinounet_hip.h
+++ b/include/dinounet_hip.h
@@ -79,6 +79,18 @@
 int du_gemm_route(const du_gemm_args* args);
 int du_gemm_plan_describe(const du_gemm_args* args, int64_t* out, int n);
 
+#define DU_GEMM_JOBS_MAX 8
+typedef struct du_gemm_job {
+  const void* A; int64_t lda;
+  const void* B; int64_t ldb;
+  void* C; int64_t ldc;
+  const float* bias;
+  int32_t M, N, K;
+  int32_t reserved;
+} du_gemm_job;
+int du_gemm_jobs(const du_gemm_args* shape, const du_gemm_job* jobs, int njobs, void* stream);
+int du_gemm_jobs_plan_describe(const du_gemm_args* shape, const du_gemm_job* jobs, int njobs, int64_t* out, int n);
+
 typedef struct du_tn_job {
   const void* A; int64_t lda;
   const void* B; int64_t ldb;
@@ -122,6 +134,17 @@
 int64_t du_reduce_ws_elems(int dtype, int G, int64_t pix_per_group, int C);
 int du_layernorm_bwd(int dtype, const void* x, const void* dy, const float* w, const float* mean, const float* rstd,
                      void* dx, float* dwdb, int64_t rows, int D, float* ws, int64_t ws_elems, const void* dres, void* stream);
+#define DU_LN_JOBS_MAX 8
+typedef struct du_ln_job {
+  const void* x; int64_t ldx;
+  const float* w; const float* b;
+  void* y; int64_t ldy;
+  float* mean; float* rstd;
+  int64_t rows;
+  const void* dy;
+} du_ln_job;
+int du_layernorm_fwd_jobs(int in_dtype, int out_dtype, const du_ln_job* jobs, int njobs, int D, float eps, void* stream);
+int du_layernorm_bwd_params_jobs(int dtype, const du_ln_job* jobs, int njobs, int D, float* dwdb, float* ws, int64_t ws_elems, void* stream);
 int du_layernorm_bwd_prod_plan(int dtype, const void* x, const void* G, int64_t ldg, const void* Wt, int64_t ldw, int K, const void* dx,
                                const void* dres, int64_t rows, int D, int64_t* out, int n);
 int du_layernorm_bwd_prod(int dtype, const void* x, const void* G, int64_t ldg, const void* Wt, int64_t ldw, int K, const float* w,
```

New measurement: 323.9 slices/s, median of 6. About the same (+0.9%).
